# TAU-VAILab/Vox-E

Hardware: AMD Instinct MI355X
Metric: rendered rays/sec (fwd+bwd) (higher is better)
Workload: dtype f32; 1 GPU; 160^3 SH-0 softplus ReLU-field grid (random), one 400x400 camera per GPU and step, the steps cycle through 20 cameras of the 100-view set, S=256, jitter on, white bkgd, ray order image; step = render fwd + bwd + Adam (fused grid step); grid=160, samples_per_ray=256, grad_exchange=single, optimizer=fused

## Files before the change

### include/voxe.h

```cpp
#ifndef VOXE_H_
#define VOXE_H_

#include <stddef.h>
#include <stdint.h>

#ifdef __cplusplus
extern "C" {
#endif

#define VOXE_ABI_VERSION 13

typedef enum VoxeStatus {
  VOXE_OK = 0,
  VOXE_ERR_NULL_POINTER = -1,
  VOXE_ERR_BAD_SHAPE = -2,
  VOXE_ERR_UNSUPPORTED = -3,
  VOXE_ERR_WORKSPACE = -4,
  VOXE_ERR_LAUNCH = -5,
  VOXE_ERR_NO_DEVICE = -6
} VoxeStatus;

typedef enum VoxeAct {
  VOXE_ACT_IDENTITY = 0,
  VOXE_ACT_ABS = 1,
// ... 139 lines not shown
int voxe_render_bwd_acc_into(const VoxeGridDesc* grid, const VoxeRenderCfg* cfg,
                             const float* rays_o, const float* rays_d, int64_t R, const float* jitter,
                             const float* colour, const float* depth, const float* acc,
                             const float* d_colour, const float* d_depth, const float* d_acc,
                             int32_t want_densities, int32_t want_features, int32_t zero_first, int32_t* grad_layout,
                             void* workspace, size_t workspace_bytes, void* grad_workspace, size_t grad_workspace_bytes,
                             void* stream);
int voxe_render_bwd_layout(const VoxeGridDesc* grid, const VoxeRenderCfg* cfg, int64_t R);
size_t voxe_workspace_grad_offset(const VoxeGridDesc* grid);
size_t voxe_workspace_grad_bytes(const VoxeGridDesc* grid);
typedef struct VoxeGridRegularisers {
  const float* dcl_reference;
  float dcl_weight;
  float* dcl_loss;
  void* scratch;
  size_t scratch_bytes;
  int32_t density_kind;
  const float* feat_reference;
  float feat_weight;
  float* feat_loss;
} VoxeGridRegularisers;
int voxe_grid_adam_step(const VoxeGridDesc* grid, int32_t grad_layout, int32_t x_begin, int32_t x_end,
                        const float* extra_d_densities, const float* extra_d_features,
                        float* exp_avg_densities, float* exp_avg_sq_densities,
                        float* exp_avg_features, float* exp_avg_sq_features,
                        float lr, float beta1, float beta2, float eps, int64_t step, int64_t step_features,
                        const VoxeGridRegularisers* regularisers ,
                        void* workspace, size_t workspace_bytes, void* stream);

enum { VOXE_ROUTE_NONE = -1, VOXE_ROUTE_SCATTER = 0, VOXE_ROUTE_TILE = 1, VOXE_ROUTE_PACKED_SCATTER = 2,
       VOXE_ROUTE_REGION = 3, VOXE_ROUTE_DETERMINISTIC = 4 };
int voxe_render_route(const VoxeGridDesc* grid, const VoxeRenderCfg* cfg, int64_t R);

int voxe_disparity_bwd(const float* depth, const float* acc, const float* d_disparity, const float* d_depth_in,
                       const float* d_acc_in, float* d_depth_out, float* d_acc_out, int64_t R, void* stream);

typedef struct {
  int32_t H, W;
  float focal;
  const float* poses;
  const int64_t* image_rows;
  const float* images;
  int32_t num_images;
  int32_t K;
  int64_t batch;
  int32_t diffuse_regularisation;
  float lr, beta1, beta2, eps;
  int64_t step_densities, step_features;
  float *exp_avg_densities, *exp_avg_sq_densities, *exp_avg_features, *exp_avg_sq_features;
  float* losses;
  int32_t zero_gradient_first;
} VoxeReconStep;
size_t voxe_recon_scratch_bytes(int64_t batch);
int voxe_recon_step(const VoxeGridDesc* grid, const VoxeRenderCfg* cfg, const VoxeReconStep* step,
                    void* workspace, size_t workspace_bytes, void* workspace2, size_t workspace2_bytes,
                    void* scratch, size_t scratch_bytes, void* stream);
int voxe_recon_prefetch(const VoxeGridDesc* grid, const VoxeRenderCfg* cfg, const VoxeReconStep* next_step,
                        void* workspace, size_t workspace_bytes, void* workspace2, size_t workspace2_bytes,
                        void* scratch, size_t scratch_bytes, void* stream);
int voxe_recon_prefetch_stats(int64_t* out);

size_t voxe_attn_masked_l1_scratch_bytes(void);
int voxe_attn_masked_l1(const float* render, const float* attn_map, int64_t n, float* d_render, float* loss_out,
                        void* scratch, size_t scratch_bytes, void* stream);

typedef struct {
  const float* attn_map;
  float tv_weight;
  int32_t tv_loss_always;
  float lr, beta1, beta2, eps;
  int64_t step;
  float *exp_avg, *exp_avg_sq;
  float* losses;
  float* attn_render;
  int32_t zero_gradient_first;
} VoxeAttnRefineStep;
size_t voxe_attn_refine_scratch_bytes(const VoxeGridDesc* grid, int64_t R);
int voxe_attn_refine_step(const VoxeGridDesc* grid, const VoxeRenderCfg* cfg, const VoxeAttnRefineStep* step,
                          const float* rays_o, const float* rays_d, int64_t R, void* workspace, size_t workspace_bytes,
                          void* scratch, size_t scratch_bytes, void* stream);

int voxe_clock_probe(int32_t spin, double* shader_hz, void* stream);
int voxe_region_debug_layout(const VoxeGridDesc* grid, const VoxeRenderCfg* cfg, int64_t R, int64_t out[17]);

int voxe_adam_step(float* param, const float* grad, float* exp_avg, float* exp_avg_sq, int64_t n,
                   float lr, float beta1, float beta2, float eps, int64_t step, void* stream);

int voxe_upsample_trilinear(const float* src, int32_t X, int32_t Y, int32_t Z, int32_t C,
                            float* dst, int32_t X2, int32_t Y2, int32_t Z2, void* stream);


#define VOXE_GRAPH_CAP_ONE (1 << 28)
enum { VOXE_DIR_XP = 0, VOXE_DIR_XM = 1, VOXE_DIR_YP = 2, VOXE_DIR_YM = 3, VOXE_DIR_ZP = 4, VOXE_DIR_ZM = 5 };

int voxe_graph_build(const float* density_grid, const float* feature_grid,
                     int32_t X, int32_t Y, int32_t Z, int32_t F, float sigma, int32_t dilate_yz,
                     uint8_t* node_mask, int32_t* cap, void* stream);

size_t voxe_graphcut_scratch_bytes(int32_t X, int32_t Y, int32_t Z);
int voxe_graphcut(const uint8_t* node_mask, const int8_t* terminal, int32_t* cap,
                  int32_t X, int32_t Y, int32_t Z, uint8_t* segment, int64_t* flow,
                  void* scratch, size_t scratch_bytes, void* stream);

size_t voxe_cc_scratch_bytes(int32_t X, int32_t Y, int32_t Z, int32_t k);
int voxe_cc_largest_k(const uint8_t* mask, int32_t X, int32_t Y, int32_t Z, int32_t k,
                      int32_t* labels, int32_t* num_components,
                      void* scratch, size_t scratch_bytes, void* stream);

size_t voxe_mesh_scratch_bytes(int32_t X, int32_t Y, int32_t Z);
int voxe_mesh_count(const VoxeGridDesc* grid, float level, const uint8_t* mask, int64_t* totals,
                    void* scratch, size_t scratch_bytes, void* stream);
int voxe_mesh_emit(const VoxeGridDesc* grid, float level, const uint8_t* mask,
                   float* vertices, int64_t max_vertices, int32_t* faces, int64_t max_faces,
                   void* scratch, size_t scratch_bytes, void* stream);

int voxe_query_normals(const VoxeGridDesc* grid, const float* points, int64_t N, float* normals, void* stream);
int voxe_render_normals(const VoxeGridDesc* grid, const VoxeRenderCfg* cfg,
                        const float* rays_o, const float* rays_d, int64_t R, const float* jitter,
                        float* normals, float* depth, float* acc, void* stream);

int voxe_visibility_accumulate(const VoxeGridDesc* grid, const VoxeRenderCfg* cfg,
                               const float* rays_o, const float* rays_d, int64_t R, const float* jitter,
                               float* max_weight , float* max_trans ,
                               void* stream);
int voxe_visibility_mask(const float* vis, int32_t X, int32_t Y, int32_t Z, float threshold, int32_t dilate,
                         uint8_t* mask , void* stream);

size_t voxe_distortion_scratch_bytes(int64_t R);
int voxe_distortion_fwd_bwd(const VoxeGridDesc* grid, const VoxeRenderCfg* cfg,
                            const float* rays_o, const float* rays_d, int64_t R, const float* jitter,
                            float grad_scale,
                            float* loss_out      ,
                            float* ray_loss      ,
                            float* d_densities   ,
                            int32_t accumulate   ,
                            void* scratch, size_t scratch_bytes, void* stream);
int voxe_distortion_debug_lanes(int32_t lanes);

int voxe_cpu_cast_rays(int32_t H, int32_t W, float focal, const float* rot, const float* trans,
                       float* rays_o, float* rays_d);
int voxe_cpu_cast_rays_indexed(int32_t H, int32_t W, float focal, const float* poses, int32_t K,
                               const int64_t* flat_index, int64_t B, float* rays_o, float* rays_d);
int voxe_cpu_random_subset(int64_t n, int64_t count, uint64_t seed, uint64_t rng_offset, int64_t* out);
int voxe_cpu_render_fwd(const VoxeGridDesc* grid, const VoxeRenderCfg* cfg,
                        const float* rays_o, const float* rays_d, int64_t R, const float* jitter,
                        float* colour, float* depth, float* acc, float* disparity);
int voxe_cpu_render_bwd(const VoxeGridDesc* grid, const VoxeRenderCfg* cfg,
                        const float* rays_o, const float* rays_d, int64_t R, const float* jitter,
                        const float* d_colour, const float* d_depth, const float* d_acc,
                        float* d_densities, float* d_features, int32_t accumulate);
int voxe_cpu_query_fwd(const VoxeGridDesc* grid, const float* points, int64_t N, float* out);
int voxe_cpu_query_bwd(const VoxeGridDesc* grid, const float* points, int64_t N, const float* d_out,
                       float* d_densities, float* d_features, int32_t accumulate);
int voxe_cpu_sample_probe(const VoxeGridDesc* grid, const VoxeRenderCfg* cfg,
                          const float* rays_o, const float* rays_d, int64_t R, const float* jitter,
                          int32_t* idx, uint8_t* inside, float* zvals, float* sigma, float* rad);
int voxe_cpu_dcl_fwd_bwd(const float* a, const float* b, int64_t n, float grad_scale,
                         float* loss_out, float* d_a, int32_t accumulate);
int voxe_cpu_density_diff_fwd_bwd(const float* a, const float* b, int64_t n, int32_t kind, float grad_scale,
                                  float* loss_out, float* d_a, int32_t accumulate);
int voxe_cpu_feature_correlation_fwd_bwd(const float* f, const float* r, int64_t nvox, int32_t F, float grad_scale,
                                         float* loss_out, float* d_f, int32_t accumulate);
int voxe_cpu_tv_fwd_bwd(const float* grid, int32_t X, int32_t Y, int32_t Z, int32_t C,
                        float grad_scale, float* loss_out, float* d_grid, int32_t accumulate);
int voxe_cpu_adam_step(float* param, const float* grad, float* exp_avg, float* exp_avg_sq,
                       int64_t n, float lr, float beta1, float beta2, float eps, int64_t step);
// ... 17 lines not shown
```

### vox-e_amd/csrc/voxe_api.hip

```cpp
#include <hip/hip_runtime.h>
#include <stdlib.h>
#include <string.h>

#include <mutex>
#include <unordered_map>

#include "../../include/voxe.h"
#include "voxe_launch.hpp"
#include "voxe_render_common.hpp"

using namespace voxe;

namespace {

const VoxeDispatch kDefaultDispatch = {};
const VoxeDispatch& disp_of(const VoxeRenderCfg* c) { return (c && c->dispatch) ? *c->dispatch : kDefaultDispatch; }
bool force_scatter_bwd(const VoxeDispatch& d) { return d.bwd_mode == 1; }
bool force_no_tile_bwd(const VoxeDispatch& d) { return d.bwd_mode != 0; }
bool two_phase_disabled(const VoxeDispatch& d) { return d.tile_two_phase < 0; }

int tile_map_mode(int image_width, const VoxeDispatch& d) {
  if (d.tile_map >= 1 && d.tile_map <= 3) return d.tile_map - 1;
  return image_width > 0 ? 0 : 1;
}
// ... 238 lines not shown

int voxe_device_check(char* name, size_t name_len) {
  int dev = 0;
  if (hipGetDevice(&dev) != hipSuccess) return VOXE_ERR_NO_DEVICE;
  hipDeviceProp_t prop;
  if (hipGetDeviceProperties(&prop, dev) != hipSuccess) return VOXE_ERR_NO_DEVICE;
  if (name && name_len) {
    strncpy(name, prop.gcnArchName, name_len - 1);
    name[name_len - 1] = 0;
  }
  return strncmp(prop.gcnArchName, "gfx950", 6) == 0 ? VOXE_OK : VOXE_ERR_NO_DEVICE;
}

int voxe_profile_enable(int32_t on) {
  if (on && !g_prof.created) {
    for (int i = 0; i < Profiler::kMax; ++i)
      for (int j = 0; j < 2; ++j)
        if (hipEventCreate(&g_prof.ev[i][j]) != hipSuccess) return VOXE_ERR_LAUNCH;
    g_prof.created = true;
  }
  g_prof.on = on != 0;
  g_prof.count = 0;
  g_prof.dropped = 0;
  return VOXE_OK;
}

int voxe_profile_read(VoxeProfile* out) {
  if (!out) return VOXE_ERR_NULL_POINTER;
  memset(out, 0, sizeof(*out));
  double* ms[PH_COUNT] = {&out->ms_pack, &out->ms_fwd, &out->ms_memset, &out->ms_bwd, &out->ms_unpack};
  int32_t* n[PH_COUNT] = {&out->n_pack, &out->n_fwd, &out->n_memset, &out->n_bwd, &out->n_unpack};
  for (int i = 0; i < g_prof.count; ++i) {
    if (hipEventSynchronize(g_prof.ev[i][1]) != hipSuccess) return VOXE_ERR_LAUNCH;
    float t = 0.f;
    if (hipEventElapsedTime(&t, g_prof.ev[i][0], g_prof.ev[i][1]) != hipSuccess) return VOXE_ERR_LAUNCH;
    *ms[g_prof.phase[i]] += (double)t;
    *n[g_prof.phase[i]] += 1;
  }
  out->n_dropped = g_prof.dropped;
  g_prof.count = 0;
  g_prof.dropped = 0;
  return VOXE_OK;
}

int voxe_cast_rays(int32_t H, int32_t W, float focal, const float* rot, const float* trans,
                   float* rays_o, float* rays_d, void* stream) {
  if (!rot || !trans || !rays_o || !rays_d) return VOXE_ERR_NULL_POINTER;
  if (H <= 0 || W <= 0) return VOXE_ERR_BAD_SHAPE;
  launch_cast_rays(H, W, focal, rot, trans, rays_o, rays_d, (hipStream_t)stream);
  return finish();
}

int voxe_cast_rays_indexed(int32_t H, int32_t W, float focal, const float* poses, int32_t K,
                           const int64_t* flat_index, int64_t B, float* rays_o, float* rays_d, void* stream) {
  if (!poses || !flat_index || !rays_o || !rays_d) return VOXE_ERR_NULL_POINTER;
  if (H <= 0 || W <= 0 || K <= 0 || B < 0) return VOXE_ERR_BAD_SHAPE;
  if (B == 0) return VOXE_OK;
  launch_cast_rays_indexed(H, W, focal, poses, K, (const long long*)flat_index, B, rays_o, rays_d,
                           (hipStream_t)stream);
  return finish();
}

int voxe_random_subset(int64_t n, int64_t count, uint64_t seed, uint64_t rng_offset, int64_t* out, void* stream) {
  if (!out) return VOXE_ERR_NULL_POINTER;
  if (n <= 0 || n > (1ll << 31) || count < 0 || count > n) return VOXE_ERR_BAD_SHAPE;
  if (count == 0) return VOXE_OK;
  launch_random_subset(n, count, seed, rng_offset, (long long*)out, (hipStream_t)stream);
  return finish();
}

int voxe_tile_sched_debug_layout(const VoxeGridDesc* grid, const VoxeRenderCfg* cfg, int64_t R, int64_t out[4]) {
  Variant v;
  const int st = validate(grid, cfg, R, &v);
  if (st) return st;
  if (!out) return VOXE_ERR_NULL_POINTER;
  DevGrid dg; HostCfg dc;
  make_dev(grid, cfg, R, v, &dg, &dc);
  const WsLayout l = ws_layout(grid, cfg, R);
  const int64_t ntp = dc.image_width > 0 ? blocks_for_tiles(dc.map_mode, (dc.image_width + 7) / 8, tile_rows_total(dc, 8)) : 0;
  out[0] = (l.total > l.sched_off && tile_sched_applies(dc)) ? 1 : 0;
  out[1] = (int64_t)l.sched_off;
  out[2] = ntp * num_segments(dc.S, dc.seg_len);
  out[3] = ntp;
  return VOXE_OK;
}

size_t voxe_workspace_bytes(const VoxeGridDesc* grid, const VoxeRenderCfg* cfg, int64_t R) {
  if (!grid || grid->X <= 0 || grid->Y <= 0 || grid->Z <= 0 || grid->F <= 0) return 0;
  const WsLayout l = ws_layout(grid, cfg, R);
  if (cfg && cfg->ray_state_valid < 0) return l.total;
  return l.total_with_src;
}

int voxe_render_fwd(const VoxeGridDesc* grid, const VoxeRenderCfg* cfg, const float* rays_o,
                    const float* rays_d, int64_t R, const float* jitter, float* colour, float* depth,
                    float* acc, float* disparity, void* workspace, size_t workspace_bytes,
                    void* stream) {
  Variant v;
  const int st = validate(grid, cfg, R, &v);
  if (st) return st;
  if (R > 0 && (!rays_o || !rays_d || !colour)) return VOXE_ERR_NULL_POINTER;
  const WsLayout l = ws_layout(grid, cfg, R);
  if (!workspace || workspace_bytes < l.fwd_total) return VOXE_ERR_WORKSPACE;
  hipStream_t s = (hipStream_t)stream;
  float* packed = (float*)((char*)workspace + l.packed_off);
  if (!cfg->reuse_packed_grid) { PhaseTimer t(PH_PACK, s); launch_pack_any(grid, packed, s); }
  if (R == 0) return finish();
  {
    FwdStamp k = make_stamp(grid, cfg, rays_o, rays_d, R, jitter, workspace_bytes);
    k.kept = cfg->ray_state_valid >= 0 ? 1 : 0;
    record_stamp(workspace, k);
  }
  DevGrid dg; HostCfg dc;
  make_dev(grid, cfg, R, v, &dg, &dc);
  float* state = nullptr;
  const bool tiled = tile_bwd_supported(dc, cfg->sh_degree) && !force_no_tile_bwd(dc.disp);
  const bool packed_bwd = !tiled && packed_scatter_supported(cfg->sh_degree) && !force_scatter_bwd(dc.disp);
  if ((tiled || packed_bwd) && workspace_bytes >= l.total) state = (float*)((char*)workspace + l.state_off);
  float* segbuf = workspace_bytes >= l.total ? (float*)((char*)workspace + l.seg_off) : nullptr;
  FwdArgs a{packed, rays_o, rays_d, jitter, colour, depth, acc, disparity, state, segbuf};
  a.keep_samples = cfg->ray_state_valid >= 0;
  if (segbuf && cfg->ray_state_valid >= 0 && precise_sums_apply(l, dg, dc, cfg, jitter)) a.segsum_d = (double*)((char*)workspace + l.prec_off);
  if (segbuf && l.total > l.sched_off) a.sched = (int*)((char*)workspace + l.sched_off);
  if (cfg->ray_state_valid >= 0 && tiled && l.fwdval_off > l.src_off && workspace_bytes >= l.total_with_src && !two_phase_disabled(dc.disp))
    a.sample_fwd = (float*)((char*)workspace + l.fwdval_off);
  if (l.region && workspace_bytes >= l.total_with_src) {
    PhaseTimer t(PH_FWD, s);
    launch_fwd_region(dg, dc, cfg->sh_degree, cfg->render_diffuse, a, (char*)workspace + l.region_off, s);
    return finish();
  }
  { PhaseTimer t(PH_FWD, s); launch_fwd(dg, dc, cfg->sh_degree, cfg->render_diffuse, a, s); }
  return finish();
}

}

namespace {
int render_bwd_common(const VoxeGridDesc* grid, const VoxeRenderCfg* cfg, const Variant& v, const float* rays_o,
                      const float* rays_d, int64_t R, const float* jitter, const float* colour, const float* depth,
                      const float* acc, const float* d_colour, const float* d_depth, const float* d_acc, bool want_d,
                      bool want_f, bool zero_first, bool* bricked, void* workspace, size_t workspace_bytes,
                      hipStream_t s, void* grad_workspace = nullptr, size_t grad_workspace_bytes = 0) {
  const WsLayout l = ws_layout(grid, cfg, R);
  if (!workspace || workspace_bytes < l.total) return VOXE_ERR_WORKSPACE;
  if (grad_workspace && grad_workspace_bytes < l.state_off) return VOXE_ERR_WORKSPACE;
  float* packed = (float*)((char*)workspace + l.packed_off);
  float* gpacked = (float*)((char*)(grad_workspace ? grad_workspace : workspace) + l.grad_off);
  float* state = (float*)((char*)workspace + l.state_off);
  if (!cfg->reuse_packed_grid) { PhaseTimer t(PH_PACK, s); launch_pack_any(grid, packed, s); }
  if (zero_first) {
    PhaseTimer t(PH_MEMSET, s);
    if (hipMemsetAsync(gpacked, 0, l.state_off - l.grad_off, s) != hipSuccess) return VOXE_ERR_LAUNCH;
  }
  *bricked = false;
  if (R > 0) {
    DevGrid dg; HostCfg dc;
    make_dev(grid, cfg, R, v, &dg, &dc);
    const bool tiled = tile_bwd_supported(dc, cfg->sh_degree) && !force_no_tile_bwd(dc.disp);
    const bool packed_bwd = !tiled && packed_scatter_supported(cfg->sh_degree) && !force_scatter_bwd(dc.disp);
    BwdArgs a{packed, rays_o, rays_d, jitter, colour, depth, acc, d_colour, d_depth, d_acc, gpacked,
              want_d, want_f, (tiled || packed_bwd) ? state : nullptr};
    const bool precise = precise_sums_apply(l, dg, dc, cfg, jitter);
    if (precise) a.segsum_d = (const double*)((char*)workspace + l.prec_off);
    if (l.total > l.sched_off) a.sched = (const int*)((char*)workspace + l.sched_off);
    const bool two_phase = tiled && l.fwdval_off > l.src_off && workspace_bytes >= l.total_with_src && !two_phase_disabled(dc.disp);
    if (two_phase) {
// ... 981 lines not shown
```

### vox-e_amd/csrc/voxe_launch.hpp

```cpp
#pragma once

#include <hip/hip_runtime.h>

#include "voxe_device.hpp"

namespace voxe {

struct FwdArgs {
  const float *packed, *rays_o, *rays_d, *jitter;
  float *colour, *depth, *acc, *disparity;
  float* ray_state;
  float* segbuf;
  float* sample_fwd = nullptr;
  bool keep_samples = true;
  double* segsum_d = nullptr;
  int* sched = nullptr;
};
struct BwdArgs {
  const float *packed, *rays_o, *rays_d, *jitter, *colour, *depth, *acc, *d_colour, *d_depth, *d_acc;
  float* gpacked;
  bool want_d, want_f;
  const float* ray_state;
  float* sample_src = nullptr;
  const float* sample_fwd = nullptr;
  float* grad_planar = nullptr;
  unsigned long long* gdet = nullptr;
  float* det_scale = nullptr;
  const double* segsum_d = nullptr;
  const int* sched = nullptr;
};
struct HostCfg : DevCfg {
  VoxeDispatch disp;
};
inline long long disp_tile_min_rays(const VoxeDispatch& d) { return d.tile_min_rays == 0 ? 8192ll : (d.tile_min_rays < 0 ? 0ll : (long long)d.tile_min_rays); }
inline long long disp_region_min_rays(const VoxeDispatch& d) { return d.region_min_rays == 0 ? 16384ll : (long long)d.region_min_rays; }
inline bool disp_region_lds_ranks(const VoxeDispatch& d) { return d.region_lds_ranks >= 0; }
inline float disp_region_image_ratio(const VoxeDispatch& d) { return d.region_image_ratio == 0.0f ? 1.3f : (d.region_image_ratio < 0.0f ? 0.0f : d.region_image_ratio); }
inline float disp_or(float v, float dflt) { return v == 0.0f ? dflt : v; }

struct ProbeArgs {
  const float *packed, *rays_o, *rays_d, *jitter;
  int32_t* idx;
  uint8_t* inside;
  float *zvals, *sigma, *rad;
};


void launch_pack_any(const VoxeGridDesc* gd, float* packed, hipStream_t st);
void launch_unpack_any(const VoxeGridDesc* gd, const float* gpacked, float* d_dens, float* d_feat,
                       int accumulate, int bricked, hipStream_t st);
struct DclTerm {
  const float* b = nullptr;
  const double* stats = nullptr;
  int kind = 0;
  float k = 0.0f;
  const float* fref = nullptr;
  float fk = 0.0f;
};
bool launch_grid_adam(const VoxeGridDesc* gd, bool bricked, int x_begin, int x_end, float* gpacked, const float* extra_d, const float* extra_f,
                      float* m_d, float* v_d, float* m_f, float* v_f, float lr, float beta1, float beta2, float eps,
                      long long step_d, long long step_f, float* packed_out, hipStream_t st, DclTerm dcl = DclTerm());
const double* launch_dcl_moments(const float* a, const float* b, long long n, float grad_scale, float* loss_out, void* scratch,
                                 hipStream_t st);
void launch_fwd(const DevGrid& g, const HostCfg& c, int deg, int diffuse, const FwdArgs& a,
                hipStream_t st);
void launch_bwd(const DevGrid& g, const DevCfg& c, int deg, int diffuse, const BwdArgs& a,
                hipStream_t st);
void launch_probe(const DevGrid& g, const DevCfg& c, int deg, int diffuse, const ProbeArgs& a,
                  hipStream_t st);

void launch_query(const DevGrid& g, int C, const float* packed, const float* points, long long N, float* out,
                  const float* d_out, float* gpacked, bool want_d, bool want_f, hipStream_t st);

bool tile_bwd_supported(const HostCfg& c, int deg);
size_t tile_src_bytes(long long R, int W, int H, int S, int deg, int diffuse, int attn);
void launch_bwd_tile(const DevGrid& g, const HostCfg& c, int deg, int diffuse, const BwdArgs& a, hipStream_t st);
bool tile4_bwd_supported(const DevGrid& g, const HostCfg& c, const BwdArgs& a, int kl);
void launch_bwd_tile4(const DevGrid& g, const HostCfg& c, const BwdArgs& a, int kl, int nb, int qsplit, float fit_m, float fit_lat,
                      hipStream_t st);
size_t tile_planar_bytes(long long nvox, int cm);
bool tile4_dep_supported(const DevGrid& g, const HostCfg& c, const BwdArgs& a, int ncu, int cm);
void launch_bwd_tile4_dep(const DevGrid& g, const HostCfg& c, const BwdArgs& a, int ncu, int nb, int qsplit, int ngrp, float fit_m,
                          float fit_lat, hipStream_t st);
bool fwd_tile4_supported(const DevGrid& g, const HostCfg& c, const FwdArgs& a, int cout, int ncm);
void launch_fwd_tile4(const DevGrid& g, const HostCfg& c, const FwdArgs& a, hipStream_t st);
bool tile_sched_applies(const HostCfg& c);
size_t tile_sched_bytes(long long R, int W, int H, int S);
bool fwd_tile_supported(const DevGrid& g, const HostCfg& c, int cout, int ncm);
void launch_fwd_tile(const DevGrid& g, const HostCfg& c, const FwdArgs& a, hipStream_t st);
bool fwd_tilew_supported(const DevGrid& g, const HostCfg& c, const FwdArgs& a, int cout, int ncm, int ncu);
void launch_fwd_tilew(const DevGrid& g, const HostCfg& c, int ncm, const FwdArgs& a, hipStream_t st);
bool det_bwd_supported(const DevCfg& c, int deg, int diffuse);
size_t det_bytes(long long nvox, int C);

bool packed_scatter_supported(int deg);
void launch_bwd_packed_scatter(const DevGrid& g, const DevCfg& c, int deg, int diffuse, const BwdArgs& a, hipStream_t st);

bool region_bwd_supported(const DevGrid& g, const HostCfg& c, int deg, int diffuse, bool tiled);
size_t region_scratch_bytes(int X, int Y, int Z, long long R, int S, bool full_sh);
void launch_fwd_region(const DevGrid& g, const HostCfg& c, int deg, int diffuse, const FwdArgs& a, void* scratch,
                       hipStream_t st);
void launch_bwd_region(const DevGrid& g, const DevCfg& c, int deg, int diffuse, const BwdArgs& a, void* scratch,
                       hipStream_t st);
struct RegionBins { void* tables; int prebinned; hipEvent_t after_fwd; };
extern thread_local const RegionBins* tl_region_bins;
void launch_bin_region(const DevGrid& g, const HostCfg& c, const float* rays_o, const float* rays_d, const float* jitter, void* tables,
                       hipStream_t st, int phase = 3);
void region_debug_layout(int X, int Y, int Z, long long R, int S, long long out[16]);

void launch_cast_rays(int H, int W, float focal, const float* rot, const float* trans, float* rays_o,
                      float* rays_d, hipStream_t st);
void launch_cast_rays_indexed(int H, int W, float focal, const float* poses, int K, const long long* flat_index,
                              long long B, float* rays_o, float* rays_d, hipStream_t st);
void launch_random_subset(long long n, long long count, unsigned long long seed, unsigned long long rng_offset,
                          long long* out, hipStream_t st);
size_t dcl_scratch_bytes(long long n);
void launch_density_diff(const float* a, const float* b, long long n, int kind, float grad_scale, float* loss_out, float loss_norm,
                         float* d_a, int accumulate, void* scratch, hipStream_t st);
void launch_feature_correlation(const float* f, const float* r, long long nvox, int F, float grad_scale, float* loss_out, float* d_f,
                                int accumulate, void* scratch, hipStream_t st);
void launch_dcl(const float* a, const float* b, long long n, float grad_scale, float* loss_out,
                float* d_a, int accumulate, void* scratch, hipStream_t st);
size_t tv_scratch_bytes(int X, int Y, int Z, int C);
void launch_tv(const float* grid, int X, int Y, int Z, int C, float grad_scale, float* loss_out,
               float* d_grid, int accumulate, void* scratch, hipStream_t st);
void launch_adam(float* param, const float* grad, float* m, float* v, long long n, float lr,
                 float beta1, float beta2, float eps, long long step, hipStream_t st);
void launch_upsample(const float* src, int X, int Y, int Z, int C, float* dst, int X2, int Y2, int Z2,
                     hipStream_t st);
void launch_disparity_bwd(const float* depth, const float* acc, const float* d_disp, const float* d_depth_in,
                          const float* d_acc_in, float* d_depth_out, float* d_acc_out, long long R, hipStream_t st);
void launch_gather_pixels(const float* images, const long long* image_rows, const long long* subset, long long B, int per,
                          int num_images, float* out, hipStream_t st);
size_t l1_scratch_bytes();
void launch_l1_loss_grad(const float* a, const float* b, long long n, float* d_a, float* out2, void* scratch, hipStream_t st);
size_t attn_l1_scratch_bytes();
void launch_attn_masked_l1(const float* render, const float* map, long long n, float* d_render, float* loss_out, void* scratch,
                           hipStream_t st);
void launch_l1_loss_grad_n(const float* a, const float* b, long long n, int renders, float* d_a, float* out2, void* scratch,
                           hipStream_t st);
void launch_recon_batch(long long B, unsigned long long seed, unsigned long long rng_offset, int H, int W, float focal, int K,
                        const float* poses, const float* images, const long long* image_rows, int num_images, long long* subset,
                        float* rays_o, float* rays_d, float* target, hipStream_t st);
double run_clock_probe(int spin, hipStream_t st);


void launch_graph_build(const float* dens, const float* feat, int X, int Y, int Z, int F, float sigma,
                        int dilate_yz, uint8_t* node_mask, int32_t* cap, hipStream_t stream);
size_t graphcut_scratch_bytes(int X, int Y, int Z);
hipError_t run_graphcut(const uint8_t* node_mask, const int8_t* terminal, int32_t* cap, int X, int Y, int Z,
                        uint8_t* segment, int64_t* flow, void* scratch, hipStream_t stream);
size_t cc_scratch_bytes(int X, int Y, int Z, int k);
void launch_cc_largest_k(const uint8_t* mask, int X, int Y, int Z, int k, int32_t* labels, int32_t* ncomp,
                         void* scratch, hipStream_t stream);

bool mesh_dims_ok(int X, int Y, int Z);
size_t mesh_scratch_bytes(int X, int Y, int Z);
void launch_mesh_count(const VoxeGridDesc* g, float L, const uint8_t* mask, int64_t* totals, void* scratch, hipStream_t st);
void launch_mesh_emit(const VoxeGridDesc* g, float L, const uint8_t* mask, float* vertices, long long max_vertices,
                      int32_t* faces, long long max_faces, void* scratch, hipStream_t st);

int normals_lanes_for(long long R);
void launch_query_normals(const DevGrid& g, const float* dens, const float* points, long long N, float* normals, hipStream_t st);
void launch_render_normals(const DevGrid& g, const DevCfg& c, const float* dens, const float* rays_o, const float* rays_d,
                           const float* jitter, float* normals, float* depth, float* acc, hipStream_t st);

void launch_visibility_accumulate(const DevGrid& g, const DevCfg& c, const float* dens, const float* rays_o, const float* rays_d,
                                  const float* jitter, float* max_weight, float* max_trans, hipStream_t st);
void launch_visibility_mask(const float* vis, int X, int Y, int Z, float threshold, int dilate, uint8_t* mask, hipStream_t st);

// ... 9 lines not shown
```

### vox-e_amd/csrc/voxe_render_tile.hip

```cpp
#include <limits.h>
#include <stdlib.h>

#include <type_traits>

#include "voxe_device.hpp"
#include "voxe_launch.hpp"
#include "voxe_render_common.hpp"
#include "voxe_tile_window.hpp"

namespace voxe {

template <int WC, int KL, bool DET = false>
__device__ __forceinline__ void flush_layer(double* __restrict__ win, float* __restrict__ gpacked,
                                            const Window& w, int key, int lane, int CM, int memch,
                                            unsigned long long* __restrict__ gdet = nullptr) {
  constexpr int C = WC;
  constexpr int kLat = KL, kLayerSlots = Lat<KL>::kLayerSlots;
  constexpr int kPerInstr = 64 / C;
  constexpr int NJ = (kLayerSlots + kPerInstr - 1) / kPerInstr;
  const int im = w.sgn * key;
  const int offu = __builtin_amdgcn_readfirstlane(w.off_u(im)), offv = __builtin_amdgcn_readfirstlane(w.off_v(im));
  const long long vox0 = (long long)im * w.stride_m + (long long)offu * w.stride_u + (long long)offv * w.stride_v;
  const int ch = lane % C;
  int idx[NJ];
// ... 887 lines not shown
        Cell cell;
        make_cell_fast(g, fp, cell);
        float v, rad[COUT];
        gather<3, 1, 1>(g, packed, cell, rc.basis, v, rad);
        const float sigma = post_activate(g.post_act, v);
        const float dl = last ? kInfinity : (z_next - z);
        const float delta = dl * rc.dnorm;
        const float e = fast_exp(-(sigma * delta));
        const float alpha = 1.0f - e;
        const float om = 1.0f - alpha;
        const float wgt = alpha * T;
        T = T * om;
#pragma unroll
        for (int ch = 0; ch < COUT; ++ch) csum[ch] = fmaf(sigmoidf(rad[ch]), wgt, csum[ch]);
        asum = asum + wgt;
        dsum = fmaf(z, wgt, dsum);
      }
    }
  };
  auto march_tile = [&](auto strata_tag) {
    constexpr bool ST = decltype(strata_tag)::value;
    const SegDepth<ST> sd{strat, ks};
    if (m < 0) march_rays(strata_tag);
    else if (m == 0) fwd_window_march<0, ST>(g, c, packed, rc, lane, has, k_lo, k_hi, kmin, kmax, ref, tex, org, sd, csum, asum, dsum, T);
    else if (m == 1) fwd_window_march<1, ST>(g, c, packed, rc, lane, has, k_lo, k_hi, kmin, kmax, ref, tex, org, sd, csum, asum, dsum, T);
    else fwd_window_march<2, ST>(g, c, packed, rc, lane, has, k_lo, k_hi, kmin, kmax, ref, tex, org, sd, csum, asum, dsum, T);
  };
  if (use_strata) march_tile(std::true_type{});
  else march_tile(std::false_type{});
  if (!alive) return;
  const long long base = (long long)seg * NC;
  segbuf[(base + 0) * c.R + r] = T;
#pragma unroll
  for (int ch = 0; ch < COUT; ++ch) segbuf[(base + 1 + ch) * c.R + r] = csum[ch];
  segbuf[(base + 1 + COUT) * c.R + r] = asum;
  segbuf[(base + 2 + COUT) * c.R + r] = dsum;
}

bool fwd_tile_supported(const DevGrid& g, const HostCfg& c, int cout, int ncm) {
  (void)g;
  if (cout != 3 || ncm != 1 || c.image_width <= 0) return false;
  return c.disp.fwd_window >= 0;
}
void launch_fwd_tile(const DevGrid& g, const HostCfg& c, const FwdArgs& a, hipStream_t st) {
  const int nseg = num_segments(c.S, c.seg_len);
  const int nb = blocks_for_tiles(c.map_mode, (c.image_width + 7) / 8, tile_rows_total(c, 8)) * nseg;
  const float fit_lat = disp_or(c.disp.fwd_fit_lat, 5.5f), fit_m = disp_or(c.disp.fwd_fit_m, 4.5f);
  const float zdom = disp_or(c.disp.fwd_zdom, 1.0f), max_adv = disp_or(c.disp.fwd_max_adv, 1.7f);
  render_fwd_tile_kernel<<<nb, 64, 0, st>>>(g, c, a.packed, a.rays_o, a.rays_d, a.jitter, a.segbuf, fit_lat, fit_m, zdom, max_adv);
}

bool tile_bwd_supported(const HostCfg& c, int deg) {
  (void)deg;
  return c.image_width > 0 && c.R >= disp_tile_min_rays(c.disp);
}

__global__ void det_scale_kernel(float* __restrict__ det_scale) {
  for (int i = 0; i < 2; ++i) {
    int e = 0;
    const float m = det_scale[i];
    if (m > 0.0f && m < 3.0e38f) (void)frexpf(m, &e);
    det_scale[2 + i] = ldexpf(1.0f, 38 - e);
  }
}
__global__ __launch_bounds__(256) void det_finalize_kernel(unsigned long long* __restrict__ gdet, float* __restrict__ gpacked,
                                                           long long n, int CM, const float* __restrict__ det_scale) {
  const double inv_f = 1.0 / (double)det_scale[2], inv_d = 1.0 / (double)det_scale[3];
  const long long stride = (long long)gridDim.x * blockDim.x;
  for (long long i = (long long)blockIdx.x * blockDim.x + threadIdx.x; i < n; i += stride) {
    const long long q = (long long)gdet[i];
    if (q != 0) {
      gpacked[i] += (float)((double)q * ((int)(i % CM) == CM - 1 ? inv_d : inv_f));
      gdet[i] = 0ull;
    }
  }
}
size_t det_bytes(long long nvox, int C) { return (((size_t)nvox * C * 8 + 255) / 256 + 1) * 256; }
bool det_bwd_supported(const DevCfg& c, int deg, int diffuse) {
  return c.image_width > 0 && (c.attn || deg == 0 || diffuse);
}

constexpr float kWideWindowRatio = 0.58f;

template <int COUT, int NCM, int NCU>
static void launch_bwd_tile_t(const DevGrid& g, const HostCfg& c, const BwdArgs& a, hipStream_t st) {
  const long long ntx8 = (c.image_width + 7) / 8, nty8 = tile_rows_total(c, 8);
  const int env_q = c.disp.tile_qsplit;
  constexpr int NG = COUT * NCU + 1, WC = NG < 4 ? NG : 4, NGRP = (NG + WC - 1) / WC;
  const int grp_begin = a.want_f ? 0 : NGRP - 1, ngrp = a.want_f ? NGRP : 1;
  const long long tiles = ntx8 * nty8 * num_segments(c.S, c.seg_len) * ngrp;
  const int qsplit = env_q ? (env_q == 4 ? 4 : 1) : (tiles <= 11000 ? 4 : 1);
  const int nb = blocks_for_tiles(c.map_mode, ntx8, nty8) * num_segments(c.S, c.seg_len) * qsplit * ngrp;
  const float env_fit_m = c.disp.tile_fit_m;
  const long long tile_segs = ntx8 * nty8 * num_segments(c.S, c.seg_len);
  const int side_for_kl = g.X > g.Y ? (g.X > g.Z ? g.X : g.Z) : (g.Y > g.Z ? g.Y : g.Z);
  const bool wide = (float)side_for_kl >= kWideWindowRatio * (float)c.image_width;
  const float env_fit_lat = c.disp.tile_fit_lat;
  const float fit_lat = env_fit_lat;
  const float fit_m = env_fit_m > 0.0f ? env_fit_m : (qsplit == 4 ? (wide ? 4.5f : 4.0f) : (tile_segs <= 16000 ? 4.5f : 5.5f));
#define VOXE_TBWD(WD, WF, MODE, KL, NB, GB, NGR)                                                 \
  render_bwd_tile_kernel<COUT, NCM, NCU, WD, WF, MODE, KL><<<NB, 64, 0, st>>>(                    \
      g, c, a.packed, a.rays_o, a.rays_d, a.jitter, a.colour, a.depth, a.acc, a.d_colour,         \
      a.d_depth, a.d_acc, a.ray_state, a.gpacked, qsplit, GB, NGR, reinterpret_cast<float4*>(a.sample_src), nullptr, nullptr, 0, fit_m, fit_lat, \
      reinterpret_cast<const float4*>(a.sample_fwd))
  if constexpr (NGRP == 1) {
    if (a.gdet) {
      const long long n = (long long)g.X * g.Y * g.Z * (COUT * NCM + 1);
      (void)hipMemsetAsync(a.det_scale, 0, 4 * sizeof(float), st);
      for (int phase = 0; phase < 2; ++phase) {
        render_bwd_tile_kernel<COUT, NCM, NCU, true, true, 0, 8, true><<<nb, 64, 0, st>>>(
            g, c, a.packed, a.rays_o, a.rays_d, a.jitter, a.colour, a.depth, a.acc, a.d_colour, a.d_depth, a.d_acc,
            a.ray_state, a.gpacked, qsplit, 0, 1, nullptr, a.gdet, a.det_scale, phase, fit_m, fit_lat);
        if (phase == 0) det_scale_kernel<<<1, 1, 0, st>>>(a.det_scale);
      }
      det_finalize_kernel<<<4096, 256, 0, st>>>(a.gdet, a.gpacked, n, COUT * NCM + 1, a.det_scale);
      return;
    }
  }
  if constexpr (NGRP > 1) {
    if (a.sample_src && a.want_f) {
      if (a.want_d) VOXE_TBWD(true, true, 1, 8, nb / ngrp, 0, 1);
      else VOXE_TBWD(false, true, 1, 8, nb / ngrp, 0, 1);
      if (NCM == NCU && tile4_dep_supported(g, c, a, NCU, COUT * NCM + 1))
        launch_bwd_tile4_dep(g, c, a, NCU, nb, qsplit, ngrp, fit_m, fit_lat, st);
      else
        VOXE_TBWD(true, true, 2, 8, nb, 0, ngrp);
      return;
    }
    if (a.want_d && a.want_f) VOXE_TBWD(true, true, 0, 8, nb, grp_begin, ngrp);
    else if (a.want_d) VOXE_TBWD(true, false, 0, 8, nb, grp_begin, ngrp);
    else VOXE_TBWD(false, true, 0, 8, nb, grp_begin, ngrp);
  } else {
    const int env_kl = c.disp.tile_kl;
    const int side = g.X > g.Y ? (g.X > g.Z ? g.X : g.Z) : (g.Y > g.Z ? g.Y : g.Z);
    const int kl = env_kl ? env_kl : ((float)side >= kWideWindowRatio * (float)c.image_width ? 10 : 8);
#define VOXE_TBWD_KL(KL)                                                       \
    do {                                                                       \
      if (a.want_d && a.want_f) VOXE_TBWD(true, true, 0, KL, nb, 0, 1);         \
      else if (a.want_d) VOXE_TBWD(true, false, 0, KL, nb, 0, 1);               \
      else VOXE_TBWD(false, true, 0, KL, nb, 0, 1);                             \
    } while (0)
    if constexpr (COUT == 3 && NCM == 1 && NCU == 1) {
      if (tile4_bwd_supported(g, c, a, kl)) {
        launch_bwd_tile4(g, c, a, kl, nb, qsplit, fit_m, fit_lat, st);
        return;
      }
    }
    if (kl == 10) VOXE_TBWD_KL(10);
#ifdef VOXE_TILE_KL_EXPERIMENTS
    else if (kl == 9 && COUT == 3 && NCM == 1 && a.want_d && a.want_f) VOXE_TBWD(true, true, 0, 9, nb, 0, 1);
    else if (kl == 12 && COUT == 3 && NCM == 1 && a.want_d && a.want_f) VOXE_TBWD(true, true, 0, 12, nb, 0, 1);
    else if (kl == 16 && COUT == 3 && NCM == 1 && a.want_d && a.want_f) VOXE_TBWD(true, true, 0, 16, nb, 0, 1);
#endif
    else VOXE_TBWD_KL(8);
#undef VOXE_TBWD_KL
  }
#undef VOXE_TBWD
}

size_t tile_src_bytes(long long R, int W, int H1, int S, int deg, int diffuse, int attn) {
  if (W <= 0 || R <= 0 || deg <= 0 || diffuse || attn) return 0;
  const long long H = H1 > 0 ? H1 : R / W, nimg = R / (H * W);
  const long long tiles = ((W + 7) / 8) * ((H + 7) / 8) * (nimg > 0 ? nimg : 1);
  const int seg = seg_len_for(R);
  const size_t bytes = (size_t)tiles * num_segments(S, seg) * seg * 64 * sizeof(float4);
  return bytes <= ((size_t)4 << 30) ? bytes : 0;
}

void launch_bwd_tile(const DevGrid& g, const HostCfg& c, int deg, int diffuse, const BwdArgs& a, hipStream_t st) {
  if (c.attn) launch_bwd_tile_t<1, 1, 1>(g, c, a, st);
  else if (deg == 0) launch_bwd_tile_t<3, 1, 1>(g, c, a, st);
  else if (deg == 1) { if (diffuse) launch_bwd_tile_t<3, 4, 1>(g, c, a, st); else launch_bwd_tile_t<3, 4, 4>(g, c, a, st); }
  else if (deg == 2) { if (diffuse) launch_bwd_tile_t<3, 9, 1>(g, c, a, st); else launch_bwd_tile_t<3, 9, 9>(g, c, a, st); }
  else { if (diffuse) launch_bwd_tile_t<3, 16, 1>(g, c, a, st); else launch_bwd_tile_t<3, 16, 16>(g, c, a, st); }
}

}
```

### vox-e_amd/csrc/voxe_render_tile4.hip

```cpp
#include <limits.h>

#include <type_traits>

#include "voxe_device.hpp"
#include "voxe_launch.hpp"
#include "voxe_render_common.hpp"
#include "voxe_tile_window.hpp"

namespace voxe {

#ifndef VOXE_TILE4_LB
#define VOXE_TILE4_LB 3
#endif
#ifndef VOXE_T4_EXP
#define VOXE_T4_EXP 0
#endif
#ifndef VOXE_T4_SKEW
#define VOXE_T4_SKEW 0
#endif
#ifndef VOXE_T4_CHJ
#define VOXE_T4_CHJ 1
#endif
#ifndef VOXE_T4_PHASE_MARGIN
#define VOXE_T4_PHASE_MARGIN 0.0f
#endif
#ifndef VOXE_T4_REMAT
#define VOXE_T4_REMAT 0
#endif
#ifndef VOXE_T4_DEBUG
#define VOXE_T4_DEBUG 0
#endif

struct Tile4Args {
  const float *packed, *rays_o, *rays_d, *colour, *depth, *acc, *d_colour, *d_depth, *d_acc, *ray_state;
  float* gpacked;
  int qsplit;
  float fit_m, fit_lat;
  int want_d, want_f;
  int phases;
  const double* segsum;
  const float4* sample_src;
  int ngrp, ng;
  long long nvox;
  const int* sched;
};

constexpr int kSchedMaxBuckets = 9;
constexpr int kSchedMaxSegs = 64;
constexpr int kSchedEmpty = (int)0x80000000;
constexpr long long kSchedMaxBlocks = 1ll << 18;
#ifndef VOXE_SCHED_BUCKET
#define VOXE_SCHED_BUCKET 4
#endif
static_assert(VOXE_SCHED_BUCKET >= 4 && 32 / VOXE_SCHED_BUCKET + 1 <= kSchedMaxBuckets, "bucket rows of the schedule histogram");

template <class RC>
__device__ __forceinline__ void seg_sample_range(const RC& rc, const bool alive, const int ks, const int ke, int& k_lo, int& k_hi) {
  k_lo = max(rc.k_lo, ks);
  k_hi = alive ? min(rc.k_hi, ke) : k_lo - 1;
}
__device__ __forceinline__ int sched_rank(int it, int nbk) {
  return it == 0 ? nbk - 1 : nbk - 1 - min((it + VOXE_SCHED_BUCKET - 1) / VOXE_SCHED_BUCKET, nbk - 1);
}

__global__ __launch_bounds__(1024) void tile_sched_cost_kernel(const DevGrid g, const DevCfg c, const float* __restrict__ rays_o,
                                                               const float* __restrict__ rays_d, const int ntp, const int nbk,
                                                               const int hstride, unsigned char* __restrict__ cost,
                                                               unsigned char* __restrict__ hist) {
  __shared__ unsigned char rk[kSchedMaxSegs][16];
  const int lane = threadIdx.x & 63, w = threadIdx.x >> 6;
  const int rb = blockIdx.x * 16 + w;
  const int nseg = num_segments(c.S, c.seg_len);
  const int ntx = (c.image_width + 7) >> 3, nty = (int)tile_rows_total(c, 8);
  const int tile = rb < ntp ? logical_tile_of(c, rb, ntp, ntx, nty) : -1;
  if (tile < 0) {
    for (int seg = lane; seg < nseg; seg += 64) {
      if (rb < ntp) cost[(long long)seg * ntp + rb] = 0;
      rk[seg][w] = rb < ntp ? (unsigned char)(nbk - 1) : (unsigned char)255;
    }
  } else {
    const int ty = tile / ntx, tx = tile - ty * ntx;
    long long r_px;
    const bool alive = tile_pixel_ray(c, ty, lane >> 3, (tx << 3) + (lane & 7), 8, r_px);
    const long long r = alive ? r_px : 0;
    RayCtx<3, 1, 1> rc;
    rc.init(g, c, r, rays_o, rays_d, nullptr);
    for (int seg = 0; seg < nseg; ++seg) {
      const int ks = seg * c.seg_len, ke = min(c.S, ks + c.seg_len) - 1;
      int k_lo, k_hi;
      seg_sample_range(rc, alive, ks, ke, k_lo, k_hi);
      const bool has = k_lo <= k_hi;
      const int kmin = wave_min_i32(has ? k_lo : INT_MAX);
      const int kmax = wave_max_i32(has ? k_hi : -1);
      const int it = kmin <= kmax ? kmax - kmin + 1 : 0;
      if (lane == 0) {
        cost[(long long)seg * ntp + rb] = (unsigned char)it;
        rk[seg][w] = (unsigned char)sched_rank(it, nbk);
      }
    }
  }
  __syncthreads();
  const int ngrp = gridDim.x;
  for (int p = threadIdx.x; p < nseg * nbk; p += 1024) {
    const int seg = p / nbk, r = p - seg * nbk;
    int n = 0;
#pragma unroll
    for (int i = 0; i < 16; ++i) n += rk[seg][i] == r ? 1 : 0;
    hist[(long long)r * hstride + seg * ngrp + blockIdx.x] = (unsigned char)n;
  }
}

__device__ __forceinline__ int wave_sum_i32(int v) {
#pragma unroll
  for (int d = 1; d < 64; d <<= 1) v += __shfl_xor(v, d, 64);
  return v;
}

__global__ __launch_bounds__(256) void tile_sched_scatter_kernel(const unsigned char* __restrict__ cost,
                                                                 const unsigned char* __restrict__ hist, const int ntp,
                                                                 const int ngrp, const int nbk, const int hstride,
                                                                 int* __restrict__ list) {
  __shared__ int s_tot[kSchedMaxBuckets], s_pre[kSchedMaxBuckets], s_base[kSchedMaxBuckets];
  __shared__ int s_wc[kSchedMaxBuckets][4];
  const int tid = threadIdx.x, lane = tid & 63, w = tid >> 6;
  const int seg = blockIdx.y, nseg = gridDim.y;
  const int H = nseg * ngrp;
  const int G0 = seg * ngrp + blockIdx.x * 16;
  for (int r = w; r < nbk; r += 4) {
    const unsigned int* row = reinterpret_cast<const unsigned int*>(hist + (long long)r * hstride);
    int tot = 0, pre = 0;
    for (int q = lane; q * 4 < H; q += 64) {
      const unsigned int v = row[q];
#pragma unroll
      for (int i = 0; i < 4; ++i) {
        const int e = 4 * q + i, n = (int)(v >> (8 * i) & 255u);
        tot += e < H ? n : 0;
        pre += e < G0 ? n : 0;
      }
    }
    tot = wave_sum_i32(tot); pre = wave_sum_i32(pre);
    if (lane == 0) { s_tot[r] = tot; s_pre[r] = pre; }
  }
  const int rb = blockIdx.x * 256 + tid;
  const bool valid = rb < ntp;
  const int b = seg * ntp + rb;
  const int it = valid ? (int)cost[b] : 0;
  const int rank = valid ? sched_rank(it, nbk) : -1;
  int within = 0, mine = 0;
  for (int r = 0; r < nbk; ++r) {
    const unsigned long long m = __ballot(rank == r);
    if (rank == r) within = __popcll(m & ((1ull << lane) - 1ull));
    if (lane == r) mine = __popcll(m);
  }
  if (lane < nbk) s_wc[lane][w] = mine;
  __syncthreads();
  if (tid < nbk) {
    int base = s_pre[tid];
    for (int r = 0; r < tid; ++r) base += s_tot[r];
    s_base[tid] = base;
  }
  __syncthreads();
  if (valid) {
    int pos = s_base[rank] + within;
    for (int i = 0; i < w; ++i) pos += s_wc[rank][i];
    list[pos] = it == 0 ? (b | kSchedEmpty) : b;
  }
}

bool tile_sched_applies(const HostCfg& c) {
  if ((c.disp.tile_map != 0 && c.disp.tile_map != 4) || c.image_width <= 0 || c.attn || c.disp.fwd_segments_per_thread > 1) return false;
  const int nseg = num_segments(c.S, c.seg_len);
  const long long tiles = (long long)((c.image_width + 7) / 8) * tile_rows_total(c, 8);
  const long long nb = (long long)blocks_for_tiles(c.map_mode, (c.image_width + 7) / 8, tile_rows_total(c, 8)) * nseg;
  return nseg > 1 && nseg <= kSchedMaxSegs && c.seg_len <= 32 && (tiles * nseg > 11000 || c.disp.tile_map == 4) && nb <= kSchedMaxBlocks;
}
static long long sched_hist_stride(long long ntp, int nseg) { return ((ntp + 15) / 16 * nseg + 3) / 4 * 4; }
static long long sched_cost_bytes(long long nb) { return (nb + 15) / 16 * 16; }
size_t tile_sched_bytes(long long R, int W, int H1, int S) {
  if (W <= 0 || R <= 0) return 0;
  const long long H = H1 > 0 ? H1 : R / W, nimg = R / (H * W);
  const long long ntp = (((W + 7) / 8) * ((H + 7) / 8) * (nimg > 0 ? nimg : 1) + 7) / 8 * 8;
  const int nseg = num_segments(S, seg_len_for(R));
  const long long nb = ntp * nseg;
  if (nb > kSchedMaxBlocks) return 0;
  return (size_t)nb * sizeof(int) + (size_t)sched_cost_bytes(nb) + (size_t)(kSchedMaxBuckets * sched_hist_stride(ntp, nseg));
}
static void build_tile_sched(const DevGrid& g, const HostCfg& c, const float* rays_o, const float* rays_d, int* sched, hipStream_t st) {
  const int nseg = num_segments(c.S, c.seg_len);
  const int ntp = blocks_for_tiles(c.map_mode, (c.image_width + 7) / 8, tile_rows_total(c, 8));
  const int nb = ntp * nseg;
  unsigned char* cost = reinterpret_cast<unsigned char*>(sched + nb);
  unsigned char* hist = cost + sched_cost_bytes(nb);
  const int nbk = (c.seg_len + VOXE_SCHED_BUCKET - 1) / VOXE_SCHED_BUCKET + 1;
  const int ngrp = (ntp + 15) / 16, hstride = (int)sched_hist_stride(ntp, nseg);
  tile_sched_cost_kernel<<<ngrp, 1024, 0, st>>>(g, c, rays_o, rays_d, ntp, nbk, hstride, cost, hist);
  tile_sched_scatter_kernel<<<dim3((ntp + 255) / 256, nseg), 256, 0, st>>>(cost, hist, ntp, ngrp, nbk, hstride, sched);
}

struct DepCtx {
  float mA[4], mB[4];
  int cA, cB;
  long long src_base;
};

constexpr int kTabKeys = 64;

template <int KL>
struct Pcb {
  static_assert(WinMap<KL, 4>::kPcb, "the lean kernel needs the parity-class banked window");
  static constexpr int SB = WinMap<KL, 4>::kSB * 8, SA = WinMap<KL, 4>::kSA * 8, SS = WinMap<KL, 4>::kSS * 8;
  static __device__ __forceinline__ int mterm(int slot) { return (slot >> 1) * SS + ((slot & 1) << 5); }
  static __device__ __forceinline__ int aterm(int x_even) { return (x_even >> 1) * SA; }
  static __device__ __forceinline__ int bterm(int x_even) { return (x_even >> 1) * SB; }
};

struct Geo4 {
  float Au, Bu, Av, Bv;
  int sgn;
};

__device__ __forceinline__ int rfl(int x) { return __builtin_amdgcn_readfirstlane(x); }
__device__ __forceinline__ unsigned mad24(unsigned a, unsigned b, unsigned c) {
  unsigned r;
  asm("v_mad_u32_u24 %0, %1, %2, %3" : "=v"(r) : "v"(a), "s"(b), "v"(c));
  return r;
}
typedef __attribute__((address_space(1))) char gchar;
typedef __attribute__((address_space(1))) float gfloat;
__device__ __forceinline__ gchar* scalar_ptr(unsigned long long v) {
  unsigned lo = (unsigned)__builtin_amdgcn_readfirstlane((int)(unsigned)v), hi = (unsigned)__builtin_amdgcn_readfirstlane((int)(unsigned)(v >> 32));
  asm volatile("" : "+s"(lo), "+s"(hi));
  return reinterpret_cast<gchar*>(((unsigned long long)hi << 32) | lo);
}
__device__ __forceinline__ void global_add_f32(gchar* base, unsigned voff, float x) {
  asm volatile("" : "+v"(voff));
  __hip_atomic_fetch_add(reinterpret_cast<gfloat*>(base + (size_t)voff), x, __ATOMIC_RELAXED, __HIP_MEMORY_SCOPE_AGENT);
}
__device__ __forceinline__ int wave_min_dpp(int v) {
  asm volatile(
      "s_nop 1\n\t"
      "v_min_i32_dpp %0, %0, %0 quad_perm:[1,0,3,2] row_mask:0xf bank_mask:0xf\n\t"
      "s_nop 1\n\t"
      "v_min_i32_dpp %0, %0, %0 quad_perm:[2,3,0,1] row_mask:0xf bank_mask:0xf\n\t"
      "s_nop 1\n\t"
      "v_min_i32_dpp %0, %0, %0 row_half_mirror row_mask:0xf bank_mask:0xf\n\t"
      "s_nop 1\n\t"
      "v_min_i32_dpp %0, %0, %0 row_mirror row_mask:0xf bank_mask:0xf\n\t"
      "s_nop 1"
      : "+v"(v));
  const int a = __builtin_amdgcn_readlane(v, 0), b = __builtin_amdgcn_readlane(v, 16);
  const int c = __builtin_amdgcn_readlane(v, 32), d = __builtin_amdgcn_readlane(v, 48);
  return min(min(a, b), min(c, d));
}

__device__ __forceinline__ bool tile_lanes_down_columns(const DevGrid& g, const float (&d0)[3], const float (&dx)[3], const float (&dy)[3]) {
  float ex[3], ey[3];
  const int N[3] = {g.X, g.Y, g.Z};
#pragma unroll
  for (int a = 0; a < 3; ++a) {
    const float s = g.scale[a] * (float)N[a];
    ex[a] = (dx[a] - d0[a]) * s;
    ey[a] = (dy[a] - d0[a]) * s;
  }
  const float lat_x = ex[0] * ex[0] + ex[1] * ex[1], lat_y = ey[0] * ey[0] + ey[1] * ey[1];
  return (ey[2] * ey[2]) * lat_x > (ex[2] * ex[2]) * lat_y;
}

template <int MA, int KL, bool PREC, bool DEP, int NP = 1, bool LK = (NP > 1)>
__device__ __forceinline__ void bwd4_march(const DevGrid& g, const DevCfg& c, const Tile4Args& a, RayCtx<3, 1, 1>& rc,
                                           double* __restrict__ win, int2* __restrict__ tab, const int lane, const long long r,
                                           bool has, const int k_lo, int k_hi, const int kmin, const int kmax, const int seg,
                                           const int ks, const Geo4 geo, const float strat_lo, const float strat_sp,
                                           const DepCtx& dep, const int phase = 0, const int xm1 = 0, const int xm2 = 0, const int koff = 0) {
  static_assert(!LK || (!PREC && !DEP), "per-lane sample indices (phases, skew): the SH-0 float kernel only");
  static_assert(NP == 1 || LK, "sample phases need the per-lane sample index");
  constexpr int UA = (MA == 0) ? 1 : 0, VA = (MA == 2) ? 1 : 2;
  constexpr int COUT = 3;
  constexpr int kCtr = Lat<KL>::kCentre;
  typedef Pcb<KL> P;
  static_assert(!(DEP && PREC), "deposit passes carry no suffix sums");
  constexpr unsigned TB = 16u;

  float gc[COUT] = {0.0f, 0.0f, 0.0f}, gsum = 0.0f;
  if constexpr (!DEP) {
#pragma unroll
    for (int ch = 0; ch < COUT; ++ch) { gc[ch] = a.d_colour[r * COUT + ch]; gsum += gc[ch]; }
  }
  const float gdep = (!DEP && a.d_depth) ? a.d_depth[r] : 0.0f;
  const float gacc = (!DEP && a.d_acc) ? a.d_acc[r] : 0.0f;
  const bool white = c.white != 0;
  float T = 1.0f, suffix0 = 0.0f;
  if constexpr (!DEP) {
    const float asum = a.acc[r];
    float total = gdep * a.depth[r] + gacc * asum;
#pragma unroll
    for (int ch = 0; ch < COUT; ++ch) {
      const float csum = white ? a.colour[r * COUT + ch] - (1.0f - asum) : a.colour[r * COUT + ch];
      total += gc[ch] * csum;
    }
    if (white) total -= gsum * asum;
    suffix0 = total;
    if (seg > 0) {
      constexpr int NC = COUT + 3;
      float suf_c[COUT];
      T = a.ray_state[ray_state_index(seg, 0, NC, c.R, r)];
#pragma unroll
      for (int ch = 0; ch < COUT; ++ch) suf_c[ch] = a.ray_state[ray_state_index(seg, 1 + ch, NC, c.R, r)];
      const float suf_a = a.ray_state[ray_state_index(seg, 1 + COUT, NC, c.R, r)];
      const float suf_d = a.ray_state[ray_state_index(seg, 2 + COUT, NC, c.R, r)];
      suffix0 = gdep * suf_d + gacc * suf_a;
#pragma unroll
      for (int ch = 0; ch < COUT; ++ch) suffix0 += gc[ch] * suf_c[ch];
      if (white) suffix0 -= gsum * suf_a;
    }
  }
  float suffix_next = 0.0f, T_start = 1.0f, Tl = 1.0f;
  double rem = 0.0;
  if constexpr (PREC) {
    constexpr int NC = COUT + 3;
    const int nseg_p = num_segments(c.S, c.seg_len);
    T_start = T;
    if (seg + 1 < nseg_p) {
      suffix_next = gdep * a.ray_state[ray_state_index(seg + 1, 2 + COUT, NC, c.R, r)] +
                    gacc * a.ray_state[ray_state_index(seg + 1, 1 + COUT, NC, c.R, r)];
#pragma unroll
      for (int ch = 0; ch < COUT; ++ch) suffix_next += gc[ch] * a.ray_state[ray_state_index(seg + 1, 1 + ch, NC, c.R, r)];
      if (white) suffix_next -= gsum * a.ray_state[ray_state_index(seg + 1, 1 + COUT, NC, c.R, r)];
    }
    const double* const ss = a.segsum + (long long)seg * 5 * c.R + r;
    const double sa = ss[3 * c.R];
    rem = (double)gdep * ss[4 * c.R] + ((double)gacc - (double)(white ? gsum : 0.0f)) * sa;
#pragma unroll
    for (int ch = 0; ch < COUT; ++ch) rem = fma((double)gc[ch], ss[(long long)ch * c.R], rem);
    rem += T_start > 0.0f ? (double)suffix_next / (double)T_start : 0.0;
  }
  const float gsumw = white ? gsum : 0.0f;
  float gcf[COUT];
#pragma unroll
  for (int ch = 0; ch < COUT; ++ch) gcf[ch] = a.want_f ? gc[ch] : 0.0f;
  const float dmask = a.want_d ? 1.0f : 0.0f;
  float run = 0.0f;

  const int hm = (lane >> 1) & 1, hu = (lane >> 2) & 1, hv = (lane >> 3) & 1;
  const int crot = (lane & 1) | ((lane >> 3) & 2);
  const int k0u = 1 - hu, k1u = hu, k0v = 1 - hv, k1v = hv;
  const int KU0 = hu << 4, KU1 = (1 - hu) << 4;
#if VOXE_T4_CHJ
  const int KV0 = hv << 3, KV1 = (1 - hv) << 3;
  int CHJ[4];
#pragma unroll
  for (int j = 0; j < 4; ++j) CHJ[j] = ((j + crot) & 3) << 6;
#define VOXE_CH(bv, j) CHJ[j]
#else
  const int KV0 = 0, KV1 = 0;
  int CH[2][4];
#pragma unroll
  for (int cv = 0; cv < 2; ++cv)
#pragma unroll
    for (int j = 0; j < 4; ++j) CH[cv][j] = ((hv ^ cv) << 3) + (((j + crot) & 3) << 6);
#define VOXE_CH(bv, j) CH[bv][j]
#endif
  const bool c1 = crot & 1, c2 = crot & 2;

  const int sgn = geo.sgn;
  const int smask = sgn < 0 ? -1 : 0;
  const int sx = g.Y * g.Z, sy = g.Z;
  const int stride_m = (MA == 0) ? sx : ((MA == 1) ? sy : 1);
  const int stride_u = (UA == 0) ? sx : sy;
  const int stride_v = (VA == 1) ? sy : 1;
  auto build_tab = [&](int key0) {
    const int key = key0 + lane, im = sgn * key;
    const int ou = (int)floorf(geo.Au + geo.Bu * (float)im) - kCtr, ov = (int)floorf(geo.Av + geo.Bv * (float)im) - kCtr;
    tab[lane] = make_int2((ou & 0xffff) | (ov << 16), P::mterm(ring_slot(key)));
  };

  auto depth_of = [&](int k) {
    const int j = k - ks;
    const float lo = __int_as_float(__builtin_amdgcn_readlane(__float_as_int(strat_lo), j));
    const float sp = __int_as_float(__builtin_amdgcn_readlane(__float_as_int(strat_sp), j));
    const float su = sp * jitter_uniform(rc.dg.base, k);
    return lo + su;
  };
  auto depth_lane = [&](int k) {
    const int j = (k - ks) & 63;
    const float lo = __shfl(strat_lo, j, 64), sp = __shfl(strat_sp, j, 64);
    const float su = sp * jitter_uniform(rc.dg.base, k);
    return lo + su;
  };
  int kf = k_lo;
  int kb0 = kmin, kb1 = kmax;
  if constexpr (LK) {
    kb0 = wave_min_i32(has ? k_lo - koff : INT_MAX);
    kb1 = wave_max_i32(has ? k_hi - koff : -(1 << 30));
    const int m = (kb0 + koff - k_lo) % NP;
    kf = k_lo + (m < 0 ? m + NP : m);
    if (kf > k_hi) has = false;
  }
  float z_cur = 0.0f;
  Footprint fp;
  fp.inside = false;
#pragma unroll
  for (int ax = 0; ax < 3; ++ax) { fp.i0[ax] = 0; fp.w[ax][0] = fp.w[ax][1] = 0.0f; }
  int nextkey = INT_MAX;
  if (has) {
    const float2 st0 = depth_stratum(rc.dg, kf);
    const float su0 = st0.y * jitter_uniform(rc.dg.base, kf);
    z_cur = st0.x + su0;
    float p[3];
    rc.point(z_cur, p);
    footprint(g, p, fp);
    nextkey = fp.i0[MA] ^ smask;
  }
  int base = wave_min_i32(nextkey);
  int key0 = base;
  build_tab(key0);
  __syncthreads();

  const int q4 = lane >> 2, ch4 = lane & 3;
  constexpr int NJ = (KL == 8) ? KL / 2 : (KL * KL + 15) / 16;
  int fl_lds[KL == 8 ? 1 : NJ];
  unsigned fl_vox[KL == 8 ? 1 : NJ];
  if constexpr (KL == 8) {
    const int fa = q4 & 1, fb = q4 >> 1;
    fl_lds[0] = ((fa << 1) + (fb >> 1) * (P::SB / 8) + (fb & 1) + (ch4 << 3)) * 8;
    fl_vox[0] = (unsigned)(fa * stride_u + fb * stride_v) * TB + (unsigned)(ch4 * 4);
  } else {
#pragma unroll
    for (int j = 0; j < NJ; ++j) {
      const int ab = j * 16 + q4, fa = ab / KL, fb = ab - fa * KL;
      const bool cell_live = ab < KL * KL;
      fl_lds[j] = cell_live ? ((fa >> 1) * P::SA + ((fa & 1) << 4) + (fb >> 1) * P::SB + ((fb & 1) << 3) + (ch4 << 6)) : -1;
      fl_vox[j] = (unsigned)(fa * stride_u + fb * stride_v) * TB + (unsigned)(ch4 * 4);
    }
  }
  const unsigned long long gaddr = reinterpret_cast<unsigned long long>(a.gpacked);
  const long long sm16 = (long long)stride_m * TB, su16 = (long long)stride_u * TB, sv16 = (long long)stride_v * TB;
#ifndef VOXE_T4_ZPAIR
#define VOXE_T4_ZPAIR 1
#endif
  constexpr bool kPair = VOXE_T4_ZPAIR && MA == 2 && KL == 8;
  unsigned long long pend[NJ];
#pragma unroll
  for (int j = 0; j < NJ; ++j) pend[j] = 0ull;
  unsigned long long pend_vb = 0ull;
  int npend = 0;
  unsigned long long pendB[kPair ? NJ : 1];
  unsigned long long pendB_vb = 0ull;
  int oddA = 0, oddB = 0;
  const bool lane_hi = lane >= 32;
  const unsigned step4 = (unsigned)(4 * stride_v) * TB;
  const unsigned vox_b03 = kPair ? fl_vox[0] - (lane_hi ? step4 : 0u) : 0u;
  auto flush_issue = [&](int key) __attribute__((always_inline)) {
    if (VOXE_T4_EXP & 4) return;
    const int2 e = tab[key - key0];
    const int ex = rfl(e.x), mt = rfl(e.y);
    const int ou = (int)(short)(ex & 0xffff), ov = ex >> 16;
// ... 76 lines not shown
      npend = 0;
      return;
    }
    consume_single(pend, pend_vb, 0);
    npend = 0;
  };

  const unsigned sxb = g.X > 1 ? (unsigned)(g.Y * g.Z) * 16u : 0u, syb = g.Y > 1 ? (unsigned)g.Z * 16u : 0u;
  const unsigned szb = g.Z > 1 ? 16u : 0u;
  const unsigned sxi = (unsigned)(g.Y * g.Z) * 16u, syi = (unsigned)g.Z * 16u;
  const char* const pbytes = reinterpret_cast<const char*>(a.packed);
  char* const gbytes = reinterpret_cast<char*>(a.gpacked);
  const int Sm1 = c.S - 1;
  const float term_eps = c.term_eps;
  const int nk0 = -key0;
  int nkey0 = nk0;

  for (int kb = kb0; kb <= kb1; kb += NP) {
    const int k = LK ? kb + koff : kb;
    const bool on = has && (k >= k_lo) && (k <= k_hi);
    const bool live = on && fp.inside;
    float z_n1 = 0.0f, z_nP = 0.0f;
    if constexpr (LK) {
      z_n1 = depth_lane(k + 1);
      z_nP = (NP > 1) ? depth_lane(k + NP) : z_n1;
    }
    if (live) {
      if (__builtin_amdgcn_ballot_w64(!cell_is_interior(g, fp)) != 0ull) {
        Cell cf;
        make_cell(g, fp, cf);
#pragma unroll
        for (int ax = 0; ax < 3; ++ax) { fp.i0[ax] = cf.i[ax]; fp.w[ax][0] = cf.w[ax][0]; fp.w[ax][1] = cf.w[ax][1]; }
      }
    }
    Cell cell;
#pragma unroll
    for (int ax = 0; ax < 3; ++ax) { cell.i[ax] = fp.i0[ax]; cell.w[ax][0] = fp.w[ax][0]; cell.w[ax][1] = fp.w[ax][1]; }
    float4 t[DEP ? 1 : 8];
    if constexpr (DEP) {
      const long long so = live ? dep.src_base + (long long)k * 64 : dep.src_base + (long long)ks * 64;
      t[0] = a.sample_src[so];
    } else {
      unsigned off0 = mad24((unsigned)cell.i[0], sxi, mad24((unsigned)cell.i[1], syi, (unsigned)cell.i[2] << 4));
      if (!live || (VOXE_T4_EXP & 1)) off0 = 0u;
#pragma unroll
      for (int q = 0; q < 8; ++q) {
        const unsigned o = off0 + ((q & 1) ? sxb : 0u) + ((q & 2) ? syb : 0u);
        t[q] = *reinterpret_cast<const float4*>(pbytes + ((size_t)o + ((q & 4) ? szb : 0u)));
      }
    }
    const int tm = (cell.i[MA] ^ hm) & 1;
    const int imA = cell.i[MA] + tm, imB = cell.i[MA] + 1 - tm;
    const int relA = ((imA ^ smask) - smask) + nkey0, relB = ((imB ^ smask) - smask) + nkey0;
    const int2 eA = tab[relA & (kTabKeys - 1)], eB = tab[relB & (kTabKeys - 1)];
    float f0, f1, f2, v;
    if constexpr (DEP) { f0 = t[0].x; f1 = t[0].y; f2 = t[0].z; v = t[0].w; }
    else interp_texels4(t, cell, f0, f1, f2, v);
    asm volatile("" ::"v"(f0), "v"(f1), "v"(f2), "v"(v));
    flush_consume();
    auto do_deposit = [&](const float (&gch)[4]) __attribute__((always_inline)) {
#if VOXE_T4_REMAT
      int ln = lane;
      asm volatile("" : "+v"(ln));
      const int hu = (ln >> 2) & 1, hv = (ln >> 3) & 1;
      const int crot = (ln & 1) | ((ln >> 3) & 2);
      const int k0u = 1 - hu, k1u = hu, k0v = 1 - hv, k1v = hv;
      const int KU0 = hu << 4, KU1 = (1 - hu) << 4;
      const int KV0 = hv << 3, KV1 = (1 - hv) << 3;
      int CHJ[4];
#pragma unroll
      for (int j = 0; j < 4; ++j) CHJ[j] = ((j + crot) & 3) << 6;
      const bool c1 = crot & 1, c2 = crot & 2;
#endif
      const int pm = cell.i[MA], pu = cell.i[UA], pv = cell.i[VA];
      const float wm0 = cell.w[MA][0], wm1 = cell.w[MA][1];
      const float wu0 = cell.w[UA][0], wu1 = cell.w[UA][1], wv0 = cell.w[VA][0], wv1 = cell.w[VA][1];
      int eAx = eA.x, eBx = eB.x;
      asm volatile("" : "+v"(eAx), "+v"(eBx));
      const int ouA = (int)(short)(eAx & 0xffff), ovA = eAx >> 16, ouB = (int)(short)(eBx & 0xffff), ovB = eBx >> 16;
      const int PU0 = pu + k0u, PU1 = pu + k1u, PV0 = pv + k0v, PV1 = pv + k1v;
      const int xA0 = PU0 - ouA, xA1 = PU1 - ouA, yA0 = PV0 - ovA, yA1 = PV1 - ovA;
      const int xB0 = PU0 - ouB, xB1 = PU1 - ouB, yB0 = PV0 - ovB, yB1 = PV1 - ovB;
      const int klrel = min(relA, relB);
      bool fits = (unsigned)(klrel - (base + nkey0)) < (unsigned)(kRing - 1);
      if constexpr (KL == 8) fits = fits && ((unsigned)(xA0 | xA1 | yA0 | yA1 | xB0 | xB1 | yB0 | yB1) < 8u);
      else fits = fits && (max(max(max((unsigned)xA0, (unsigned)xA1), max((unsigned)yA0, (unsigned)yA1)),
                               max(max((unsigned)xB0, (unsigned)xB1), max((unsigned)yB0, (unsigned)yB1))) < (unsigned)KL);
      if (VOXE_T4_DEBUG & 3) fits = false;
      if (fits) {
        const float wmA = tm ? wm1 : wm0, wmB = tm ? wm0 : wm1;
        auto pick2 = [](int x1, float w0, float w1, float& o0, float& o1) {
          const bool hi = x1 & 1;
          o0 = hi ? w1 : w0;
          o1 = hi ? w0 : w1;
        };
        float wuA[2], wuB[2], wvA[2], wvB[2];
        pick2(xA1, wu0, wu1, wuA[0], wuA[1]);
        pick2(xB1, wu0, wu1, wuB[0], wuB[1]);
        pick2(yA1, wv0, wv1, wvA[0], wvA[1]);
        pick2(yB1, wv0, wv1, wvB[0], wvB[1]);
        const float wmuA[2] = {wmA * wuA[0], wmA * wuA[1]}, wmuB[2] = {wmB * wuB[0], wmB * wuB[1]};
        const int MA0 = eA.y + KU0, MA1 = eA.y + KU1, MB0 = eB.y + KU0, MB1 = eB.y + KU1;
        const int muA[2] = {P::aterm(xA0 & ~1) + MA0, P::aterm(xA1 & ~1) + MA1};
        const int muB[2] = {P::aterm(xB0 & ~1) + MB0, P::aterm(xB1 & ~1) + MB1};
        const int bvA[2] = {P::bterm(yA0 & ~1) + KV0, P::bterm(yA1 & ~1) + KV1}, bvB[2] = {P::bterm(yB0 & ~1) + KV0, P::bterm(yB1 & ~1) + KV1};
        const float q0 = c1 ? gch[1] : gch[0], q1 = c1 ? gch[2] : gch[1], q2 = c1 ? gch[3] : gch[2], q3 = c1 ? gch[0] : gch[3];
        const double gr[4] = {(double)(c2 ? q2 : q0), (double)(c2 ? q3 : q1), (double)(c2 ? q0 : q2), (double)(c2 ? q1 : q3)};
        char* const wb = reinterpret_cast<char*>(win);
#pragma unroll
        for (int cc = 0; cc < 8; ++cc) {
          const int bm = cc & 1, bu = (cc >> 1) & 1, bv = cc >> 2;
          const double wgt = (double)((bm ? wmuB[bu] : wmuA[bu]) * (bm ? wvB[bv] : wvA[bv]));
          const int idx = (bm ? muB[bu] : muA[bu]) + (bm ? bvB[bv] : bvA[bv]);
#pragma unroll
          for (int j = 0; j < 4; ++j) {
            if (VOXE_T4_EXP & 2) { const double pr = gr[j] * wgt; const int ad = idx + VOXE_CH(bv, j); asm volatile("" ::"v"(pr), "v"(ad)); continue; }
            __hip_atomic_fetch_add(reinterpret_cast<double*>(wb + (idx + VOXE_CH(bv, j))), gr[j] * wgt, __ATOMIC_RELAXED,
                                   __HIP_MEMORY_SCOPE_WORKGROUP);
          }
        }
      } else {
        const int brel = base + nkey0;
        const int2 e0 = tm ? eB : eA, e1 = tm ? eA : eB;
        const int rel0 = tm ? relB : relA, rel1 = tm ? relA : relB;
        const unsigned vo = (unsigned)(pm * stride_m + pu * stride_u + pv * stride_v) * TB;
#pragma unroll
        for (int cc = 0; cc < 8; ++cc) {
          const int cm = cc & 1, cu = (cc >> 1) & 1, cv = cc >> 2;
          const float wgt = ((cm ? wm1 : wm0) * (cu ? wu1 : wu0)) * (cv ? wv1 : wv0);
          if (wgt != 0.0f) {
            const int2 es = cm ? e1 : e0;
            const int aa = pu + cu - (int)(short)(es.x & 0xffff), bb = pv + cv - (es.x >> 16);
            const bool inwin = !(VOXE_T4_DEBUG & 2) && ((unsigned)((cm ? rel1 : rel0) - brel) < (unsigned)kRing) &&
                               ((unsigned)aa < (unsigned)KL) && ((unsigned)bb < (unsigned)KL);
            if (inwin) {
              double* const wp = reinterpret_cast<double*>(reinterpret_cast<char*>(win) +
                                                           (es.y + (aa >> 1) * P::SA + ((aa & 1) << 4) + (bb >> 1) * P::SB + ((bb & 1) << 3)));
#pragma unroll
              for (int ch = 0; ch < 4; ++ch)
                __hip_atomic_fetch_add(wp + ch * 8, (double)(gch[ch] * wgt), __ATOMIC_RELAXED, __HIP_MEMORY_SCOPE_WORKGROUP);
            } else {
              float* const gp = reinterpret_cast<float*>(gbytes + (size_t)(vo + (unsigned)(cm * stride_m + cu * stride_u + cv * stride_v) * TB));
#pragma unroll
              for (int ch = 0; ch < 4; ++ch)
                atomicAdd(gp + ch, gch[ch] * wgt);
            }
          }
        }
      }
    };
    if constexpr (NP > 1) {
      const float z = z_cur;
      const bool last = (k == Sm1);
      const bool act = on && fp.inside;
      float om = 1.0f, alpha = 0.0f, dldw = 0.0f, de = 0.0f, dpost = 0.0f, c0 = 0.0f, c1 = 0.0f, c2 = 0.0f;
      if (act) {
        const float rad[COUT] = {kC0 * f0, kC0 * f1, kC0 * f2};
        float sigma;
        post_activate_vg(g.post_act, v, sigma, dpost);
        const float dl = last ? kInfinity : (z_n1 - z);
        const float delta = dl * rc.dnorm;
        const float e = fast_exp(-(sigma * delta));
        alpha = 1.0f - e;
        om = 1.0f - alpha;
        de = delta * e;
        c0 = sigmoidf(rad[0]); c1 = sigmoidf(rad[1]); c2 = sigmoidf(rad[2]);
        dldw = fmaf(gdep, z, gacc);
        dldw = fmaf(gc[0], c0, dldw); dldw = fmaf(gc[1], c1, dldw); dldw = fmaf(gc[2], c2, dldw);
        dldw -= gsumw;
      }
      auto of_phase = [&](float own, float (&out)[NP]) __attribute__((always_inline)) {
        if constexpr (NP == 1) { out[0] = own; return; }
        const float s1 = __shfl_xor(own, xm1, 64);
        float s2 = 0.0f, s3 = 0.0f;
        if constexpr (NP == 4) { s2 = __shfl_xor(own, xm2, 64); s3 = __shfl_xor(own, xm1 ^ xm2, 64); }
#pragma unroll
        for (int q = 0; q < NP; ++q) {
          const int x = phase ^ q;
          out[q] = (x == 0) ? own : ((x == 1) ? s1 : ((x == 2) ? s2 : s3));
        }
      };
      float omv[NP], dlv[NP], wkv[NP];
      of_phase(om, omv);
      float Tk = T, Tn = T;
#pragma unroll
      for (int q = 0; q < NP; ++q) {
        if (q < phase) Tk = Tk * omv[q];
        Tn = Tn * omv[q];
      }
      const float wk = alpha * Tk;
      of_phase(dldw, dlv);
      of_phase(wk, wkv);
      float run_k = run, run_n = run;
#pragma unroll
      for (int q = 0; q < NP; ++q) {
        run_n = fmaf(dlv[q], wkv[q], run_n);
        if (q == phase) run_k = run_n;
      }
      T = Tn;
      run = run_n;
      if (act) {
        const float suffix = last ? 0.0f : (suffix0 - run_k);
        const float tail = (om > 0.0f) ? suffix * fast_rcp(om) : 0.0f;
        const float dsig = de * fmaf(Tk, dldw, -tail);
        float gch[4];
        gch[0] = ((wk * gcf[0]) * (c0 * (1.0f - c0))) * kC0;
        gch[1] = ((wk * gcf[1]) * (c1 * (1.0f - c1))) * kC0;
        gch[2] = ((wk * gcf[2]) * (c2 * (1.0f - c2))) * kC0;
        gch[3] = (dsig * dpost) * dmask;
        if (!(VOXE_T4_EXP & 16) && (wk != 0.0f || gch[3] != 0.0f)) do_deposit(gch);
      }
      if (term_eps > 0.0f && Tn < term_eps && k <= k_hi) k_hi = k;
      if (on) {
        nextkey = INT_MAX;
        if (k + NP <= k_hi) {
          float pn[3];
          rc.point(z_nP, pn);
          footprint(g, pn, fp);
          z_cur = z_nP;
          nextkey = fp.i0[MA] ^ smask;
        }
      }
    } else {
    if (on) {
      const float z = z_cur;
      const bool last = (k == Sm1);
      const float z_next = last ? z : (LK ? z_n1 : depth_of(k + 1));
      if (fp.inside) {
        float gch[4];
        bool deposit;
        if constexpr (DEP) {
          const float sA = dep.cA == 0 ? f0 : (dep.cA == 1 ? f1 : (dep.cA == 2 ? f2 : v));
          const float sB = dep.cB == 0 ? f0 : (dep.cB == 1 ? f1 : (dep.cB == 2 ? f2 : v));
#pragma unroll
          for (int s4 = 0; s4 < 4; ++s4) gch[s4] = fmaf(sB, dep.mB[s4], sA * dep.mA[s4]);
          deposit = gch[0] != 0.0f || gch[1] != 0.0f || gch[2] != 0.0f || gch[3] != 0.0f;
        } else {
        const float rad[COUT] = {kC0 * f0, kC0 * f1, kC0 * f2};
        float sigma, dpost;
        post_activate_vg(g.post_act, v, sigma, dpost);
        const float dl = last ? kInfinity : (z_next - z);
        const float delta = dl * rc.dnorm;
        const float e = fast_exp(-(sigma * delta));
        const float alpha = 1.0f - e;
        const float om = 1.0f - alpha;
        float col[COUT], dldw, wk, suffix, Tk;
#pragma unroll
        for (int ch = 0; ch < COUT; ++ch) col[ch] = sigmoidf(rad[ch]);
        if constexpr (PREC) {
          const float wl = alpha * Tl;
          double dd = fma((double)gdep, (double)z, (double)gacc);
#pragma unroll
          for (int ch = 0; ch < COUT; ++ch) dd = fma((double)gc[ch], (double)col[ch], dd);
          dd -= (double)gsumw;
          rem = fma(-dd, (double)wl, rem);
          dldw = (float)dd;
          suffix = last ? 0.0f : T_start * (float)rem;
          Tk = T_start * Tl;
          wk = T_start * wl;
          Tl = Tl * om;
        } else {
          dldw = fmaf(gdep, z, gacc);
#pragma unroll
          for (int ch = 0; ch < COUT; ++ch) dldw = fmaf(gc[ch], col[ch], dldw);
          dldw -= gsumw;
          Tk = T;
          wk = alpha * T;
          run = fmaf(dldw, wk, run);
          suffix = last ? 0.0f : (suffix0 - run);
        }
        const float tail = (om > 0.0f) ? suffix * fast_rcp(om) : 0.0f;
        const float dsig = (delta * e) * fmaf(Tk, dldw, -tail);
#pragma unroll
        for (int ch = 0; ch < COUT; ++ch) gch[ch] = ((wk * gcf[ch]) * (col[ch] * (1.0f - col[ch]))) * kC0;
        gch[3] = (dsig * dpost) * dmask;
        if constexpr (PREC) { if (term_eps > 0.0f && Tk * om < term_eps) k_hi = k; }
        else { T = T * om; if (term_eps > 0.0f && T < term_eps) k_hi = k; }
        deposit = wk != 0.0f || gch[3] != 0.0f;
        }

        if (!(VOXE_T4_EXP & 16) && deposit) do_deposit(gch);
      }
      nextkey = INT_MAX;
      if (!last && k < k_hi) {
        float pn[3];
        rc.point(z_next, pn);
        footprint(g, pn, fp);
        z_cur = z_next;
        nextkey = fp.i0[MA] ^ smask;
      }
    }
    }
    if (__ballot(nextkey <= base) == 0ull) {
      int n = 0;
      do {
        if (!kPair || npend == 2) flush_consume(true);
        flush_issue(base + n);
        if (VOXE_T4_ZPAIR == 2 && kPair && npend == 2) flush_consume(true);
        ++n;
      } while (n < kRing && __ballot(nextkey <= base + n) == 0ull);
      base = (n == kRing) ? wave_min_dpp(nextkey) : base + n;
      if (base != INT_MAX && base + nkey0 > kTabKeys / 2) {
        key0 = base;
        nkey0 = -key0;
        build_tab(key0);
      }
    }
  }
  flush_consume(true);
  if (base != INT_MAX) {
    for (int i = 0; i < kRing; ++i) {
      flush_issue(base + i);
      if (!kPair || npend == 2) flush_consume(true);
    }
    flush_consume(true);
  }
}

template <int KL, bool PREC, int NCU_DEP = 0>
#ifndef VOXE_TILE4_LB_PREC
#define VOXE_TILE4_LB_PREC 2
#endif
__global__ __launch_bounds__(64, KL >= 9 ? 2 : (PREC ? VOXE_TILE4_LB_PREC : VOXE_TILE4_LB)) void render_bwd_tile4_kernel(const DevGrid g, const DevCfg c, const Tile4Args a_in) {
  constexpr bool DEP = NCU_DEP > 0;
  __shared__ double win[WinMap<KL, 4>::kDoubles];
  __shared__ int2 tab[kTabKeys];
  const int lane = threadIdx.x;
  int bid = blockIdx.x;
  if constexpr (!DEP) {
    if (a_in.sched) {
      bid = a_in.sched[blockIdx.x];
      if (bid < 0) return;
    }
  }
  for (int i = lane; i < WinMap<KL, 4>::kDoubles; i += 64) win[i] = 0.0;

  const int W = c.image_width;
  const int ntx = (W + 7) >> 3, nty = (int)tile_rows_total(c, 8);
  const int nseg = num_segments(c.S, c.seg_len);
  const int ntp = gridDim.x / (nseg * a_in.qsplit * (DEP ? a_in.ngrp : 1));
  int part = bid / ntp;
  int grp = 0;
  if constexpr (DEP) { grp = part / (nseg * a_in.qsplit); part -= grp * nseg * a_in.qsplit; }
  Tile4Args a = a_in;
  if constexpr (DEP) a.gpacked = a_in.gpacked + (long long)grp * a_in.nvox * 4;
  const int quad = part / nseg, seg = part - quad * nseg;
  const int tile = logical_tile_of(c, bid % ntp, ntp, ntx, nty);
  if (tile < 0) return;
  const int ks = seg * c.seg_len, ke = min(c.S, ks + c.seg_len) - 1;
  const int ty = tile / ntx, tx = tile - ty * ntx;
  long long r_px;
  bool alive = tile_pixel_ray(c, ty, lane >> 3, (tx << 3) + (lane & 7), 8, r_px);
  long long r = alive ? r_px : 0;

  RayCtx<3, 1, 1> rc;
  rc.init(g, c, r, a.rays_o, a.rays_d, nullptr);
#ifndef VOXE_T4_ORIENT
#define VOXE_T4_ORIENT 1
#endif
  bool columns = false;
  if (VOXE_T4_ORIENT && !DEP) {
    const unsigned long long am0 = __ballot(alive);
    if ((am0 & 1ull) && (am0 >> 1 & 1ull) && (am0 >> 8 & 1ull)) {
      const float d0[3] = {readlane_f32(rc.d[0], 0), readlane_f32(rc.d[1], 0), readlane_f32(rc.d[2], 0)};
      const float dx[3] = {readlane_f32(rc.d[0], 1), readlane_f32(rc.d[1], 1), readlane_f32(rc.d[2], 1)};
      const float dy[3] = {readlane_f32(rc.d[0], 8), readlane_f32(rc.d[1], 8), readlane_f32(rc.d[2], 8)};
      if (tile_lanes_down_columns(g, d0, dx, dy)) {
        columns = true;
        alive = tile_pixel_ray(c, ty, lane & 7, (tx << 3) + (lane >> 3), 8, r_px);
        r = alive ? r_px : 0;
        rc.init(g, c, r, a.rays_o, a.rays_d, nullptr);
      }
    }
  }

  int split = 0;
  bool phases_fit = false;
  bool phases_skew = false;
  {
    const unsigned long long am = __ballot(alive);
    if ((am >> 1 & 1ull) && (am >> 8 & 1ull)) {
      const int N[3] = {g.X, g.Y, g.Z};
      const float zref = readlane_f32(rc.dg.zlin(ke), 0);
      float d0[3], ex3[3], ey3[3];
#pragma unroll
      for (int ax = 0; ax < 3; ++ax) {
        const float s = g.scale[ax] * 0.5f * (float)N[ax];
        const float da = readlane_f32(rc.d[ax], 0);
        d0[ax] = fabsf(da * s);
        ex3[ax] = fabsf((readlane_f32(rc.d[ax], 1) - da) * s * zref);
        ey3[ax] = fabsf((readlane_f32(rc.d[ax], 8) - da) * s * zref);
      }
      const int m = (d0[0] >= d0[1] && d0[0] >= d0[2]) ? 0 : ((d0[1] >= d0[2]) ? 1 : 2);
      const float fit_lat = a.fit_lat > 0.0f ? a.fit_lat : (float)KL - 2.5f;
      const bool skew_ok = VOXE_T4_SKEW == 1 && !PREC && !DEP && a.phases >= 0;
      auto fits_pass = [&](float wx, float wy) {
        float e[3];
#pragma unroll
        for (int ax = 0; ax < 3; ++ax) e[ax] = wx * ex3[ax] + wy * ey3[ax];
        const float alongm = (m == 0) ? e[0] : ((m == 1) ? e[1] : e[2]);
        const float dm = (m == 0) ? d0[0] : ((m == 1) ? d0[1] : d0[2]);
        float lat = 0.0f;
#pragma unroll
        for (int ax = 0; ax < 3; ++ax)
          if (ax != m) lat = fmaxf(lat, skew_ok ? e[ax] + alongm * (d0[ax] / dm) : e[ax]);
        return lat <= fit_lat && (skew_ok || alongm <= a.fit_m);
      };
      if (!fits_pass(7.0f, 7.0f)) {
        const bool hx = fits_pass(3.0f, 7.0f), hy = fits_pass(7.0f, 3.0f);
        const float sx = ex3[0] + ex3[1] + ex3[2], sy = ey3[0] + ey3[1] + ey3[2];
        if (hx && hy) split = (sx >= sy) ? 1 : 2;
        else split = hx ? 1 : (hy ? 2 : 3);
        const float pe = ((split == 2) ? 7.0f : 3.0f) * ((m == 0) ? ex3[0] : ((m == 1) ? ex3[1] : ex3[2])) +
                         ((split == 1) ? 7.0f : 3.0f) * ((m == 0) ? ey3[0] : ((m == 1) ? ey3[1] : ey3[2]));
        const float dzs = fabsf(zref - readlane_f32(rc.dg.zlin(max(ke - 1, 0)), 0));
        const float per_sample = ((m == 0) ? d0[0] : ((m == 1) ? d0[1] : d0[2])) * dzs;
        const float more = (float)((split == 3) ? 3 : 1) * per_sample;
        phases_fit = pe + more <= a.fit_m + VOXE_T4_PHASE_MARGIN;
        if (VOXE_T4_SKEW == 2 && !phases_fit) {
          const float wx = (split == 2) ? 7.0f : 3.0f, wy = (split == 1) ? 7.0f : 3.0f;
          const float dmm = (m == 0) ? d0[0] : ((m == 1) ? d0[1] : d0[2]);
          float lat = 0.0f;
#pragma unroll
          for (int ax = 0; ax < 3; ++ax)
            if (ax != m) lat = fmaxf(lat, wx * ex3[ax] + wy * ey3[ax] + pe * (d0[ax] / dmm));
          phases_skew = lat <= fit_lat && 1.0f + more <= a.fit_m + VOXE_T4_PHASE_MARGIN;
          phases_fit = phases_skew;
        }
      }
    }
  }
  float strat_lo = 0.0f, strat_sp = 0.0f;
  if (ks + lane < c.S && lane <= ke + 1 - ks) {
    const float2 st = depth_stratum(rc.dg, ks + lane);
    strat_lo = st.x; strat_sp = st.y;
  }
  DepCtx dep;
  dep.cA = dep.cB = 0; dep.src_base = 0;
#pragma unroll
  for (int s4 = 0; s4 < 4; ++s4) dep.mA[s4] = dep.mB[s4] = 0.0f;
  if constexpr (DEP) {
    float basis[NCU_DEP];
    {
      const float vdir[3] = {rc.d[0] / rc.dnorm, rc.d[1] / rc.dnorm, rc.d[2] / rc.dnorm};
      sh_basis<NCU_DEP>(vdir, basis);
    }
    const int q0 = 4 * grp;
    dep.cA = q0 >= a.ng - 1 ? 3 : q0 / NCU_DEP;
    dep.cB = dep.cA;
#pragma unroll
    for (int s4 = 0; s4 < 4; ++s4) {
      const int q = q0 + s4;
      if (q >= a.ng) continue;
      const int src = q == a.ng - 1 ? 3 : q / NCU_DEP;
      float m = 1.0f;
      if (src != 3) {
        const int j = q - src * NCU_DEP;
        m = basis[0];
#pragma unroll
        for (int t = 1; t < NCU_DEP; ++t) m = (j == t) ? basis[t] : m;
      }
      if (src == dep.cA) dep.mA[s4] = m;
      else { dep.cB = src; dep.mB[s4] = m; }
    }
    dep.src_base = ((long long)tile * nseg + seg) * c.seg_len * 64 + lane - (long long)ks * 64;
  }

  auto run_pass = [&](const bool alive_q, const int centre_lane, const int centre_lane2, auto ph_tag, const int phase, const int xm1, const int xm2) {
    constexpr int PH = decltype(ph_tag)::value;
    int k_lo, k_hi;
    seg_sample_range(rc, alive_q, ks, ke, k_lo, k_hi);
    bool has = k_lo <= k_hi;
    if (has && seg > 0 && c.term_eps > 0.0f) {
      if (a.ray_state[ray_state_index(seg, 0, 6, c.R, r)] < c.term_eps) { has = false; k_hi = k_lo - 1; }
    }
    const int kmin = wave_min_i32(has ? k_lo : INT_MAX);
    const int kmax = wave_max_i32(has ? k_hi : -1);
    if (kmin > kmax) return;
    Geo4 geo;
    int m, ref_lane;
    {
      const unsigned long long hmk = __ballot(has);
      const int ref = ((hmk >> centre_lane) & 1ull) ? centre_lane : (__ffsll((long long)hmk) - 1);
      ref_lane = ref;
      const int ref2 = (VOXE_TILE_CENTRE2 && ref == centre_lane && ((hmk >> centre_lane2) & 1ull)) ? centre_lane2 : ref;
      const int N[3] = {g.X, g.Y, g.Z};
      float U0[3], DU[3];
#pragma unroll
      for (int ax = 0; ax < 3; ++ax) {
        const float ro = readlane_f32(rc.o[ax], ref), rd = 0.5f * (readlane_f32(rc.d[ax], ref) + readlane_f32(rc.d[ax], ref2));
        const float half = 0.5f * (float)N[ax];
        U0[ax] = ((ro * g.scale[ax] + g.bias[ax]) + 1.0f) * half - 0.5f;
        DU[ax] = rd * g.scale[ax] * half;
      }
      const float ax_ = fabsf(DU[0]), ay_ = fabsf(DU[1]), az_ = fabsf(DU[2]);
      m = (ax_ >= ay_ && ax_ >= az_) ? 0 : ((ay_ >= az_) ? 1 : 2);
      const int u = (m == 0) ? 1 : 0, v = (m == 2) ? 1 : 2;
      const float DUm = (m == 0) ? DU[0] : ((m == 1) ? DU[1] : DU[2]);
      const float U0m = (m == 0) ? U0[0] : ((m == 1) ? U0[1] : U0[2]);
      const float DUu = (u == 0) ? DU[0] : DU[1], U0u = (u == 0) ? U0[0] : U0[1];
      const float DUv = (v == 1) ? DU[1] : DU[2], U0v = (v == 1) ? U0[1] : U0[2];
      geo.sgn = (DUm < 0.0f) ? -1 : 1;
      const float inv = (DUm != 0.0f) ? 1.0f / DUm : 0.0f;
      geo.Bu = DUu * inv; geo.Au = U0u - geo.Bu * U0m;
      geo.Bv = DUv * inv; geo.Av = U0v - geo.Bv * U0m;
    }
    int sh = 0;
    if constexpr ((VOXE_T4_SKEW == 1 || (VOXE_T4_SKEW == 2 && PH > 1)) && !PREC && !DEP) {
      if (a.phases >= 0 && has && (VOXE_T4_SKEW == 1 || phases_skew)) {
        const int kmid = (kmin + kmax) >> 1;
        const float zmid = readlane_f32(rc.dg.zlin(kmid), ref_lane), zmid1 = readlane_f32(rc.dg.zlin(min(kmid + 1, c.S - 1)), ref_lane);
        const float om_ = (m == 0) ? rc.o[0] : ((m == 1) ? rc.o[1] : rc.o[2]), dm_ = (m == 0) ? rc.d[0] : ((m == 1) ? rc.d[1] : rc.d[2]);
        const float sc_ = (m == 0) ? g.scale[0] : ((m == 1) ? g.scale[1] : g.scale[2]);
        const float half_ = 0.5f * (float)((m == 0) ? g.X : ((m == 1) ? g.Y : g.Z));
        const float pos = (om_ + dm_ * zmid) * sc_ * half_;
        const float pos_ref = readlane_f32(pos, ref_lane);
        const float per_sample = fabsf(readlane_f32(dm_, ref_lane) * sc_ * half_ * (zmid1 - zmid));
        if (per_sample > 1e-6f) {
          const float ahead = (float)geo.sgn * (pos - pos_ref) / per_sample;
          sh = (int)rintf(fminf(fmaxf(ahead, -12.0f), 12.0f));
        }
      }
    }
    const bool skew = __ballot(sh != 0) != 0ull;
#define VOXE_T4_MARCH(AX)                                                                                                           \
    do {                                                                                                                            \
      if constexpr (PH > 1)                                                                                                         \
        bwd4_march<AX, KL, PREC, DEP, PH, true>(g, c, a, rc, win, tab, lane, r, has, k_lo, k_hi, kmin, kmax, seg, ks, geo, strat_lo, \
                                                strat_sp, dep, phase, xm1, xm2, phase - sh);                                   \
      else if constexpr (VOXE_T4_SKEW == 1 && !PREC && !DEP) {                                                                           \
        if (skew)                                                                                                                   \
          bwd4_march<AX, KL, PREC, DEP, 1, true>(g, c, a, rc, win, tab, lane, r, has, k_lo, k_hi, kmin, kmax, seg, ks, geo, strat_lo, \
                                                 strat_sp, dep, 0, 0, 0, -sh);                                                      \
        else                                                                                                                        \
          bwd4_march<AX, KL, PREC, DEP>(g, c, a, rc, win, tab, lane, r, has, k_lo, k_hi, kmin, kmax, seg, ks, geo, strat_lo, strat_sp, dep); \
      } else                                                                                                                        \
        bwd4_march<AX, KL, PREC, DEP>(g, c, a, rc, win, tab, lane, r, has, k_lo, k_hi, kmin, kmax, seg, ks, geo, strat_lo, strat_sp, dep); \
    } while (0)
    if (m == 0) VOXE_T4_MARCH(0);
    else if (m == 1) VOXE_T4_MARCH(1);
    else VOXE_T4_MARCH(2);
#undef VOXE_T4_MARCH
  };
  auto in_part = [&](int q) {
    const int hx = (lane >> 2) & 1, hy = (lane >> 5) & 1;
    return split == 0 ? true : (split == 1 ? hx == q : (split == 2 ? hy == q : hx + 2 * hy == q));
  };
  auto centre_of = [&](int q) {
    return split == 0 ? 27 : (split == 1 ? 26 + 4 * q : (split == 2 ? 19 + 32 * q : 18 + 4 * (q & 1) + 32 * (q >> 1)));
  };
  auto centre2_of = [&](int q) {
    return split == 0 ? 36 : (split == 1 ? 33 + 4 * q : (split == 2 ? 12 + 32 * q : 9 + 4 * (q & 1) + 32 * (q >> 1)));
  };
  const int nparts = split == 0 ? 1 : (split == 3 ? 4 : 2);
  const int q_begin = a.qsplit == 4 ? quad : 0;
  const int q_end = a.qsplit == 4 ? min(quad + 1, nparts) : nparts;
#ifndef VOXE_T4_PHASES_KL8
#define VOXE_T4_PHASES_KL8 0
#endif
#ifndef VOXE_T4_PHASES_KL10
#define VOXE_T4_PHASES_KL10 0
#endif
  constexpr bool kPhases = !PREC && !DEP && (KL >= 9 ? VOXE_T4_PHASES_KL10 != 0 : VOXE_T4_PHASES_KL8 != 0);
  if constexpr (kPhases) {
   if (split != 0 && a.phases >= 0 && phases_fit) {
    const int bx = (lane >> 2) & 1, by = (lane >> 5) & 1;
    for (int q = q_begin; q < q_end; ++q) {
      int phase, rl, xm1, xm2 = 0;
      if (split == 1) { phase = bx ^ q; rl = (lane & ~4) | (q << 2); xm1 = 4; }
      else if (split == 2) { phase = by ^ q; rl = (lane & ~32) | (q << 5); xm1 = 32; }
      else { phase = (bx ^ (q & 1)) | ((by ^ (q >> 1)) << 1); rl = (lane & ~36) | ((q & 1) << 2) | ((q >> 1) << 5); xm1 = 4; xm2 = 32; }
      const bool alive_q = columns ? tile_pixel_ray(c, ty, rl & 7, (tx << 3) + (rl >> 3), 8, r_px)
                                   : tile_pixel_ray(c, ty, rl >> 3, (tx << 3) + (rl & 7), 8, r_px);
      r = alive_q ? r_px : 0;
      rc.init(g, c, r, a.rays_o, a.rays_d, nullptr);
      if (split == 3) run_pass(alive_q, centre_of(q), centre2_of(q), std::integral_constant<int, 4>(), phase, xm1, xm2);
      else run_pass(alive_q, centre_of(q), centre2_of(q), std::integral_constant<int, 2>(), phase, xm1, xm2);
      __syncthreads();
    }
    return;
   }
  }
  for (int q = q_begin; q < q_end; ++q) {
    run_pass(alive && in_part(q), centre_of(q), centre2_of(q), std::integral_constant<int, 1>(), 0, 0, 0);
    __syncthreads();
  }
}

#ifndef VOXE_FWD4_LB
#define VOXE_FWD4_LB 4
#endif
template <int COUT, bool PREC>
__global__ __launch_bounds__(64, VOXE_FWD4_LB) void render_fwd_tile4_kernel(const DevGrid g, const DevCfg c,
                                                                            const float* __restrict__ packed,
                                                                            const float* __restrict__ rays_o,
                                                                            const float* __restrict__ rays_d,
                                                                            float* __restrict__ segbuf,
                                                                            double* __restrict__ segsum) {
  constexpr int NC = COUT + 3;
  static_assert(!PREC || COUT == 3, "precise_grad: SH-0 colour renders");
  const int lane = threadIdx.x;
  const int nseg = num_segments(c.S, c.seg_len);
  const int nrb = gridDim.x / nseg;
  const int seg = blockIdx.x / nrb, rb = blockIdx.x - seg * nrb;
  const int W = c.image_width;
  const int ntx = (W + 7) >> 3, nty = (int)tile_rows_total(c, 8);
  const int tile = logical_tile_of(c, rb, nrb, ntx, nty);
  if (tile < 0) return;
  const int ty = tile / ntx, tx = tile - ty * ntx;
  long long r_px;
#ifndef VOXE_F4_EXP
#define VOXE_F4_EXP 0
#endif
  bool alive = tile_pixel_ray(c, ty, lane >> 3, (tx << 3) + (lane & 7), 8, r_px);
  long long r = alive ? r_px : 0;
  RayCtx<COUT, 1, 1> rc;
  rc.init(g, c, r, rays_o, rays_d, nullptr);
  {
    const unsigned long long am = __ballot(alive);
    bool cols = (VOXE_F4_EXP & 1) != 0;
    if (!(VOXE_F4_EXP & 5) && (am & 1ull) && (am >> 1 & 1ull) && (am >> 8 & 1ull)) {
      const float d0[3] = {readlane_f32(rc.d[0], 0), readlane_f32(rc.d[1], 0), readlane_f32(rc.d[2], 0)};
      const float dx[3] = {readlane_f32(rc.d[0], 1), readlane_f32(rc.d[1], 1), readlane_f32(rc.d[2], 1)};
      const float dy[3] = {readlane_f32(rc.d[0], 8), readlane_f32(rc.d[1], 8), readlane_f32(rc.d[2], 8)};
      cols = tile_lanes_down_columns(g, d0, dx, dy);
    }
    if (cols) {
      alive = tile_pixel_ray(c, ty, lane & 7, (tx << 3) + (lane >> 3), 8, r_px);
      r = alive ? r_px : 0;
      rc.init(g, c, r, rays_o, rays_d, nullptr);
    }
  }
  const int ks = seg * c.seg_len, ke = min(c.S, ks + c.seg_len) - 1;
  int k_lo, k_hi;
  seg_sample_range(rc, alive, ks, ke, k_lo, k_hi);
  const bool has = k_lo <= k_hi;
  const int kmin = wave_min_dpp(has ? k_lo : INT_MAX);
  const int kmax = -wave_min_dpp(has ? -k_hi : INT_MAX);
  float csum[COUT];
  double csum_d[COUT];
#pragma unroll
  for (int ch = 0; ch < COUT; ++ch) { csum[ch] = 0.0f; csum_d[ch] = 0.0; }
  float asum = 0.0f, dsum = 0.0f, T = 1.0f;
  double asum_d = 0.0, dsum_d = 0.0;
  if (kmin <= kmax) {
    float strat_lo = 0.0f, strat_sp = 0.0f;
    if (ks + lane < c.S && lane <= ke + 1 - ks) {
      const float2 st = depth_stratum(rc.dg, ks + lane);
      strat_lo = st.x; strat_sp = st.y;
    }
    float z_next = 0.0f;
    if (has) {
      const float2 st = depth_stratum(rc.dg, k_lo);
      const float su = st.y * jitter_uniform(rc.dg.base, k_lo);
      z_next = st.x + su;
    }
    constexpr unsigned TB = (COUT + 1) * 4;
    const unsigned sxb = g.X > 1 ? (unsigned)(g.Y * g.Z) * TB : 0u, syb = g.Y > 1 ? (unsigned)g.Z * TB : 0u;
    const unsigned szb = g.Z > 1 ? TB : 0u;
    const unsigned sxi = (unsigned)(g.Y * g.Z) * TB, syi = (unsigned)g.Z * TB;
    const char* const pbytes = reinterpret_cast<const char*>(packed);
    const int Sm1 = c.S - 1;
    for (int k = kmin; k <= kmax; ++k) {
      const bool on = has && (k >= k_lo) && (k <= k_hi);
      const bool last = (k == Sm1);
      const float z = z_next;
      if (on && !last) {
        const int j = k + 1 - ks;
        const float lo = __int_as_float(__builtin_amdgcn_readlane(__float_as_int(strat_lo), j));
// ... 385 lines not shown
}

bool fwd_tile4_supported(const DevGrid& g, const HostCfg& c, const FwdArgs& a, int cout, int ncm) {
  if (c.disp.tile_lean < 0 || ncm != 1 || !((cout == 3 && !c.attn) || (cout == 1 && c.attn))) return false;
  if (a.jitter || c.aabb_clip || c.image_width <= 0 || !a.segbuf) return false;
  if (c.seg_len + 1 > 64) return false;
  const long long bytes = (long long)g.X * g.Y * g.Z * 16;
  return bytes < (1ll << 31) && (long long)g.Y * g.Z * 16 < (1 << 24) && g.X < (1 << 24);
}
void launch_fwd_tile4(const DevGrid& g, const HostCfg& c, const FwdArgs& a, hipStream_t st) {
  const int nseg = num_segments(c.S, c.seg_len);
  const int nb = blocks_for_tiles(c.map_mode, (c.image_width + 7) / 8, tile_rows_total(c, 8)) * nseg;
  int* const sched = (a.sched && tile_sched_applies(c)) ? a.sched : nullptr;
  if (sched) build_tile_sched(g, c, a.rays_o, a.rays_d, sched, st);
  if (c.attn) render_fwd_tile4_kernel<1, false><<<nb, 64, 0, st>>>(g, c, a.packed, a.rays_o, a.rays_d, a.segbuf, nullptr);
  else if (c.disp.fwd_window >= 0 && (reinterpret_cast<uintptr_t>(a.packed) & 15) == 0) {
    const float fit_lat = disp_or(c.disp.fwd_fit_lat, 5.5f), fit_m = disp_or(c.disp.fwd_fit_m, (float)kF4Ring - 1.5f);
    const float zdom = disp_or(c.disp.fwd_zdom, VOXE_FWD4W_ZDOM), max_adv = disp_or(c.disp.fwd_max_adv, 1.7f);
    if (a.segsum_d) render_fwd_tile4w_kernel<true><<<nb, 64, 0, st>>>(g, c, a.packed, a.rays_o, a.rays_d, a.segbuf, a.segsum_d, fit_lat, fit_m, zdom, max_adv, sched);
    else render_fwd_tile4w_kernel<false><<<nb, 64, 0, st>>>(g, c, a.packed, a.rays_o, a.rays_d, a.segbuf, nullptr, fit_lat, fit_m, zdom, max_adv, sched);
  }
  else if (a.segsum_d) render_fwd_tile4_kernel<3, true><<<nb, 64, 0, st>>>(g, c, a.packed, a.rays_o, a.rays_d, a.segbuf, a.segsum_d);
  else render_fwd_tile4_kernel<3, false><<<nb, 64, 0, st>>>(g, c, a.packed, a.rays_o, a.rays_d, a.segbuf, nullptr);
}

bool tile4_bwd_supported(const DevGrid& g, const HostCfg& c, const BwdArgs& a, int kl) {
  if (c.disp.tile_lean < 0) return false;
  if ((kl != 8 && kl != 10) || a.gdet || a.jitter || c.aabb_clip || c.attn || c.image_width <= 0) return false;
  if (c.seg_len + 1 > 64) return false;
  const long long bytes = (long long)g.X * g.Y * g.Z * 16;
  return bytes < (1ll << 31) && (long long)g.Y * g.Z * 16 < (1 << 24) && g.X < (1 << 24);
}

__global__ __launch_bounds__(256) void planar_to_packed_kernel(const float4* __restrict__ planar, float* __restrict__ gpacked,
                                                               const long long nvox, const int cm, const int ngrp) {
  constexpr int V = 64;
  extern __shared__ float4 p2p_buf4[];
  float* const buf = reinterpret_cast<float*>(p2p_buf4);
  const int tid = threadIdx.x;
  const long long nchunks = nvox / V;
  for (long long ck = blockIdx.x; ck < nchunks; ck += gridDim.x) {
    for (int q = tid; q < V * ngrp; q += 256) {
      const int gi = q / V, i = q - gi * V;
      const float4 t = planar[(long long)gi * nvox + ck * V + i];
      const float e[4] = {t.x, t.y, t.z, t.w};
#pragma unroll
      for (int u = 0; u < 4; ++u)
        if (4 * gi + u < cm) buf[i * cm + 4 * gi + u] = e[u];
    }
    __syncthreads();
    float4* __restrict__ g4 = reinterpret_cast<float4*>(gpacked + ck * V * cm);
    for (int q = tid; q < V * cm / 4; q += 256) {
      const float4 o = g4[q], t = p2p_buf4[q];
      g4[q] = make_float4(o.x + t.x, o.y + t.y, o.z + t.z, o.w + t.w);
    }
    __syncthreads();
  }
  if (blockIdx.x == 0) {
    const float* const pl = reinterpret_cast<const float*>(planar);
    for (long long e = nchunks * V * cm + tid; e < nvox * cm; e += 256) {
      const long long vox = e / cm;
      const int ch = (int)(e - vox * cm);
      gpacked[e] += pl[((long long)(ch >> 2) * nvox + vox) * 4 + (ch & 3)];
    }
  }
}

bool tile4_dep_supported(const DevGrid& g, const HostCfg& c, const BwdArgs& a, int ncu, int cm) {
  if (c.disp.tile_lean < 0 || !(ncu == 4 || ncu == 9 || ncu == 16) || cm != 3 * ncu + 1) return false;
  if (a.gdet || a.jitter || c.aabb_clip || c.attn || c.image_width <= 0 || !a.sample_src || !a.grad_planar) return false;
  if (c.seg_len + 1 > 64) return false;
  const long long bytes = (long long)g.X * g.Y * g.Z * 16;
  return bytes < (1ll << 31) && (long long)g.Y * g.Z * 16 < (1 << 24) && g.X < (1 << 24);
}
size_t tile_planar_bytes(long long nvox, int cm) { return (size_t)nvox * 16 * (size_t)((cm + 3) / 4); }
void launch_bwd_tile4_dep(const DevGrid& g, const HostCfg& c, const BwdArgs& a, int ncu, int nb, int qsplit, int ngrp, float fit_m,
                          float fit_lat, hipStream_t st) {
  Tile4Args t;
  t.packed = a.packed; t.rays_o = a.rays_o; t.rays_d = a.rays_d; t.colour = a.colour; t.depth = a.depth; t.acc = a.acc;
  t.d_colour = a.d_colour; t.d_depth = a.d_depth; t.d_acc = a.d_acc; t.ray_state = a.ray_state; t.gpacked = a.grad_planar;
  t.qsplit = qsplit; t.fit_m = fit_m; t.fit_lat = fit_lat; t.want_d = 1; t.want_f = 1;
  t.segsum = nullptr; t.phases = -1;
  t.sample_src = reinterpret_cast<const float4*>(a.sample_src);
  t.sched = nullptr;
  const int cm = 3 * ncu + 1;
  t.ngrp = ngrp; t.ng = cm; t.nvox = (long long)g.X * g.Y * g.Z;
  (void)hipMemsetAsync(a.grad_planar, 0, tile_planar_bytes(t.nvox, cm), st);
  if (ncu == 4) render_bwd_tile4_kernel<8, false, 4><<<nb, 64, 0, st>>>(g, c, t);
  else if (ncu == 9) render_bwd_tile4_kernel<8, false, 9><<<nb, 64, 0, st>>>(g, c, t);
  else render_bwd_tile4_kernel<8, false, 16><<<nb, 64, 0, st>>>(g, c, t);
  const long long nchunks = t.nvox / 64;
  planar_to_packed_kernel<<<(int)(nchunks < 8192 ? (nchunks > 0 ? nchunks : 1) : 8192), 256, (size_t)64 * cm * sizeof(float), st>>>(
      reinterpret_cast<const float4*>(a.grad_planar), a.gpacked, t.nvox, cm, ngrp);
}

void launch_bwd_tile4(const DevGrid& g, const HostCfg& c, const BwdArgs& a, int kl, int nb, int qsplit, float fit_m, float fit_lat,
                      hipStream_t st) {
  Tile4Args t;
  t.sample_src = nullptr; t.ngrp = 1; t.ng = 4; t.nvox = 0;
  t.packed = a.packed; t.rays_o = a.rays_o; t.rays_d = a.rays_d; t.colour = a.colour; t.depth = a.depth; t.acc = a.acc;
  t.d_colour = a.d_colour; t.d_depth = a.d_depth; t.d_acc = a.d_acc; t.ray_state = a.ray_state; t.gpacked = a.gpacked;
  t.qsplit = qsplit; t.fit_m = fit_m; t.fit_lat = fit_lat; t.want_d = a.want_d ? 1 : 0; t.want_f = a.want_f ? 1 : 0;
  t.segsum = a.segsum_d; t.phases = c.disp.tile_phases;
  t.sched = (a.sched && qsplit == 1 && tile_sched_applies(c)) ? a.sched : nullptr;
  if (a.segsum_d) {
    if (kl == 10) render_bwd_tile4_kernel<10, true><<<nb, 64, 0, st>>>(g, c, t);
    else render_bwd_tile4_kernel<8, true><<<nb, 64, 0, st>>>(g, c, t);
  } else if (kl == 10) render_bwd_tile4_kernel<10, false><<<nb, 64, 0, st>>>(g, c, t);
  else render_bwd_tile4_kernel<8, false><<<nb, 64, 0, st>>>(g, c, t);
}

}
```

### vox-e_amd/csrc/voxe_tile_window.hpp

```cpp
#pragma once

#include <limits.h>

#include "voxe_device.hpp"

namespace voxe {

#ifndef VOXE_TILE_ORIENT_K
#define VOXE_TILE_ORIENT_K 1.0f
#endif
#ifndef VOXE_TILE_CENTRE2
#define VOXE_TILE_CENTRE2 1
#endif
#ifndef VOXE_TILE_RING
#define VOXE_TILE_RING 6
#endif
constexpr int kRing = VOXE_TILE_RING;
__device__ __forceinline__ int ring_slot(int key) {
  if constexpr ((VOXE_TILE_RING & (VOXE_TILE_RING - 1)) == 0) return key & (VOXE_TILE_RING - 1);
  const int m = key % VOXE_TILE_RING;
  return m < 0 ? m + VOXE_TILE_RING : m;
}
#ifndef VOXE_TILE_PAD
#define VOXE_TILE_PAD 6
#endif
#ifndef VOXE_TILE_ROT
#define VOXE_TILE_ROT 25
#endif
#ifndef VOXE_TILE_LANEROT
#define VOXE_TILE_LANEROT(lane) (((lane) & 7) + 3 * ((lane) >> 3))
#endif
#ifndef VOXE_TILE_CROT
#define VOXE_TILE_CROT(lane) (lane)
#endif
#ifndef VOXE_TILE_SLOTINC
#define VOXE_TILE_SLOTINC 0
#endif
#ifndef VOXE_TILE_F64MUL
#define VOXE_TILE_F64MUL 0
#endif
#ifndef VOXE_TILE_SLIDE_MIN
#define VOXE_TILE_SLIDE_MIN 1
#endif
template <int KL>
struct Lat {
  static constexpr int kLat = KL;
  static constexpr int kLayerSlots = KL * KL;
  static constexpr int kPlane = kRing * KL * KL + VOXE_TILE_PAD;
  static constexpr int kCentre = KL / 2 - 1;
  static __device__ __forceinline__ int pos(int key, int ab) {
    if constexpr (KL == 8) return (ab + VOXE_TILE_ROT * ring_slot(key)) & 63;
    return ab;
  }
  static __device__ __forceinline__ int rot_of(int key) { return KL == 8 ? VOXE_TILE_ROT * ring_slot(key) : 0; }
  static __device__ __forceinline__ int wrap(int x) { return KL == 8 ? (x & 63) : x; }
};

#ifndef VOXE_TILE_PCB
#define VOXE_TILE_PCB 1
#endif
#ifndef VOXE_TILE_STRATA
#define VOXE_TILE_STRATA 1
#endif
#ifndef VOXE_TILE_STRATA_SH
#define VOXE_TILE_STRATA_SH 0
#endif
#ifndef VOXE_TILE_STRATA_BWD
#define VOXE_TILE_STRATA_BWD 0
#endif
#ifndef VOXE_TILE_AXIS_TEMPLATE_SH
#define VOXE_TILE_AXIS_TEMPLATE_SH 0
#endif
#ifndef VOXE_TILE_AXIS_TEMPLATE
#define VOXE_TILE_AXIS_TEMPLATE 1
#endif
template <int KL, int C>
struct WinMap {
  static constexpr bool kPcb = VOXE_TILE_PCB && (KL % 2 == 0) && C == 4 && (VOXE_TILE_RING % 2 == 0);
  static constexpr int kSB = 32, kSA = 32 * (KL / 2), kSS = 32 * (KL / 2) * (KL / 2);
  static constexpr int kDoubles = kPcb ? (VOXE_TILE_RING / 2) * kSS : C * Lat<KL>::kPlane;
  static __device__ __forceinline__ int at(int slot, int key, int a, int b, int ch) {
    if constexpr (kPcb) {
      (void)key;
      return (slot >> 1) * kSS + ((slot & 1) << 2) + (a >> 1) * kSA + ((a & 1) << 1) + (b >> 1) * kSB + (b & 1) + (ch << 3);
    } else {
      return ch * Lat<KL>::kPlane + slot * Lat<KL>::kLayerSlots + Lat<KL>::pos(key, a * KL + b);
    }
  }
};

__device__ __forceinline__ int wave_min_i32(int v) {
  v = min(v, __builtin_amdgcn_update_dpp(v, v, 0xB1, 0xF, 0xF, false));
  v = min(v, __builtin_amdgcn_update_dpp(v, v, 0x4E, 0xF, 0xF, false));
  v = min(v, __builtin_amdgcn_update_dpp(v, v, 0x141, 0xF, 0xF, false));
  v = min(v, __builtin_amdgcn_update_dpp(v, v, 0x140, 0xF, 0xF, false));
  const int a = __builtin_amdgcn_readlane(v, 0), b = __builtin_amdgcn_readlane(v, 16);
  const int c = __builtin_amdgcn_readlane(v, 32), d = __builtin_amdgcn_readlane(v, 48);
  return min(min(a, b), min(c, d));
}
__device__ __forceinline__ int wave_max_i32(int v) { return -wave_min_i32(-v); }

__device__ __forceinline__ float readlane_f32(float x, int lane) {
  return __int_as_float(__builtin_amdgcn_readlane(__float_as_int(x), lane));
}

struct Window {
  int m, u, v;
  int sgn;
  float Au, Bu, Av, Bv;
  int stride_m, stride_u, stride_v;
  int base;
  int ctr;

  __device__ __forceinline__ int off_u(int im) const { return (int)floorf(Au + Bu * (float)im) - ctr; }
  __device__ __forceinline__ int off_v(int im) const { return (int)floorf(Av + Bv * (float)im) - ctr; }
};

}
```

### vox-e_amd/voxe_hip/abi.py

```python
import ctypes as C

ABI_VERSION = 13

OK = 0
ERR_NULL_POINTER = -1
ERR_BAD_SHAPE = -2
ERR_UNSUPPORTED = -3
ERR_WORKSPACE = -4
ERR_LAUNCH = -5
ERR_NO_DEVICE = -6

ACT_IDENTITY = 0
ACT_ABS = 1
ACT_RELU = 2
ACT_SOFTPLUS = 3

DREG_CORRELATION, DREG_L2, DREG_L1 = 0, 1, 2

FEAT_SH = 0
FEAT_ATTN = 1

_f3 = C.c_float * 3


# ... 76 lines not shown

class VoxeGridRegularisers(C.Structure):
    _fields_ = [
        ("dcl_reference", C.c_void_p), ("dcl_weight", C.c_float), ("dcl_loss", C.c_void_p),
        ("scratch", C.c_void_p), ("scratch_bytes", C.c_size_t),
        ("density_kind", C.c_int32), ("feat_reference", C.c_void_p), ("feat_weight", C.c_float), ("feat_loss", C.c_void_p),
    ]


class VoxeReconStep(C.Structure):
    _fields_ = [
        ("H", C.c_int32), ("W", C.c_int32), ("focal", C.c_float),
        ("poses", C.c_void_p), ("image_rows", C.c_void_p), ("images", C.c_void_p), ("num_images", C.c_int32),
        ("K", C.c_int32), ("batch", C.c_int64), ("diffuse_regularisation", C.c_int32),
        ("lr", C.c_float), ("beta1", C.c_float), ("beta2", C.c_float), ("eps", C.c_float),
        ("step_densities", C.c_int64), ("step_features", C.c_int64),
        ("exp_avg_densities", C.c_void_p), ("exp_avg_sq_densities", C.c_void_p),
        ("exp_avg_features", C.c_void_p), ("exp_avg_sq_features", C.c_void_p),
        ("losses", C.c_void_p), ("zero_gradient_first", C.c_int32),
    ]


class VoxeAttnRefineStep(C.Structure):
    _fields_ = [
        ("attn_map", C.c_void_p), ("tv_weight", C.c_float), ("tv_loss_always", C.c_int32),
        ("lr", C.c_float), ("beta1", C.c_float), ("beta2", C.c_float), ("eps", C.c_float),
        ("step", C.c_int64), ("exp_avg", C.c_void_p), ("exp_avg_sq", C.c_void_p),
        ("losses", C.c_void_p), ("attn_render", C.c_void_p), ("zero_gradient_first", C.c_int32),
    ]


_P = C.c_void_p
_GD = C.POINTER(VoxeGridDesc)
_RC = C.POINTER(VoxeRenderCfg)

_COMMON = {
    "cast_rays": (C.c_int, [C.c_int32, C.c_int32, C.c_float, C.POINTER(C.c_float), C.POINTER(C.c_float), _P, _P], False, True),
    "cast_rays_indexed": (C.c_int, [C.c_int32, C.c_int32, C.c_float, _P, C.c_int32, _P, C.c_int64, _P, _P], False, True),
    "random_subset": (C.c_int, [C.c_int64, C.c_int64, C.c_uint64, C.c_uint64, _P], False, True),
    "render_fwd": (C.c_int, [_GD, _RC, _P, _P, C.c_int64, _P, _P, _P, _P, _P], True, True),
    "render_bwd": (C.c_int, [_GD, _RC, _P, _P, C.c_int64, _P, _P, _P, _P, _P, _P, _P, _P, _P, C.c_int32], True, True),
    "sample_probe": (C.c_int, [_GD, _RC, _P, _P, C.c_int64, _P, _P, _P, _P, _P, _P], True, True),
    "dcl_fwd_bwd": (C.c_int, [_P, _P, C.c_int64, C.c_float, _P, _P, C.c_int32], True, True),
    "density_diff_fwd_bwd": (C.c_int, [_P, _P, C.c_int64, C.c_int32, C.c_float, _P, _P, C.c_int32], True, True),
    "feature_correlation_fwd_bwd": (C.c_int, [_P, _P, C.c_int64, C.c_int32, C.c_float, _P, _P, C.c_int32], True, True),
    "tv_fwd_bwd": (C.c_int, [_P, C.c_int32, C.c_int32, C.c_int32, C.c_int32, C.c_float, _P, _P, C.c_int32], True, True),
    "adam_step": (C.c_int, [_P, _P, _P, _P, C.c_int64, C.c_float, C.c_float, C.c_float, C.c_float, C.c_int64], False, True),
    "upsample_trilinear": (C.c_int, [_P, C.c_int32, C.c_int32, C.c_int32, C.c_int32, _P, C.c_int32, C.c_int32, C.c_int32], False, True),
    "graph_build": (C.c_int, [_P, _P, C.c_int32, C.c_int32, C.c_int32, C.c_int32, C.c_float, C.c_int32, _P, _P], False, True),
    "graphcut": (C.c_int, [_P, _P, _P, C.c_int32, C.c_int32, C.c_int32, _P, _P], True, True),
    "cc_largest_k": (C.c_int, [_P, C.c_int32, C.c_int32, C.c_int32, C.c_int32, _P, _P], True, True),
}

GRAD_ANY, GRAD_LINEAR, GRAD_BRICKED = -1, 0, 1
ROUTE_NONE, ROUTE_SCATTER, ROUTE_TILE, ROUTE_PACKED_SCATTER, ROUTE_REGION, ROUTE_DETERMINISTIC = -1, 0, 1, 2, 3, 4
GRAPH_CAP_ONE = 1 << 28
DIR_XP, DIR_XM, DIR_YP, DIR_YM, DIR_ZP, DIR_ZM = range(6)

_CPU_RENDER_BWD = [_GD, _RC, _P, _P, C.c_int64, _P, _P, _P, _P, _P, _P, C.c_int32]

_QUERY_COMMON_FWD = [_GD, _P, C.c_int64, _P]
_QUERY_COMMON_BWD = [_GD, _P, C.c_int64, _P, _P, _P, C.c_int32]

HIP_ONLY = {
    "query_fwd": (C.c_int, _QUERY_COMMON_FWD + [C.c_int32, _P, C.c_size_t, _P]),
    "query_bwd": (C.c_int, _QUERY_COMMON_BWD + [C.c_int32, _P, C.c_size_t, _P]),
    "abi_version": (C.c_int, []),
    "strerror": (C.c_char_p, [C.c_int]),
    "device_check": (C.c_int, [C.c_char_p, C.c_size_t]),
    "workspace_bytes": (C.c_size_t, [_GD, _RC, C.c_int64]),
    "render_bwd_acc": (C.c_int, [_GD, _RC, _P, _P, C.c_int64, _P, _P, _P, _P, _P, _P, _P, C.c_int32, C.c_int32, C.c_int32,
                                 C.POINTER(C.c_int32), _P, C.c_size_t, _P]),
    "render_bwd_acc_into": (C.c_int, [_GD, _RC, _P, _P, C.c_int64, _P, _P, _P, _P, _P, _P, _P, C.c_int32, C.c_int32, C.c_int32,
                                      C.POINTER(C.c_int32), _P, C.c_size_t, _P, C.c_size_t, _P]),
    "render_bwd_layout": (C.c_int, [_GD, _RC, C.c_int64]),
    "workspace_grad_offset": (C.c_size_t, [_GD]),
    "workspace_grad_bytes": (C.c_size_t, [_GD]),
    "grid_adam_step": (C.c_int, [_GD, C.c_int32, C.c_int32, C.c_int32, _P, _P, _P, _P, _P, _P, C.c_float, C.c_float, C.c_float, C.c_float,
                                 C.c_int64, C.c_int64, C.POINTER(VoxeGridRegularisers), _P, C.c_size_t, _P]),
    "render_route": (C.c_int, [_GD, _RC, C.c_int64]),
    "disparity_bwd": (C.c_int, [_P, _P, _P, _P, _P, _P, _P, C.c_int64, _P]),
    "clock_probe": (C.c_int, [C.c_int32, C.POINTER(C.c_double), _P]),
    "region_debug_layout": (C.c_int, [_GD, _RC, C.c_int64, C.POINTER(C.c_int64)]),
    "recon_scratch_bytes": (C.c_size_t, [C.c_int64]),
    "recon_step": (C.c_int, [_GD, _RC, C.POINTER(VoxeReconStep), _P, C.c_size_t, _P, C.c_size_t, _P, C.c_size_t, _P]),
    "recon_prefetch_stats": (C.c_int, [C.POINTER(C.c_int64)]),
    "recon_prefetch": (C.c_int, [_GD, _RC, C.POINTER(VoxeReconStep), _P, C.c_size_t, _P, C.c_size_t, _P, C.c_size_t, _P]),
    "attn_masked_l1_scratch_bytes": (C.c_size_t, []),
    "attn_masked_l1": (C.c_int, [_P, _P, C.c_int64, _P, _P, _P, C.c_size_t, _P]),
    "attn_refine_scratch_bytes": (C.c_size_t, [_GD, C.c_int64]),
    "attn_refine_step": (C.c_int, [_GD, _RC, C.POINTER(VoxeAttnRefineStep), _P, _P, C.c_int64, _P, C.c_size_t, _P, C.c_size_t, _P]),
    "dcl_scratch_bytes": (C.c_size_t, [C.c_int64]),
    "tv_scratch_bytes": (C.c_size_t, [C.c_int32, C.c_int32, C.c_int32, C.c_int32]),
    "graphcut_scratch_bytes": (C.c_size_t, [C.c_int32, C.c_int32, C.c_int32]),
    "cc_scratch_bytes": (C.c_size_t, [C.c_int32, C.c_int32, C.c_int32, C.c_int32]),
    "profile_enable": (C.c_int, [C.c_int32]),
    "profile_read": (C.c_int, [C.POINTER(VoxeProfile)]),
    "mesh_scratch_bytes": (C.c_size_t, [C.c_int32, C.c_int32, C.c_int32]),
    "mesh_count": (C.c_int, [_GD, C.c_float, _P, _P, _P, C.c_size_t, _P]),
    "mesh_emit": (C.c_int, [_GD, C.c_float, _P, _P, C.c_int64, _P, C.c_int64, _P, C.c_size_t, _P]),
    "query_normals": (C.c_int, [_GD, _P, C.c_int64, _P, _P]),
    "render_normals": (C.c_int, [_GD, _RC, _P, _P, C.c_int64, _P, _P, _P, _P, _P]),
    "visibility_accumulate": (C.c_int, [_GD, _RC, _P, _P, C.c_int64, _P, _P, _P, _P]),
    "visibility_mask": (C.c_int, [_P, C.c_int32, C.c_int32, C.c_int32, C.c_float, C.c_int32, _P, _P]),
    "distortion_scratch_bytes": (C.c_size_t, [C.c_int64]),
    "distortion_fwd_bwd": (C.c_int, [_GD, _RC, _P, _P, C.c_int64, _P, C.c_float, _P, _P, _P, C.c_int32, _P, C.c_size_t, _P]),
    "distortion_debug_lanes": (C.c_int, [C.c_int32]),
}

CPU_ONLY = {
    "query_fwd": (C.c_int, _QUERY_COMMON_FWD),
    "query_bwd": (C.c_int, _QUERY_COMMON_BWD),
    "num_threads": (C.c_int, []),
    "jitter_uniform": (C.c_float, [C.c_uint64, C.c_uint64, C.c_int64, C.c_int32]),
}


def hip_symbols():
    return ["voxe_" + n for n in list(_COMMON) + list(HIP_ONLY)]


def cpu_symbols():
    return ["voxe_cpu_" + n for n in list(_COMMON) + list(CPU_ONLY)]


def declare(lib, prefix):
    cpu = prefix == "voxe_cpu_"
    for name, (res, args, ws, st) in _COMMON.items():
        fn = getattr(lib, prefix + name)
        a = list(args)
        if cpu and name == "render_bwd":
            a = list(_CPU_RENDER_BWD)
        if not cpu:
            if ws:
                a += [_P, C.c_size_t]
            if st:
                a += [_P]
        fn.restype = res
        fn.argtypes = a
    extra = CPU_ONLY if cpu else HIP_ONLY
    for name, (res, args) in extra.items():
        fn = getattr(lib, prefix + name)
        fn.restype = res
        fn.argtypes = list(args)
    return lib
```

### vox-e_amd/voxe_hip/dispatch.py

```python
import contextlib
import contextvars
import dataclasses
import functools
import os
from dataclasses import dataclass
from typing import Optional

from . import abi


@dataclass(frozen=True)
class Dispatch:
    bwd_mode: int = 0
    tile_map: int = 0
    tile_min_rays: int = 0
    tile_two_phase: int = 0
    tile_qsplit: int = 0
    tile_kl: int = 0
    tile_fit_m: float = 0.0
    tile_fit_lat: float = 0.0
    fwd_window: int = 0
    fwd_fit_lat: float = 0.0
    fwd_fit_m: float = 0.0
    fwd_zdom: float = 0.0
    fwd_max_adv: float = 0.0
    fwd_segments_per_thread: int = 0
    region_min_rays: int = 0
    region_image_ratio: float = 0.0
    tile_lean: int = 0
    precise_grad: int = 0
    region_lds_ranks: int = 0
    tile_phases: int = 0

    def struct(self) -> abi.VoxeDispatch:
        return _struct_of(self)


@functools.lru_cache(maxsize=None)
def _struct_of(d: Dispatch) -> abi.VoxeDispatch:
    s = abi.VoxeDispatch()
    for f in dataclasses.fields(d):
        setattr(s, f.name, getattr(d, f.name))
    return s


SHIPPED = Dispatch()
TILE_ALWAYS = Dispatch(tile_min_rays=-1)


def _env_int(name):
    v = os.environ.get(name)
    return None if v is None or v == "" else int(v)


def _env_float(name):
    v = os.environ.get(name)
    return None if v is None or v == "" else float(v)


@functools.lru_cache(maxsize=1)
def from_env() -> Dispatch:
    kw = {}
    mode = os.environ.get("VOXE_BWD_MODE")
    if mode == "scatter":
        kw["bwd_mode"] = 1
    elif mode == "packed":
        kw["bwd_mode"] = 2
    tmap = {"interleave": 1, "band": 2, "rows": 3, "cost": 4}.get(os.environ.get("VOXE_TILE_MAP", ""))
    if tmap:
        kw["tile_map"] = tmap
    v = _env_int("VOXE_TILE_MIN_RAYS")
    if v is not None:
        kw["tile_min_rays"] = -1 if v <= 0 else v
    if os.environ.get("VOXE_TILE_TWO_PHASE", "")[:1] == "0":
        kw["tile_two_phase"] = -1
    v = _env_int("VOXE_TILE_QSPLIT")
    if v:
        kw["tile_qsplit"] = 4 if v == 4 else 1
    v = _env_int("VOXE_TILE_KL")
    if v:
        kw["tile_kl"] = v
    for env, field in (("VOXE_TILE_FIT_M", "tile_fit_m"), ("VOXE_TILE_FIT_LAT", "tile_fit_lat"),
                       ("VOXE_FWD_TILE_FIT_LAT", "fwd_fit_lat"), ("VOXE_FWD_TILE_FIT_M", "fwd_fit_m"),
                       ("VOXE_FWD_TILE_ZDOM", "fwd_zdom"), ("VOXE_FWD_TILE_ADV", "fwd_max_adv")):
        f = _env_float(env)
        if f:
            kw[field] = f
    if os.environ.get("VOXE_FWD_TILE", "")[:1] == "0":
        kw["fwd_window"] = -1
    v = _env_int("VOXE_FSEG")
    if v and v > 0:
        kw["fwd_segments_per_thread"] = v
    v = _env_int("VOXE_REGION_MIN_RAYS")
    if v is not None:
        kw["region_min_rays"] = -1 if v < 0 else max(v, 1)
    f = _env_float("VOXE_REGION_IMAGE_RATIO")
    if f is not None:
        kw["region_image_ratio"] = -1.0 if f <= 0.0 else f
    if os.environ.get("VOXE_TILE_LEAN", "")[:1] == "0":
        kw["tile_lean"] = -1
    if os.environ.get("VOXE_PRECISE_GRAD", "")[:1] == "1":
        kw["precise_grad"] = 1
    if os.environ.get("VOXE_REGION_LDS_RANKS", "")[:1] == "0":
        kw["region_lds_ranks"] = -1
    if os.environ.get("VOXE_TILE_PHASES", "")[:1] == "0":
        kw["tile_phases"] = -1
    return Dispatch(**kw)


_override: contextvars.ContextVar = contextvars.ContextVar("voxe_dispatch_override", default=None)


def current() -> Dispatch:
    o = _override.get()
    return o if o is not None else from_env()


@contextlib.contextmanager
def override(base: Optional[Dispatch] = None, **fields):
    new = dataclasses.replace(base if base is not None else current(), **fields)
    token = _override.set(new)
    try:
        yield new
    finally:
        _override.reset(token)
```

Before: 228.9 million rays/s.

## Classify backward tiles by dominant axis and launch specialised fixed-axis kernels

Extends the tile schedule cost kernel to classify each tile-segment by whether its rays fit a narrow window along the x or y march axis, emitting class keys and a header of per-class offsets. The tile4 backward then launches two specialised kernels with a fixed march axis and a shallower LDS ring (lower register and LDS use, more occupancy), plus the general kernel for the remaining tiles. It may also reorient lanes down columns when that fits the ray footprint better. The aim is to cut the runtime axis branching and the LDS footprint for most tiles, at the cost of extra launches and classification work.

```diff
diff --git a/include/voxe.h b/include/voxe.h
--- a/include/voxe.h
+++ b/include/voxe.h
@@ -245,6 +245,7 @@
 
 int voxe_clock_probe(int32_t spin, double* shader_hz, void* stream);
 int voxe_region_debug_layout(const VoxeGridDesc* grid, const VoxeRenderCfg* cfg, int64_t R, int64_t out[17]);
+int voxe_tile_class_debug_layout(const VoxeGridDesc* grid, const VoxeRenderCfg* cfg, int64_t R, int64_t out[4]);
 
 int voxe_adam_step(float* param, const float* grad, float* exp_avg, float* exp_avg_sq, int64_t n,
                    float lr, float beta1, float beta2, float eps, int64_t step, void* stream);
diff --git a/vox-e_amd/csrc/voxe_api.hip b/vox-e_amd/csrc/voxe_api.hip
--- a/vox-e_amd/csrc/voxe_api.hip
+++ b/vox-e_amd/csrc/voxe_api.hip
@@ -344,6 +344,25 @@
   out[1] = (int64_t)l.sched_off;
   out[2] = ntp * num_segments(dc.S, dc.seg_len);
   out[3] = ntp;
+  return VOXE_OK;
+}
+
+int voxe_tile_class_debug_layout(const VoxeGridDesc* grid, const VoxeRenderCfg* cfg, int64_t R, int64_t out[4]) {
+  Variant v;
+  const int st = validate(grid, cfg, R, &v);
+  if (st) return st;
+  if (!out) return VOXE_ERR_NULL_POINTER;
+  DevGrid dg; HostCfg dc;
+  make_dev(grid, cfg, R, v, &dg, &dc);
+  const WsLayout l = ws_layout(grid, cfg, R);
+  out[0] = out[1] = out[2] = out[3] = 0;
+  if (!(l.total > l.sched_off && tile_classes_apply(dg, dc))) return VOXE_OK;
+  long long off[2];
+  tile_sched_class_layout(dc, off);
+  out[0] = 1;
+  out[1] = (int64_t)l.sched_off + off[0];
+  out[2] = (int64_t)l.sched_off + off[1];
+  out[3] = (int64_t)blocks_for_tiles(dc.map_mode, (dc.image_width + 7) / 8, tile_rows_total(dc, 8)) * num_segments(dc.S, dc.seg_len);
   return VOXE_OK;
 }
 
diff --git a/vox-e_amd/csrc/voxe_launch.hpp b/vox-e_amd/csrc/voxe_launch.hpp
--- a/vox-e_amd/csrc/voxe_launch.hpp
+++ b/vox-e_amd/csrc/voxe_launch.hpp
@@ -75,6 +75,8 @@
 bool tile_bwd_supported(const HostCfg& c, int deg);
 size_t tile_src_bytes(long long R, int W, int H, int S, int deg, int diffuse, int attn);
 void launch_bwd_tile(const DevGrid& g, const HostCfg& c, int deg, int diffuse, const BwdArgs& a, hipStream_t st);
+struct TileBwdGeom { int qsplit, kl; float fit_m, fit_lat; };
+TileBwdGeom tile_bwd_geom(const DevGrid& g, const HostCfg& c, int ngrp);
 bool tile4_bwd_supported(const DevGrid& g, const HostCfg& c, const BwdArgs& a, int kl);
 void launch_bwd_tile4(const DevGrid& g, const HostCfg& c, const BwdArgs& a, int kl, int nb, int qsplit, float fit_m, float fit_lat,
                       hipStream_t st);
@@ -86,6 +88,8 @@
 void launch_fwd_tile4(const DevGrid& g, const HostCfg& c, const FwdArgs& a, hipStream_t st);
 bool tile_sched_applies(const HostCfg& c);
 size_t tile_sched_bytes(long long R, int W, int H, int S);
+bool tile_classes_apply(const DevGrid& g, const HostCfg& c);
+void tile_sched_class_layout(const HostCfg& c, long long out[2]);
 bool fwd_tile_supported(const DevGrid& g, const HostCfg& c, int cout, int ncm);
 void launch_fwd_tile(const DevGrid& g, const HostCfg& c, const FwdArgs& a, hipStream_t st);
 bool fwd_tilew_supported(const DevGrid& g, const HostCfg& c, const FwdArgs& a, int cout, int ncm, int ncu);
diff --git a/vox-e_amd/csrc/voxe_render_tile.hip b/vox-e_amd/csrc/voxe_render_tile.hip
--- a/vox-e_amd/csrc/voxe_render_tile.hip
+++ b/vox-e_amd/csrc/voxe_render_tile.hip
@@ -993,22 +993,32 @@
 
 constexpr float kWideWindowRatio = 0.58f;
 
+TileBwdGeom tile_bwd_geom(const DevGrid& g, const HostCfg& c, const int ngrp) {
+  const long long ntx8 = (c.image_width + 7) / 8, nty8 = tile_rows_total(c, 8);
+  const int env_q = c.disp.tile_qsplit;
+  const long long tile_segs = ntx8 * nty8 * num_segments(c.S, c.seg_len);
+  const long long tiles = tile_segs * ngrp;
+  TileBwdGeom t;
+  t.qsplit = env_q ? (env_q == 4 ? 4 : 1) : (tiles <= 11000 ? 4 : 1);
+  const float env_fit_m = c.disp.tile_fit_m;
+  const int side = g.X > g.Y ? (g.X > g.Z ? g.X : g.Z) : (g.Y > g.Z ? g.Y : g.Z);
+  const bool wide = (float)side >= kWideWindowRatio * (float)c.image_width;
+  t.fit_lat = c.disp.tile_fit_lat;
+  t.fit_m = env_fit_m > 0.0f ? env_fit_m : (t.qsplit == 4 ? (wide ? 4.5f : 4.0f) : (tile_segs <= 16000 ? 4.5f : 5.5f));
+  const int env_kl = c.disp.tile_kl;
+  t.kl = env_kl ? env_kl : (wide ? 10 : 8);
+  return t;
+}
+
 template <int COUT, int NCM, int NCU>
 static void launch_bwd_tile_t(const DevGrid& g, const HostCfg& c, const BwdArgs& a, hipStream_t st) {
   const long long ntx8 = (c.image_width + 7) / 8, nty8 = tile_rows_total(c, 8);
-  const int env_q = c.disp.tile_qsplit;
   constexpr int NG = COUT * NCU + 1, WC = NG < 4 ? NG : 4, NGRP = (NG + WC - 1) / WC;
   const int grp_begin = a.want_f ? 0 : NGRP - 1, ngrp = a.want_f ? NGRP : 1;
-  const long long tiles = ntx8 * nty8 * num_segments(c.S, c.seg_len) * ngrp;
-  const int qsplit = env_q ? (env_q == 4 ? 4 : 1) : (tiles <= 11000 ? 4 : 1);
+  const TileBwdGeom geom = tile_bwd_geom(g, c, ngrp);
+  const int qsplit = geom.qsplit;
   const int nb = blocks_for_tiles(c.map_mode, ntx8, nty8) * num_segments(c.S, c.seg_len) * qsplit * ngrp;
-  const float env_fit_m = c.disp.tile_fit_m;
-  const long long tile_segs = ntx8 * nty8 * num_segments(c.S, c.seg_len);
-  const int side_for_kl = g.X > g.Y ? (g.X > g.Z ? g.X : g.Z) : (g.Y > g.Z ? g.Y : g.Z);
-  const bool wide = (float)side_for_kl >= kWideWindowRatio * (float)c.image_width;
-  const float env_fit_lat = c.disp.tile_fit_lat;
-  const float fit_lat = env_fit_lat;
-  const float fit_m = env_fit_m > 0.0f ? env_fit_m : (qsplit == 4 ? (wide ? 4.5f : 4.0f) : (tile_segs <= 16000 ? 4.5f : 5.5f));
+  const float fit_m = geom.fit_m, fit_lat = geom.fit_lat;
 #define VOXE_TBWD(WD, WF, MODE, KL, NB, GB, NGR)                                                 \
   render_bwd_tile_kernel<COUT, NCM, NCU, WD, WF, MODE, KL><<<NB, 64, 0, st>>>(                    \
       g, c, a.packed, a.rays_o, a.rays_d, a.jitter, a.colour, a.depth, a.acc, a.d_colour,         \
@@ -1042,9 +1052,7 @@
     else if (a.want_d) VOXE_TBWD(true, false, 0, 8, nb, grp_begin, ngrp);
     else VOXE_TBWD(false, true, 0, 8, nb, grp_begin, ngrp);
   } else {
-    const int env_kl = c.disp.tile_kl;
-    const int side = g.X > g.Y ? (g.X > g.Z ? g.X : g.Z) : (g.Y > g.Z ? g.Y : g.Z);
-    const int kl = env_kl ? env_kl : ((float)side >= kWideWindowRatio * (float)c.image_width ? 10 : 8);
+    const int kl = geom.kl;
 #define VOXE_TBWD_KL(KL)                                                       \
     do {                                                                       \
       if (a.want_d && a.want_f) VOXE_TBWD(true, true, 0, KL, nb, 0, 1);         \
diff --git a/vox-e_amd/csrc/voxe_render_tile4.hip b/vox-e_amd/csrc/voxe_render_tile4.hip
--- a/vox-e_amd/csrc/voxe_render_tile4.hip
+++ b/vox-e_amd/csrc/voxe_render_tile4.hip
@@ -26,6 +26,9 @@
 #endif
 #ifndef VOXE_T4_REMAT
 #define VOXE_T4_REMAT 0
+#endif
+#ifndef VOXE_T4_ORIENT
+#define VOXE_T4_ORIENT 1
 #endif
 #ifndef VOXE_T4_DEBUG
 #define VOXE_T4_DEBUG 0
@@ -43,7 +46,111 @@
   int ngrp, ng;
   long long nvox;
   const int* sched;
+  const int* sched_hdr;
 };
+
+struct Geo4 {
+  float Au, Bu, Av, Bv;
+  int sgn;
+};
+
+__device__ __forceinline__ bool tile_lanes_down_columns(const DevGrid& g, const float (&d0)[3], const float (&dx)[3], const float (&dy)[3]) {
+  float ex[3], ey[3];
+  const int N[3] = {g.X, g.Y, g.Z};
+#pragma unroll
+  for (int a = 0; a < 3; ++a) {
+    const float s = g.scale[a] * (float)N[a];
+    ex[a] = (dx[a] - d0[a]) * s;
+    ey[a] = (dy[a] - d0[a]) * s;
+  }
+  const float lat_x = ex[0] * ex[0] + ex[1] * ex[1], lat_y = ey[0] * ey[0] + ey[1] * ey[1];
+  return (ey[2] * ey[2]) * lat_x > (ex[2] * ex[2]) * lat_y;
+}
+
+template <class RC>
+__device__ __forceinline__ bool tile4_orient(const DevGrid& g, const DevCfg& c, const int ty, const int tx, const int lane,
+                                             const float* __restrict__ rays_o, const float* __restrict__ rays_d, RC& rc, bool& alive,
+                                             long long& r) {
+  const unsigned long long am0 = __ballot(alive);
+  if (!((am0 & 1ull) && (am0 >> 1 & 1ull) && (am0 >> 8 & 1ull))) return false;
+  const float d0[3] = {readlane_f32(rc.d[0], 0), readlane_f32(rc.d[1], 0), readlane_f32(rc.d[2], 0)};
+  const float dx[3] = {readlane_f32(rc.d[0], 1), readlane_f32(rc.d[1], 1), readlane_f32(rc.d[2], 1)};
+  const float dy[3] = {readlane_f32(rc.d[0], 8), readlane_f32(rc.d[1], 8), readlane_f32(rc.d[2], 8)};
+  if (!tile_lanes_down_columns(g, d0, dx, dy)) return false;
+  long long r_px;
+  alive = tile_pixel_ray(c, ty, lane & 7, (tx << 3) + (lane >> 3), 8, r_px);
+  r = alive ? r_px : 0;
+  rc.init(g, c, r, rays_o, rays_d, nullptr);
+  return true;
+}
+struct TileExtent {
+  bool known;
+  int m;
+  float zref;
+  float d0[3], ex3[3], ey3[3];
+};
+template <class RC>
+__device__ __forceinline__ TileExtent tile4_extent(const DevGrid& g, const RC& rc, const bool alive, const int ke) {
+  TileExtent t;
+  const unsigned long long am = __ballot(alive);
+  t.known = (am >> 1 & 1ull) && (am >> 8 & 1ull);
+  t.m = 0;
+  t.zref = readlane_f32(rc.dg.zlin(ke), 0);
+  const int N[3] = {g.X, g.Y, g.Z};
+#pragma unroll
+  for (int ax = 0; ax < 3; ++ax) {
+    const float s = g.scale[ax] * 0.5f * (float)N[ax];
+    const float da = readlane_f32(rc.d[ax], 0);
+    t.d0[ax] = fabsf(da * s);
+    t.ex3[ax] = fabsf((readlane_f32(rc.d[ax], 1) - da) * s * t.zref);
+    t.ey3[ax] = fabsf((readlane_f32(rc.d[ax], 8) - da) * s * t.zref);
+  }
+  t.m = (t.d0[0] >= t.d0[1] && t.d0[0] >= t.d0[2]) ? 0 : ((t.d0[1] >= t.d0[2]) ? 1 : 2);
+  return t;
+}
+__device__ __forceinline__ bool tile4_fits_pass(const TileExtent& t, const float wx, const float wy, const float fit_lat,
+                                                const float fit_m, const bool skew_ok) {
+  const int m = t.m;
+  float e[3];
+#pragma unroll
+  for (int ax = 0; ax < 3; ++ax) e[ax] = wx * t.ex3[ax] + wy * t.ey3[ax];
+  const float alongm = (m == 0) ? e[0] : ((m == 1) ? e[1] : e[2]);
+  const float dm = (m == 0) ? t.d0[0] : ((m == 1) ? t.d0[1] : t.d0[2]);
+  float lat = 0.0f;
+#pragma unroll
+  for (int ax = 0; ax < 3; ++ax)
+    if (ax != m) lat = fmaxf(lat, skew_ok ? e[ax] + alongm * (t.d0[ax] / dm) : e[ax]);
+  return lat <= fit_lat && (skew_ok || alongm <= fit_m);
+}
+__device__ __forceinline__ void pass_ref_lanes(const unsigned long long hmk, const int centre_lane, const int centre_lane2, int& ref,
+                                               int& ref2) {
+  ref = ((hmk >> centre_lane) & 1ull) ? centre_lane : (__ffsll((long long)hmk) - 1);
+  ref2 = (VOXE_TILE_CENTRE2 && ref == centre_lane && ((hmk >> centre_lane2) & 1ull)) ? centre_lane2 : ref;
+}
+template <class RC>
+__device__ __forceinline__ int pass_geometry(const DevGrid& g, const RC& rc, const int ref, const int ref2, const int force_m, Geo4& geo) {
+  const int N[3] = {g.X, g.Y, g.Z};
+  float U0[3], DU[3];
+#pragma unroll
+  for (int ax = 0; ax < 3; ++ax) {
+    const float ro = readlane_f32(rc.o[ax], ref), rd = 0.5f * (readlane_f32(rc.d[ax], ref) + readlane_f32(rc.d[ax], ref2));
+    const float half = 0.5f * (float)N[ax];
+    U0[ax] = ((ro * g.scale[ax] + g.bias[ax]) + 1.0f) * half - 0.5f;
+    DU[ax] = rd * g.scale[ax] * half;
+  }
+  const float ax_ = fabsf(DU[0]), ay_ = fabsf(DU[1]), az_ = fabsf(DU[2]);
+  const int m = force_m >= 0 ? force_m : ((ax_ >= ay_ && ax_ >= az_) ? 0 : ((ay_ >= az_) ? 1 : 2));
+  const int u = (m == 0) ? 1 : 0, v = (m == 2) ? 1 : 2;
+  const float DUm = (m == 0) ? DU[0] : ((m == 1) ? DU[1] : DU[2]);
+  const float U0m = (m == 0) ? U0[0] : ((m == 1) ? U0[1] : U0[2]);
+  const float DUu = (u == 0) ? DU[0] : DU[1], U0u = (u == 0) ? U0[0] : U0[1];
+  const float DUv = (v == 1) ? DU[1] : DU[2], U0v = (v == 1) ? U0[1] : U0[2];
+  geo.sgn = (DUm < 0.0f) ? -1 : 1;
+  const float inv = (DUm != 0.0f) ? 1.0f / DUm : 0.0f;
+  geo.Bu = DUu * inv; geo.Au = U0u - geo.Bu * U0m;
+  geo.Bv = DUv * inv; geo.Av = U0v - geo.Bv * U0m;
+  return m;
+}
 
 constexpr int kSchedMaxBuckets = 9;
 constexpr int kSchedMaxSegs = 64;
@@ -53,6 +160,24 @@
 #define VOXE_SCHED_BUCKET 4
 #endif
 static_assert(VOXE_SCHED_BUCKET >= 4 && 32 / VOXE_SCHED_BUCKET + 1 <= kSchedMaxBuckets, "bucket rows of the schedule histogram");
+enum { kSchedFitX = 0, kSchedFitY = 1, kSchedRest = 2, kSchedNone = 3 };
+constexpr int kSchedClasses = 3;
+constexpr int kSchedMaxKeys = kSchedClasses * (kSchedMaxBuckets - 1) + 1;
+constexpr int kSchedHdrInts = 16;
+constexpr int kSchedHdrLaunch = 8;
+#ifndef VOXE_SCHED_FIT_MIN
+#define VOXE_SCHED_FIT_MIN 0
+#endif
+#ifndef VOXE_SCHED_FIT_M4
+#define VOXE_SCHED_FIT_M4 0.0f
+#endif
+struct SchedClassArgs {
+  int ncls;
+  float fit_m, fit_lat;
+  float fit_m4;
+  int fit_min;
+};
+constexpr int kFitRing = 4;
 
 template <class RC>
 __device__ __forceinline__ void seg_sample_range(const RC& rc, const bool alive, const int ks, const int ke, int& k_lo, int& k_hi) {
@@ -62,29 +187,49 @@
 __device__ __forceinline__ int sched_rank(int it, int nbk) {
   return it == 0 ? nbk - 1 : nbk - 1 - min((it + VOXE_SCHED_BUCKET - 1) / VOXE_SCHED_BUCKET, nbk - 1);
 }
+__device__ __forceinline__ int sched_key(int it, int cls, int nbk) {
+  return it == 0 ? kSchedClasses * (nbk - 1) : cls * (nbk - 1) + sched_rank(it, nbk);
+}
+template <class RC>
+__device__ __forceinline__ int sched_block_class(const DevGrid& g, const RC& rc, const bool alive, const bool has, const int ke,
+                                                 const SchedClassArgs& ca) {
+  const TileExtent te = tile4_extent(g, rc, alive, ke);
+  if (!te.known) return kSchedRest;
+  const float fit_lat = ca.fit_lat > 0.0f ? ca.fit_lat : 8.0f - 2.5f;
+  if (!tile4_fits_pass(te, 7.0f, 7.0f, fit_lat, ca.fit_m4, false)) return kSchedRest;
+  int ref, ref2;
+  pass_ref_lanes(__ballot(has), 27, 36, ref, ref2);
+  Geo4 geo;
+  const int m = pass_geometry(g, rc, ref, ref2, -1, geo);
+  return (m == te.m && m != 2) ? m : kSchedRest;
+}
 
 __global__ __launch_bounds__(1024) void tile_sched_cost_kernel(const DevGrid g, const DevCfg c, const float* __restrict__ rays_o,
                                                                const float* __restrict__ rays_d, const int ntp, const int nbk,
-                                                               const int hstride, unsigned char* __restrict__ cost,
-                                                               unsigned char* __restrict__ hist) {
+                                                               const int hstride, const SchedClassArgs ca,
+                                                               unsigned char* __restrict__ cost, unsigned char* __restrict__ hist,
+                                                               unsigned char* __restrict__ keyb) {
   __shared__ unsigned char rk[kSchedMaxSegs][16];
   const int lane = threadIdx.x & 63, w = threadIdx.x >> 6;
   const int rb = blockIdx.x * 16 + w;
   const int nseg = num_segments(c.S, c.seg_len);
   const int ntx = (c.image_width + 7) >> 3, nty = (int)tile_rows_total(c, 8);
   const int tile = rb < ntp ? logical_tile_of(c, rb, ntp, ntx, nty) : -1;
+  const int nkeys = ca.ncls * (nbk - 1) + 1;
   if (tile < 0) {
     for (int seg = lane; seg < nseg; seg += 64) {
       if (rb < ntp) cost[(long long)seg * ntp + rb] = 0;
-      rk[seg][w] = rb < ntp ? (unsigned char)(nbk - 1) : (unsigned char)255;
+      if (rb < ntp && ca.ncls > 1) keyb[(long long)seg * ntp + rb] = (unsigned char)(nkeys - 1);
+      rk[seg][w] = rb < ntp ? (unsigned char)(nkeys - 1) : (unsigned char)255;
     }
   } else {
     const int ty = tile / ntx, tx = tile - ty * ntx;
     long long r_px;
-    const bool alive = tile_pixel_ray(c, ty, lane >> 3, (tx << 3) + (lane & 7), 8, r_px);
-    const long long r = alive ? r_px : 0;
+    bool alive = tile_pixel_ray(c, ty, lane >> 3, (tx << 3) + (lane & 7), 8, r_px);
+    long long r = alive ? r_px : 0;
     RayCtx<3, 1, 1> rc;
     rc.init(g, c, r, rays_o, rays_d, nullptr);
+    if (ca.ncls > 1 && VOXE_T4_ORIENT) tile4_orient(g, c, ty, tx, lane, rays_o, rays_d, rc, alive, r);
     for (int seg = 0; seg < nseg; ++seg) {
       const int ks = seg * c.seg_len, ke = min(c.S, ks + c.seg_len) - 1;
       int k_lo, k_hi;
@@ -93,16 +238,20 @@
       const int kmin = wave_min_i32(has ? k_lo : INT_MAX);
       const int kmax = wave_max_i32(has ? k_hi : -1);
       const int it = kmin <= kmax ? kmax - kmin + 1 : 0;
+      int cls = 0;
+      if (ca.ncls > 1 && it > 0) cls = sched_block_class(g, rc, alive, has, ke, ca);
       if (lane == 0) {
+        const int key = ca.ncls > 1 ? sched_key(it, cls, nbk) : sched_rank(it, nbk);
         cost[(long long)seg * ntp + rb] = (unsigned char)it;
-        rk[seg][w] = (unsigned char)sched_rank(it, nbk);
+        if (ca.ncls > 1) keyb[(long long)seg * ntp + rb] = (unsigned char)key;
+        rk[seg][w] = (unsigned char)key;
       }
     }
   }
   __syncthreads();
   const int ngrp = gridDim.x;
-  for (int p = threadIdx.x; p < nseg * nbk; p += 1024) {
-    const int seg = p / nbk, r = p - seg * nbk;
+  for (int p = threadIdx.x; p < nseg * nkeys; p += 1024) {
+    const int seg = p / nkeys, r = p - seg * nkeys;
     int n = 0;
 #pragma unroll
     for (int i = 0; i < 16; ++i) n += rk[seg][i] == r ? 1 : 0;
@@ -117,16 +266,19 @@
 }
 
 __global__ __launch_bounds__(256) void tile_sched_scatter_kernel(const unsigned char* __restrict__ cost,
+                                                                 const unsigned char* __restrict__ keyb,
                                                                  const unsigned char* __restrict__ hist, const int ntp,
-                                                                 const int ngrp, const int nbk, const int hstride,
-                                                                 int* __restrict__ list) {
-  __shared__ int s_tot[kSchedMaxBuckets], s_pre[kSchedMaxBuckets], s_base[kSchedMaxBuckets];
-  __shared__ int s_wc[kSchedMaxBuckets][4];
+                                                                 const int ngrp, const int nbk, const int ncls, const int hstride,
+                                                                 const int fit_min, int* __restrict__ list,
+                                                                 int* __restrict__ clist, int* __restrict__ hdr) {
+  __shared__ int s_tot[kSchedMaxKeys], s_pre[kSchedMaxKeys], s_base[kSchedMaxKeys], s_rbase[kSchedMaxBuckets];
+  __shared__ int s_wc[kSchedMaxKeys][4], s_rwc[kSchedMaxBuckets][4];
   const int tid = threadIdx.x, lane = tid & 63, w = tid >> 6;
   const int seg = blockIdx.y, nseg = gridDim.y;
+  const int nkeys = ncls * (nbk - 1) + 1;
   const int H = nseg * ngrp;
   const int G0 = seg * ngrp + blockIdx.x * 16;
-  for (int r = w; r < nbk; r += 4) {
+  for (int r = w; r < nkeys; r += 4) {
     const unsigned int* row = reinterpret_cast<const unsigned int*>(hist + (long long)r * hstride);
     int tot = 0, pre = 0;
     for (int q = lane; q * 4 < H; q += 64) {
@@ -146,36 +298,84 @@
   const int b = seg * ntp + rb;
   const int it = valid ? (int)cost[b] : 0;
   const int rank = valid ? sched_rank(it, nbk) : -1;
-  int within = 0, mine = 0;
-  for (int r = 0; r < nbk; ++r) {
-    const unsigned long long m = __ballot(rank == r);
-    if (rank == r) within = __popcll(m & ((1ull << lane) - 1ull));
+  const int key = valid ? (ncls > 1 ? (int)keyb[b] : rank) : -1;
+  int within = 0, mine = 0, rwithin = 0, rmine = 0;
+  for (int r = 0; r < nkeys; ++r) {
+    const unsigned long long m = __ballot(key == r);
+    if (key == r) within = __popcll(m & ((1ull << lane) - 1ull));
     if (lane == r) mine = __popcll(m);
   }
-  if (lane < nbk) s_wc[lane][w] = mine;
+  if (lane < nkeys) s_wc[lane][w] = mine;
+  if (ncls > 1) {
+    for (int r = 0; r < nbk; ++r) {
+      const unsigned long long m = __ballot(rank == r);
+      if (rank == r) rwithin = __popcll(m & ((1ull << lane) - 1ull));
+      if (lane == r) rmine = __popcll(m);
+    }
+    if (lane < nbk) s_rwc[lane][w] = rmine;
+  }
   __syncthreads();
-  if (tid < nbk) {
+  if (tid < nkeys) {
     int base = s_pre[tid];
     for (int r = 0; r < tid; ++r) base += s_tot[r];
     s_base[tid] = base;
   }
+  if (ncls > 1 && tid >= 64 && tid < 64 + nbk) {
+    const int r = tid - 64;
+    int base = 0;
+    for (int q = 0; q < nbk; ++q)
+      for (int k = (q == nbk - 1 ? nkeys - 1 : q); k < (q == nbk - 1 ? nkeys : nkeys - 1); k += nbk - 1)
+        base += q < r ? s_tot[k] : (q == r ? s_pre[k] : 0);
+    s_rbase[r] = base;
+  }
+  if (hdr && blockIdx.x == 0 && blockIdx.y == 0 && tid == 128) {
+    int off[kSchedClasses + 1], cnt[kSchedClasses + 1];
+    int run = 0;
+    for (int k = 0; k <= kSchedClasses; ++k) {
+      off[k] = run; cnt[k] = 0;
+      for (int r = k * (nbk - 1); r < (k + 1) * (nbk - 1) && r < nkeys; ++r) cnt[k] += s_tot[r];
+      run += cnt[k];
+      hdr[2 * k] = off[k]; hdr[2 * k + 1] = cnt[k];
+    }
+    const bool fx = cnt[kSchedFitX] < fit_min, fy = cnt[kSchedFitY] < fit_min;
+    int* const lh = hdr + kSchedHdrLaunch;
+    lh[0] = off[kSchedFitX]; lh[1] = fx ? 0 : cnt[kSchedFitX];
+    lh[2] = off[kSchedFitY]; lh[3] = fy ? 0 : cnt[kSchedFitY];
+    lh[4] = off[kSchedRest] - (fy ? cnt[kSchedFitY] : 0); lh[5] = cnt[kSchedRest] + (fy ? cnt[kSchedFitY] : 0);
+    lh[6] = off[kSchedFitX]; lh[7] = fx ? cnt[kSchedFitX] : 0;
+  }
   __syncthreads();
   if (valid) {
-    int pos = s_base[rank] + within;
-    for (int i = 0; i < w; ++i) pos += s_wc[rank][i];
-    list[pos] = it == 0 ? (b | kSchedEmpty) : b;
+    const int entry = it == 0 ? (b | kSchedEmpty) : b;
+    int pos = s_base[key] + within;
+    for (int i = 0; i < w; ++i) pos += s_wc[key][i];
+    if (ncls > 1) {
+      clist[pos] = entry;
+      pos = s_rbase[rank] + rwithin;
+      for (int i = 0; i < w; ++i) pos += s_rwc[rank][i];
+    }
+    list[pos] = entry;
   }
 }
 
 bool tile_sched_applies(const HostCfg& c) {
-  if ((c.disp.tile_map != 0 && c.disp.tile_map != 4) || c.image_width <= 0 || c.attn || c.disp.fwd_segments_per_thread > 1) return false;
+  const int tm = c.disp.tile_map;
+  if ((tm != 0 && tm != 4 && tm != 5 && tm != 6) || c.image_width <= 0 || c.attn || c.disp.fwd_segments_per_thread > 1) return false;
   const int nseg = num_segments(c.S, c.seg_len);
   const long long tiles = (long long)((c.image_width + 7) / 8) * tile_rows_total(c, 8);
   const long long nb = (long long)blocks_for_tiles(c.map_mode, (c.image_width + 7) / 8, tile_rows_total(c, 8)) * nseg;
-  return nseg > 1 && nseg <= kSchedMaxSegs && c.seg_len <= 32 && (tiles * nseg > 11000 || c.disp.tile_map == 4) && nb <= kSchedMaxBlocks;
+  return nseg > 1 && nseg <= kSchedMaxSegs && c.seg_len <= 32 && (tiles * nseg > 11000 || tm == 4 || tm == 6) && nb <= kSchedMaxBlocks;
+}
+bool tile_classes_apply(const DevGrid& g, const HostCfg& c) {
+  if (!tile_sched_applies(c) || c.disp.tile_map == 5 || c.disp.tile_map == 6 || c.disp.precise_grad > 0) return false;
+  const TileBwdGeom t = tile_bwd_geom(g, c, 1);
+  return t.qsplit == 1 && t.kl == 8;
 }
 static long long sched_hist_stride(long long ntp, int nseg) { return ((ntp + 15) / 16 * nseg + 3) / 4 * 4; }
 static long long sched_cost_bytes(long long nb) { return (nb + 15) / 16 * 16; }
+static long long sched_clist_offset(long long ntp, int nseg) {
+  return ntp * nseg * (long long)sizeof(int) + sched_cost_bytes(ntp * nseg) + kSchedMaxKeys * sched_hist_stride(ntp, nseg);
+}
 size_t tile_sched_bytes(long long R, int W, int H1, int S) {
   if (W <= 0 || R <= 0) return 0;
   const long long H = H1 > 0 ? H1 : R / W, nimg = R / (H * W);
@@ -183,7 +383,13 @@
   const int nseg = num_segments(S, seg_len_for(R));
   const long long nb = ntp * nseg;
   if (nb > kSchedMaxBlocks) return 0;
-  return (size_t)nb * sizeof(int) + (size_t)sched_cost_bytes(nb) + (size_t)(kSchedMaxBuckets * sched_hist_stride(ntp, nseg));
+  return (size_t)sched_clist_offset(ntp, nseg) + (size_t)(nb + kSchedHdrInts) * sizeof(int) + (size_t)nb;
+}
+void tile_sched_class_layout(const HostCfg& c, long long out[2]) {
+  const int nseg = num_segments(c.S, c.seg_len);
+  const long long ntp = blocks_for_tiles(c.map_mode, (c.image_width + 7) / 8, tile_rows_total(c, 8));
+  out[0] = sched_clist_offset(ntp, nseg);
+  out[1] = out[0] + ntp * nseg * (long long)sizeof(int);
 }
 static void build_tile_sched(const DevGrid& g, const HostCfg& c, const float* rays_o, const float* rays_d, int* sched, hipStream_t st) {
   const int nseg = num_segments(c.S, c.seg_len);
@@ -193,8 +399,21 @@
   unsigned char* hist = cost + sched_cost_bytes(nb);
   const int nbk = (c.seg_len + VOXE_SCHED_BUCKET - 1) / VOXE_SCHED_BUCKET + 1;
   const int ngrp = (ntp + 15) / 16, hstride = (int)sched_hist_stride(ntp, nseg);
-  tile_sched_cost_kernel<<<ngrp, 1024, 0, st>>>(g, c, rays_o, rays_d, ntp, nbk, hstride, cost, hist);
-  tile_sched_scatter_kernel<<<dim3((ntp + 255) / 256, nseg), 256, 0, st>>>(cost, hist, ntp, ngrp, nbk, hstride, sched);
+  SchedClassArgs ca;
+  ca.ncls = 1; ca.fit_m = 0.0f; ca.fit_lat = 0.0f; ca.fit_m4 = 0.0f; ca.fit_min = 0;
+  int *clist = nullptr, *hdr = nullptr;
+  unsigned char* keyb = nullptr;
+  if (tile_classes_apply(g, c)) {
+    const TileBwdGeom t = tile_bwd_geom(g, c, 1);
+    ca.ncls = kSchedClasses; ca.fit_m = t.fit_m; ca.fit_lat = t.fit_lat;
+    ca.fit_m4 = VOXE_SCHED_FIT_M4 > 0.0f ? VOXE_SCHED_FIT_M4 : fminf(t.fit_m, (float)kRing - 1.5f) - (float)(kRing - kFitRing);
+    ca.fit_min = c.disp.tile_map == 4 ? 0 : VOXE_SCHED_FIT_MIN;
+    clist = reinterpret_cast<int*>(reinterpret_cast<char*>(sched) + sched_clist_offset(ntp, nseg));
+    hdr = clist + nb;
+    keyb = reinterpret_cast<unsigned char*>(hdr + kSchedHdrInts);
+  }
+  tile_sched_cost_kernel<<<ngrp, 1024, 0, st>>>(g, c, rays_o, rays_d, ntp, nbk, hstride, ca, cost, hist, keyb);
+  tile_sched_scatter_kernel<<<dim3((ntp + 255) / 256, nseg), 256, 0, st>>>(cost, keyb, hist, ntp, ngrp, nbk, ca.ncls, hstride, ca.fit_min, sched, clist, hdr);
 }
 
 struct DepCtx {
@@ -212,11 +431,6 @@
   static __device__ __forceinline__ int mterm(int slot) { return (slot >> 1) * SS + ((slot & 1) << 5); }
   static __device__ __forceinline__ int aterm(int x_even) { return (x_even >> 1) * SA; }
   static __device__ __forceinline__ int bterm(int x_even) { return (x_even >> 1) * SB; }
-};
-
-struct Geo4 {
-  float Au, Bu, Av, Bv;
-  int sgn;
 };
 
 __device__ __forceinline__ int rfl(int x) { return __builtin_amdgcn_readfirstlane(x); }
@@ -253,20 +467,7 @@
   return min(min(a, b), min(c, d));
 }
 
-__device__ __forceinline__ bool tile_lanes_down_columns(const DevGrid& g, const float (&d0)[3], const float (&dx)[3], const float (&dy)[3]) {
-  float ex[3], ey[3];
-  const int N[3] = {g.X, g.Y, g.Z};
-#pragma unroll
-  for (int a = 0; a < 3; ++a) {
-    const float s = g.scale[a] * (float)N[a];
-    ex[a] = (dx[a] - d0[a]) * s;
-    ey[a] = (dy[a] - d0[a]) * s;
-  }
-  const float lat_x = ex[0] * ex[0] + ex[1] * ex[1], lat_y = ey[0] * ey[0] + ey[1] * ey[1];
-  return (ey[2] * ey[2]) * lat_x > (ex[2] * ex[2]) * lat_y;
-}
-
-template <int MA, int KL, bool PREC, bool DEP, int NP = 1, bool LK = (NP > 1)>
+template <int MA, int KL, bool PREC, bool DEP, int NP = 1, bool LK = (NP > 1), int RING = kRing>
 __device__ __forceinline__ void bwd4_march(const DevGrid& g, const DevCfg& c, const Tile4Args& a, RayCtx<3, 1, 1>& rc,
                                            double* __restrict__ win, int2* __restrict__ tab, const int lane, const long long r,
                                            bool has, const int k_lo, int k_hi, const int kmin, const int kmax, const int seg,
@@ -274,6 +475,7 @@
                                            const DepCtx& dep, const int phase = 0, const int xm1 = 0, const int xm2 = 0, const int koff = 0) {
   static_assert(!LK || (!PREC && !DEP), "per-lane sample indices (phases, skew): the SH-0 float kernel only");
   static_assert(NP == 1 || LK, "sample phases need the per-lane sample index");
+  static_assert(RING % 2 == 0, "layer roles of the deposit: slot parity == key parity");
   constexpr int UA = (MA == 0) ? 1 : 0, VA = (MA == 2) ? 1 : 2;
   constexpr int COUT = 3;
   constexpr int kCtr = Lat<KL>::kCentre;
@@ -371,7 +573,7 @@
   auto build_tab = [&](int key0) {
     const int key = key0 + lane, im = sgn * key;
     const int ou = (int)floorf(geo.Au + geo.Bu * (float)im) - kCtr, ov = (int)floorf(geo.Av + geo.Bv * (float)im) - kCtr;
-    tab[lane] = make_int2((ou & 0xffff) | (ov << 16), P::mterm(ring_slot(key)));
+    tab[lane] = make_int2((ou & 0xffff) | (ov << 16), P::mterm(ring_slot_of<RING>(key)));
   };
 
   auto depth_of = [&](int k) {
@@ -614,7 +816,7 @@
       const int xA0 = PU0 - ouA, xA1 = PU1 - ouA, yA0 = PV0 - ovA, yA1 = PV1 - ovA;
       const int xB0 = PU0 - ouB, xB1 = PU1 - ouB, yB0 = PV0 - ovB, yB1 = PV1 - ovB;
       const int klrel = min(relA, relB);
-      bool fits = (unsigned)(klrel - (base + nkey0)) < (unsigned)(kRing - 1);
+      bool fits = (unsigned)(klrel - (base + nkey0)) < (unsigned)(RING - 1);
       if constexpr (KL == 8) fits = fits && ((unsigned)(xA0 | xA1 | yA0 | yA1 | xB0 | xB1 | yB0 | yB1) < 8u);
       else fits = fits && (max(max(max((unsigned)xA0, (unsigned)xA1), max((unsigned)yA0, (unsigned)yA1)),
                                max(max((unsigned)xB0, (unsigned)xB1), max((unsigned)yB0, (unsigned)yB1))) < (unsigned)KL);
@@ -663,7 +865,7 @@
           if (wgt != 0.0f) {
             const int2 es = cm ? e1 : e0;
             const int aa = pu + cu - (int)(short)(es.x & 0xffff), bb = pv + cv - (es.x >> 16);
-            const bool inwin = !(VOXE_T4_DEBUG & 2) && ((unsigned)((cm ? rel1 : rel0) - brel) < (unsigned)kRing) &&
+            const bool inwin = !(VOXE_T4_DEBUG & 2) && ((unsigned)((cm ? rel1 : rel0) - brel) < (unsigned)RING) &&
                                ((unsigned)aa < (unsigned)KL) && ((unsigned)bb < (unsigned)KL);
             if (inwin) {
               double* const wp = reinterpret_cast<double*>(reinterpret_cast<char*>(win) +
@@ -830,8 +1032,8 @@
         flush_issue(base + n);
         if (VOXE_T4_ZPAIR == 2 && kPair && npend == 2) flush_consume(true);
         ++n;
-      } while (n < kRing && __ballot(nextkey <= base + n) == 0ull);
-      base = (n == kRing) ? wave_min_dpp(nextkey) : base + n;
+      } while (n < RING && __ballot(nextkey <= base + n) == 0ull);
+      base = (n == RING) ? wave_min_dpp(nextkey) : base + n;
       if (base != INT_MAX && base + nkey0 > kTabKeys / 2) {
         key0 = base;
         nkey0 = -key0;
@@ -841,7 +1043,7 @@
   }
   flush_consume(true);
   if (base != INT_MAX) {
-    for (int i = 0; i < kRing; ++i) {
+    for (int i = 0; i < RING; ++i) {
       flush_issue(base + i);
       if (!kPair || npend == 2) flush_consume(true);
     }
@@ -849,23 +1051,14 @@
   }
 }
 
-template <int KL, bool PREC, int NCU_DEP = 0>
-#ifndef VOXE_TILE4_LB_PREC
-#define VOXE_TILE4_LB_PREC 2
-#endif
-__global__ __launch_bounds__(64, KL >= 9 ? 2 : (PREC ? VOXE_TILE4_LB_PREC : VOXE_TILE4_LB)) void render_bwd_tile4_kernel(const DevGrid g, const DevCfg c, const Tile4Args a_in) {
+template <int KL, bool PREC, int NCU_DEP, int FIT_AX>
+__device__ __forceinline__ void bwd_tile4_block(const DevGrid& g, const DevCfg& c, const Tile4Args& a_in, double* __restrict__ win,
+                                                int2* __restrict__ tab, const int bid) {
   constexpr bool DEP = NCU_DEP > 0;
-  __shared__ double win[WinMap<KL, 4>::kDoubles];
-  __shared__ int2 tab[kTabKeys];
+  constexpr int RING = FIT_AX >= 0 ? kFitRing : kRing;
+  static_assert(FIT_AX < 0 || (KL == 8 && !PREC && !DEP && FIT_AX < 2), "per-axis kernels: SH-0, 8-wide window, lateral marches");
   const int lane = threadIdx.x;
-  int bid = blockIdx.x;
-  if constexpr (!DEP) {
-    if (a_in.sched) {
-      bid = a_in.sched[blockIdx.x];
-      if (bid < 0) return;
-    }
-  }
-  for (int i = lane; i < WinMap<KL, 4>::kDoubles; i += 64) win[i] = 0.0;
+  for (int i = lane; i < WinMap<KL, 4, RING>::kDoubles; i += 64) win[i] = 0.0;
 
   const int W = c.image_width;
   const int ntx = (W + 7) >> 3, nty = (int)tile_rows_total(c, 8);
@@ -887,57 +1080,22 @@
 
   RayCtx<3, 1, 1> rc;
   rc.init(g, c, r, a.rays_o, a.rays_d, nullptr);
-#ifndef VOXE_T4_ORIENT
-#define VOXE_T4_ORIENT 1
-#endif
   bool columns = false;
-  if (VOXE_T4_ORIENT && !DEP) {
-    const unsigned long long am0 = __ballot(alive);
-    if ((am0 & 1ull) && (am0 >> 1 & 1ull) && (am0 >> 8 & 1ull)) {
-      const float d0[3] = {readlane_f32(rc.d[0], 0), readlane_f32(rc.d[1], 0), readlane_f32(rc.d[2], 0)};
-      const float dx[3] = {readlane_f32(rc.d[0], 1), readlane_f32(rc.d[1], 1), readlane_f32(rc.d[2], 1)};
-      const float dy[3] = {readlane_f32(rc.d[0], 8), readlane_f32(rc.d[1], 8), readlane_f32(rc.d[2], 8)};
-      if (tile_lanes_down_columns(g, d0, dx, dy)) {
-        columns = true;
-        alive = tile_pixel_ray(c, ty, lane & 7, (tx << 3) + (lane >> 3), 8, r_px);
-        r = alive ? r_px : 0;
-        rc.init(g, c, r, a.rays_o, a.rays_d, nullptr);
-      }
-    }
-  }
+  if (VOXE_T4_ORIENT && !DEP)
+    columns = tile4_orient(g, c, ty, tx, lane, a.rays_o, a.rays_d, rc, alive, r);
 
   int split = 0;
   bool phases_fit = false;
   bool phases_skew = false;
-  {
-    const unsigned long long am = __ballot(alive);
-    if ((am >> 1 & 1ull) && (am >> 8 & 1ull)) {
-      const int N[3] = {g.X, g.Y, g.Z};
-      const float zref = readlane_f32(rc.dg.zlin(ke), 0);
-      float d0[3], ex3[3], ey3[3];
-#pragma unroll
-      for (int ax = 0; ax < 3; ++ax) {
-        const float s = g.scale[ax] * 0.5f * (float)N[ax];
-        const float da = readlane_f32(rc.d[ax], 0);
-        d0[ax] = fabsf(da * s);
-        ex3[ax] = fabsf((readlane_f32(rc.d[ax], 1) - da) * s * zref);
-        ey3[ax] = fabsf((readlane_f32(rc.d[ax], 8) - da) * s * zref);
-      }
-      const int m = (d0[0] >= d0[1] && d0[0] >= d0[2]) ? 0 : ((d0[1] >= d0[2]) ? 1 : 2);
+  if constexpr (FIT_AX < 0) {
+    const TileExtent te = tile4_extent(g, rc, alive, ke);
+    if (te.known) {
+      const int m = te.m;
+      const float zref = te.zref;
+      const float (&d0)[3] = te.d0, (&ex3)[3] = te.ex3, (&ey3)[3] = te.ey3;
       const float fit_lat = a.fit_lat > 0.0f ? a.fit_lat : (float)KL - 2.5f;
       const bool skew_ok = VOXE_T4_SKEW == 1 && !PREC && !DEP && a.phases >= 0;
-      auto fits_pass = [&](float wx, float wy) {
-        float e[3];
-#pragma unroll
-        for (int ax = 0; ax < 3; ++ax) e[ax] = wx * ex3[ax] + wy * ey3[ax];
-        const float alongm = (m == 0) ? e[0] : ((m == 1) ? e[1] : e[2]);
-        const float dm = (m == 0) ? d0[0] : ((m == 1) ? d0[1] : d0[2]);
-        float lat = 0.0f;
-#pragma unroll
-        for (int ax = 0; ax < 3; ++ax)
-          if (ax != m) lat = fmaxf(lat, skew_ok ? e[ax] + alongm * (d0[ax] / dm) : e[ax]);
-        return lat <= fit_lat && (skew_ok || alongm <= a.fit_m);
-      };
+      auto fits_pass = [&](float wx, float wy) { return tile4_fits_pass(te, wx, wy, fit_lat, a.fit_m, skew_ok); };
       if (!fits_pass(7.0f, 7.0f)) {
         const bool hx = fits_pass(3.0f, 7.0f), hy = fits_pass(7.0f, 3.0f);
         const float sx = ex3[0] + ex3[1] + ex3[2], sy = ey3[0] + ey3[1] + ey3[2];
@@ -1012,30 +1170,10 @@
     Geo4 geo;
     int m, ref_lane;
     {
-      const unsigned long long hmk = __ballot(has);
-      const int ref = ((hmk >> centre_lane) & 1ull) ? centre_lane : (__ffsll((long long)hmk) - 1);
+      int ref, ref2;
+      pass_ref_lanes(__ballot(has), centre_lane, centre_lane2, ref, ref2);
       ref_lane = ref;
-      const int ref2 = (VOXE_TILE_CENTRE2 && ref == centre_lane && ((hmk >> centre_lane2) & 1ull)) ? centre_lane2 : ref;
-      const int N[3] = {g.X, g.Y, g.Z};
-      float U0[3], DU[3];
-#pragma unroll
-      for (int ax = 0; ax < 3; ++ax) {
-        const float ro = readlane_f32(rc.o[ax], ref), rd = 0.5f * (readlane_f32(rc.d[ax], ref) + readlane_f32(rc.d[ax], ref2));
-        const float half = 0.5f * (float)N[ax];
-        U0[ax] = ((ro * g.scale[ax] + g.bias[ax]) + 1.0f) * half - 0.5f;
-        DU[ax] = rd * g.scale[ax] * half;
-      }
-      const float ax_ = fabsf(DU[0]), ay_ = fabsf(DU[1]), az_ = fabsf(DU[2]);
-      m = (ax_ >= ay_ && ax_ >= az_) ? 0 : ((ay_ >= az_) ? 1 : 2);
-      const int u = (m == 0) ? 1 : 0, v = (m == 2) ? 1 : 2;
-      const float DUm = (m == 0) ? DU[0] : ((m == 1) ? DU[1] : DU[2]);
-      const float U0m = (m == 0) ? U0[0] : ((m == 1) ? U0[1] : U0[2]);
-      const float DUu = (u == 0) ? DU[0] : DU[1], U0u = (u == 0) ? U0[0] : U0[1];
-      const float DUv = (v == 1) ? DU[1] : DU[2], U0v = (v == 1) ? U0[1] : U0[2];
-      geo.sgn = (DUm < 0.0f) ? -1 : 1;
-      const float inv = (DUm != 0.0f) ? 1.0f / DUm : 0.0f;
-      geo.Bu = DUu * inv; geo.Au = U0u - geo.Bu * U0m;
-      geo.Bv = DUv * inv; geo.Av = U0v - geo.Bv * U0m;
+      m = pass_geometry(g, rc, ref, ref2, FIT_AX, geo);
     }
     int sh = 0;
     if constexpr ((VOXE_T4_SKEW == 1 || (VOXE_T4_SKEW == 2 && PH > 1)) && !PREC && !DEP) {
@@ -1058,18 +1196,19 @@
 #define VOXE_T4_MARCH(AX)                                                                                                           \
     do {                                                                                                                            \
       if constexpr (PH > 1)                                                                                                         \
-        bwd4_march<AX, KL, PREC, DEP, PH, true>(g, c, a, rc, win, tab, lane, r, has, k_lo, k_hi, kmin, kmax, seg, ks, geo, strat_lo, \
+        bwd4_march<AX, KL, PREC, DEP, PH, true, RING>(g, c, a, rc, win, tab, lane, r, has, k_lo, k_hi, kmin, kmax, seg, ks, geo, strat_lo, \
                                                 strat_sp, dep, phase, xm1, xm2, phase - sh);                                   \
       else if constexpr (VOXE_T4_SKEW == 1 && !PREC && !DEP) {                                                                           \
         if (skew)                                                                                                                   \
-          bwd4_march<AX, KL, PREC, DEP, 1, true>(g, c, a, rc, win, tab, lane, r, has, k_lo, k_hi, kmin, kmax, seg, ks, geo, strat_lo, \
+          bwd4_march<AX, KL, PREC, DEP, 1, true, RING>(g, c, a, rc, win, tab, lane, r, has, k_lo, k_hi, kmin, kmax, seg, ks, geo, strat_lo, \
                                                  strat_sp, dep, 0, 0, 0, -sh);                                                      \
         else                                                                                                                        \
-          bwd4_march<AX, KL, PREC, DEP>(g, c, a, rc, win, tab, lane, r, has, k_lo, k_hi, kmin, kmax, seg, ks, geo, strat_lo, strat_sp, dep); \
+          bwd4_march<AX, KL, PREC, DEP, 1, false, RING>(g, c, a, rc, win, tab, lane, r, has, k_lo, k_hi, kmin, kmax, seg, ks, geo, strat_lo, strat_sp, dep); \
       } else                                                                                                                        \
-        bwd4_march<AX, KL, PREC, DEP>(g, c, a, rc, win, tab, lane, r, has, k_lo, k_hi, kmin, kmax, seg, ks, geo, strat_lo, strat_sp, dep); \
+        bwd4_march<AX, KL, PREC, DEP, 1, false, RING>(g, c, a, rc, win, tab, lane, r, has, k_lo, k_hi, kmin, kmax, seg, ks, geo, strat_lo, strat_sp, dep); \
     } while (0)
-    if (m == 0) VOXE_T4_MARCH(0);
+    if constexpr (FIT_AX >= 0) VOXE_T4_MARCH(FIT_AX);
+    else if (m == 0) VOXE_T4_MARCH(0);
     else if (m == 1) VOXE_T4_MARCH(1);
     else VOXE_T4_MARCH(2);
 #undef VOXE_T4_MARCH
@@ -1117,6 +1256,39 @@
     run_pass(alive && in_part(q), centre_of(q), centre2_of(q), std::integral_constant<int, 1>(), 0, 0, 0);
     __syncthreads();
   }
+}
+
+template <int KL, bool PREC, int NCU_DEP = 0>
+#ifndef VOXE_TILE4_LB_PREC
+#define VOXE_TILE4_LB_PREC 2
+#endif
+__global__ __launch_bounds__(64, KL >= 9 ? 2 : (PREC ? VOXE_TILE4_LB_PREC : VOXE_TILE4_LB)) void render_bwd_tile4_kernel(const DevGrid g, const DevCfg c, const Tile4Args a_in) {
+  __shared__ double win[WinMap<KL, 4>::kDoubles];
+  __shared__ int2 tab[kTabKeys];
+  int bid = blockIdx.x;
+  if constexpr (NCU_DEP == 0) {
+    if (a_in.sched) {
+      if (a_in.sched_hdr) {
+        const int* const lh = a_in.sched_hdr + kSchedHdrLaunch + 4;
+        const int i = blockIdx.x, n1 = lh[1];
+        if (i >= n1 + lh[3]) return;
+        bid = a_in.sched[i < n1 ? lh[0] + i : lh[2] + (i - n1)];
+      } else {
+        bid = a_in.sched[blockIdx.x];
+        if (bid < 0) return;
+      }
+    }
+  }
+  bwd_tile4_block<KL, PREC, NCU_DEP, -1>(g, c, a_in, win, tab, bid);
+}
+
+template <int AX>
+__global__ __launch_bounds__(64, 4) void render_bwd_tile4_fit_kernel(const DevGrid g, const DevCfg c, const Tile4Args a_in) {
+  __shared__ double win[WinMap<8, 4, kFitRing>::kDoubles];
+  __shared__ int2 tab[kTabKeys];
+  const int off = a_in.sched_hdr[kSchedHdrLaunch + 2 * AX], cnt = a_in.sched_hdr[kSchedHdrLaunch + 2 * AX + 1];
+  if ((int)blockIdx.x >= cnt) return;
+  bwd_tile4_block<8, false, 0, AX>(g, c, a_in, win, tab, a_in.sched[off + blockIdx.x]);
 }
 
 #ifndef VOXE_FWD4_LB
@@ -1668,7 +1840,7 @@
   t.qsplit = qsplit; t.fit_m = fit_m; t.fit_lat = fit_lat; t.want_d = 1; t.want_f = 1;
   t.segsum = nullptr; t.phases = -1;
   t.sample_src = reinterpret_cast<const float4*>(a.sample_src);
-  t.sched = nullptr;
+  t.sched = nullptr; t.sched_hdr = nullptr;
   const int cm = 3 * ncu + 1;
   t.ngrp = ngrp; t.ng = cm; t.nvox = (long long)g.X * g.Y * g.Z;
   (void)hipMemsetAsync(a.grad_planar, 0, tile_planar_bytes(t.nvox, cm), st);
@@ -1689,6 +1861,17 @@
   t.qsplit = qsplit; t.fit_m = fit_m; t.fit_lat = fit_lat; t.want_d = a.want_d ? 1 : 0; t.want_f = a.want_f ? 1 : 0;
   t.segsum = a.segsum_d; t.phases = c.disp.tile_phases;
   t.sched = (a.sched && qsplit == 1 && tile_sched_applies(c)) ? a.sched : nullptr;
+  t.sched_hdr = nullptr;
+  if (t.sched && !a.segsum_d && kl == 8 && tile_classes_apply(g, c)) {
+    long long off[2];
+    tile_sched_class_layout(c, off);
+    t.sched = reinterpret_cast<const int*>(reinterpret_cast<const char*>(a.sched) + off[0]);
+    t.sched_hdr = reinterpret_cast<const int*>(reinterpret_cast<const char*>(a.sched) + off[1]);
+    render_bwd_tile4_fit_kernel<0><<<nb, 64, 0, st>>>(g, c, t);
+    render_bwd_tile4_fit_kernel<1><<<nb, 64, 0, st>>>(g, c, t);
+    render_bwd_tile4_kernel<8, false><<<nb, 64, 0, st>>>(g, c, t);
+    return;
+  }
   if (a.segsum_d) {
     if (kl == 10) render_bwd_tile4_kernel<10, true><<<nb, 64, 0, st>>>(g, c, t);
     else render_bwd_tile4_kernel<8, true><<<nb, 64, 0, st>>>(g, c, t);
diff --git a/vox-e_amd/csrc/voxe_tile_window.hpp b/vox-e_amd/csrc/voxe_tile_window.hpp
--- a/vox-e_amd/csrc/voxe_tile_window.hpp
+++ b/vox-e_amd/csrc/voxe_tile_window.hpp
@@ -20,6 +20,12 @@
   if constexpr ((VOXE_TILE_RING & (VOXE_TILE_RING - 1)) == 0) return key & (VOXE_TILE_RING - 1);
   const int m = key % VOXE_TILE_RING;
   return m < 0 ? m + VOXE_TILE_RING : m;
+}
+template <int RING>
+__device__ __forceinline__ int ring_slot_of(int key) {
+  if constexpr ((RING & (RING - 1)) == 0) return key & (RING - 1);
+  const int m = key % RING;
+  return m < 0 ? m + RING : m;
 }
 #ifndef VOXE_TILE_PAD
 #define VOXE_TILE_PAD 6
@@ -74,11 +80,12 @@
 #ifndef VOXE_TILE_AXIS_TEMPLATE
 #define VOXE_TILE_AXIS_TEMPLATE 1
 #endif
-template <int KL, int C>
+template <int KL, int C, int RING = VOXE_TILE_RING>
 struct WinMap {
-  static constexpr bool kPcb = VOXE_TILE_PCB && (KL % 2 == 0) && C == 4 && (VOXE_TILE_RING % 2 == 0);
+  static constexpr bool kPcb = VOXE_TILE_PCB && (KL % 2 == 0) && C == 4 && (RING % 2 == 0);
   static constexpr int kSB = 32, kSA = 32 * (KL / 2), kSS = 32 * (KL / 2) * (KL / 2);
-  static constexpr int kDoubles = kPcb ? (VOXE_TILE_RING / 2) * kSS : C * Lat<KL>::kPlane;
+  static constexpr int kDoubles = kPcb ? (RING / 2) * kSS : C * Lat<KL>::kPlane;
+  static_assert(kPcb || RING == VOXE_TILE_RING, "the channel-plane map has one ring depth");
   static __device__ __forceinline__ int at(int slot, int key, int a, int b, int ch) {
     if constexpr (kPcb) {
       (void)key;
diff --git a/vox-e_amd/voxe_hip/abi.py b/vox-e_amd/voxe_hip/abi.py
--- a/vox-e_amd/voxe_hip/abi.py
+++ b/vox-e_amd/voxe_hip/abi.py
@@ -182,6 +182,7 @@
     "disparity_bwd": (C.c_int, [_P, _P, _P, _P, _P, _P, _P, C.c_int64, _P]),
     "clock_probe": (C.c_int, [C.c_int32, C.POINTER(C.c_double), _P]),
     "region_debug_layout": (C.c_int, [_GD, _RC, C.c_int64, C.POINTER(C.c_int64)]),
+    "tile_class_debug_layout": (C.c_int, [_GD, _RC, C.c_int64, C.POINTER(C.c_int64)]),
     "recon_scratch_bytes": (C.c_size_t, [C.c_int64]),
     "recon_step": (C.c_int, [_GD, _RC, C.POINTER(VoxeReconStep), _P, C.c_size_t, _P, C.c_size_t, _P, C.c_size_t, _P]),
     "recon_prefetch_stats": (C.c_int, [C.POINTER(C.c_int64)]),
diff --git a/vox-e_amd/voxe_hip/dispatch.py b/vox-e_amd/voxe_hip/dispatch.py
--- a/vox-e_amd/voxe_hip/dispatch.py
+++ b/vox-e_amd/voxe_hip/dispatch.py
@@ -66,7 +66,7 @@
         kw["bwd_mode"] = 1
     elif mode == "packed":
         kw["bwd_mode"] = 2
-    tmap = {"interleave": 1, "band": 2, "rows": 3, "cost": 4}.get(os.environ.get("VOXE_TILE_MAP", ""))
+    tmap = {"interleave": 1, "band": 2, "rows": 3, "cost": 4, "auto1": 5, "cost1": 6}.get(os.environ.get("VOXE_TILE_MAP", ""))
     if tmap:
         kw["tile_map"] = tmap
     v = _env_int("VOXE_TILE_MIN_RAYS")
```

After: 184.6 million rays/s. 19.4% lower.
